# linyicheng1/trackingBench-SLAM

Hardware: AMD Instinct MI355X
Metric: frames/sec end-to-end (extract+match+local-BA) (higher is better)
Workload: dtype u8 (pyramid/FAST/ORB/Hamming) + f64 (pose-opt/BA); 1 GPU; 1280x720 stereo, 8-level pyramid x0.8, 2000 kpts/image (FAST 80/30), searchByBF L<->R, pose-opt, 10-KF/5000-pt local BA x10 iters; distinct_synthetic_pairs=64, distinct_ba_windows=32, ba_partitions=3, ba_schedule=joined at the end of every step, parallelism=frames sharded x1, RCCL gather of tracks

## Files before the change

### include/tb_capi.h

```cpp
#ifndef TB_CAPI_H
#define TB_CAPI_H

#include "tb_types.h"

#ifdef __cplusplus
extern "C" {
#endif

typedef struct tb_ctx tb_ctx;
typedef struct tb_extractor tb_extractor;

int tb_create(int device, tb_ctx** out);
void tb_destroy(tb_ctx* ctx);
const char* tb_last_error(const tb_ctx* ctx);
const char* tb_strerror(int code);
const char* tb_version(void);
int tb_set_stream(tb_ctx* ctx, void* hip_stream);
int tb_synchronize(tb_ctx* ctx);
int tb_profile_enable(tb_ctx* ctx, int on);
int tb_profile_only(tb_ctx* ctx, const char* kernel);
int tb_pack_rows_dev(tb_ctx* ctx, const void* src, int row_bytes, int cap, const int32_t* counts, int nframes, void* dst,
                     long long* total);
int tb_set_concurrency(tb_ctx* ctx, int peers);
int tb_measure_copy_seconds(tb_ctx* ctx, const void* d_src, void* d_dst, size_t bytes, int reps, double* seconds);
int tb_debug_force_dense_fast(tb_ctx* ctx, int on);
int tb_profile_report(tb_ctx* ctx, char* buf, int cap);

int tb_scale_factors(int nlevels, float scale, float* sf, float* inv_sf, float* sigma2, float* inv_sigma2);
int tb_pyramid_sizes(int width, int height, int nlevels, const float* sf, int* widths, int* heights);
int tb_orb_quotas(int nlevels, const float* sf, int target, int* quotas);

int tb_extractor_create(tb_ctx* ctx, int width, int height, int nlevels, const float* sf,
                        const int* widths, const int* heights,
                        int max_images, int max_target, tb_extractor** out);
void tb_extractor_destroy(tb_extractor* ex);
int tb_extractor_set_images_host(tb_extractor* ex, const uint8_t* images, int n, int stride, size_t pitch);
int tb_extractor_set_images_dev(tb_extractor* ex, const uint8_t* dev_images, int n, int stride, size_t pitch);
int tb_extractor_set_levels_host(tb_extractor* ex, int index, const uint8_t* const* levels, const int* strides);
int tb_extractor_build_pyramid(tb_extractor* ex, int n);
int tb_extractor_get_level_host(tb_extractor* ex, int index, int level, uint8_t* out, int out_stride);
int tb_extractor_orb(tb_extractor* ex, int n, int target, float init_th, float min_th, int quota_mode,
                     const tb_keypoint* exit_keys, int n_exit);
int tb_extractor_fastgrid(tb_extractor* ex, int n, const float* inv_sf, int target, float threshold,
                          const uint8_t* occupancy, int n_occupancy);
int tb_extractor_counts_host(tb_extractor* ex, int n, int* counts);
int tb_extractor_results_host(tb_extractor* ex, int index, tb_keypoint* kps, uint8_t* desc, int cap, int* count);
int tb_extractor_results_dev(tb_extractor* ex, const tb_keypoint** kps, const uint8_t** desc,
                             const int32_t** counts, int* kp_capacity);
int tb_extractor_copy_results_dev(tb_extractor* ex, int n, tb_keypoint* kps, uint8_t* desc, int32_t* counts, int cap);
int tb_extractor_candidates_host(tb_extractor* ex, int index, int level, tb_corner* out, int cap, int* count);

int tb_pyramid(tb_ctx* ctx, const uint8_t* image, int width, int height, int stride, int nlevels,
               const float* sf, uint8_t* const* levels_out, const int* strides_out);
int tb_fast_detect(tb_ctx* ctx, const uint8_t* image, int width, int height, int stride, int threshold,
                   int nms, tb_corner* out, int cap, int* count);
int tb_orb_extract(tb_ctx* ctx, const uint8_t* const* levels, const int* widths, const int* heights,
                   const int* strides, int nlevels, const float* sf, int target, float init_th, float min_th,
                   const tb_keypoint* exit_keys, int n_exit, int use_quotas, int* quotas_inout,
                   tb_keypoint* kps, uint8_t* desc, int cap, int* count);
int tb_fastgrid_extract(tb_ctx* ctx, const uint8_t* const* levels, const int* widths, const int* heights,
                        const int* strides, int nlevels, const float* inv_sf, int target, float threshold,
                        const uint8_t* occupancy, int n_occupancy, tb_keypoint* kps, int cap, int* count);

int tb_descriptor_distance(const uint8_t* a, const uint8_t* b);
void tb_three_maxima(const int* bin_sizes, int nbins, int* ind1, int* ind2, int* ind3);
int tb_match_bf(tb_ctx* ctx, const uint8_t* d1, int n1, const uint8_t* d2, int n2, int crosscheck,
                tb_match* out, int cap, int* count);
int tb_search_by_bf(tb_ctx* ctx, const uint8_t* d1, int n1, const uint8_t* d2, int n2, float ratio,
                    float min_th, tb_match* out, int cap, int* count);
int tb_search_by_bf_batch_dev(tb_ctx* ctx, int npairs, const uint8_t* desc1, const int32_t* counts1,
                              const uint8_t* desc2, const int32_t* counts2, size_t set_pitch,
                              float ratio, float min_th, tb_match* out, int cap, int32_t* out_counts);

typedef struct tb_lsh tb_lsh;
int tb_lsh_draw_bits(int tables, int key_size, uint64_t seed, uint16_t* out);
int tb_lsh_create(tb_ctx* ctx, int tables, int key_size, int multi_probe_level, uint64_t seed, const uint16_t* bits,
                  tb_lsh** out);
void tb_lsh_destroy(tb_lsh* lsh);
int tb_lsh_info(const tb_lsh* lsh, int* tables, int* key_size, int* multi_probe_level, uint16_t* bits);
int tb_match_lsh(tb_ctx* ctx, const tb_lsh* lsh, const uint8_t* d1, int n1, const uint8_t* d2, int n2, tb_match* out, int cap,
                 int* count);
int tb_search_by_nn(tb_ctx* ctx, const tb_lsh* lsh, const uint8_t* d1, int n1, const uint8_t* d2, int n2, float ratio,
                    float min_th, tb_match* out, int cap, int* count);
int tb_search_by_nn_batch_dev(tb_ctx* ctx, const tb_lsh* lsh, int npairs, const uint8_t* desc1, const int32_t* counts1,
                              const uint8_t* desc2, const int32_t* counts2, size_t set_pitch, float ratio, float min_th,
                              tb_match* out, int cap, int32_t* out_counts);
int tb_search_by_violence(tb_ctx* ctx, const tb_keypoint* k1, const uint8_t* d1, int n1,
                          const tb_keypoint* k2, const uint8_t* d2, int n2, int img2_width, int img2_height,
                          int min_level, int max_level, float radius, int th_low, float nratio,
                          int histo_len, int check_orientation, tb_match* out, int cap, int* count);

int tb_search_by_bow(tb_ctx* ctx, const tb_keypoint* k1, const uint8_t* d1, int n1, const uint32_t* nodes1, const int32_t* start1,
                     const uint32_t* items1, int nn1, const tb_keypoint* k2, const uint8_t* d2, int n2, const uint8_t* has_mp2,
                     const uint32_t* nodes2, const int32_t* start2, const uint32_t* items2, int nn2, int map_point_only, int th_low,
                     float nratio, int histo_len, int check_orientation, tb_match* out, int cap, int* count);

int tb_search_by_projection(tb_ctx* ctx, const float Tcw1[16], const tb_camera* cam1, int img1_width, int img1_height,
                            const tb_keypoint* k1, const uint8_t* d1, const uint8_t* taken1, int n1,
                            const tb_keypoint* k2, const tb_mappoint* mp2, const uint8_t* mp2_desc, int n2,
                            const float* scale_factors, int nlevels, float nratio, int th_high, int histo_len,
                            int check_orientation, tb_match* out, int cap, int* count);
int tb_search_by_projection_map(tb_ctx* ctx, const float Tcw1[16], const tb_camera* cam1, int img1_width, int img1_height,
                                const tb_keypoint* k1, const uint8_t* d1, const uint8_t* taken1, int n1,
                                const tb_mappoint* mps, const uint8_t* mp_desc, int nmp,
                                const float* scale_factors, int nlevels, float nratio, float radio, int th_high,
                                tb_match* out, int cap, int* count);

int tb_frame_grid_batch_dev(tb_ctx* ctx, int nframes, const tb_keypoint* keys, const int32_t* counts, int key_pitch,
                            int img_width, int img_height, int32_t* cell_start, int32_t* cell_items);
int tb_search_by_projection_batch_dev(tb_ctx* ctx, int npairs, const float* Tcw1, const tb_camera* cam1, int img1_width,
                                      int img1_height, const tb_keypoint* k1, const uint8_t* d1, const uint8_t* taken1,
                                      const int32_t* n1, int pitch1, const int32_t* cell_start, const int32_t* cell_items,
                                      const tb_keypoint* k2, const tb_mappoint* mp2, const uint8_t* mp2_desc,
                                      const int32_t* n2, int pitch2, const float* scale_factors, int nlevels, float nratio,
                                      int th_high, int histo_len, int check_orientation, tb_match* out, int cap,
                                      int32_t* out_counts, int32_t* flags);

int tb_search_by_projection_map_batch_dev(tb_ctx* ctx, int npairs, const float* Tcw1, const tb_camera* cam1, int img1_width,
                                          int img1_height, const tb_keypoint* k1, const uint8_t* d1, const uint8_t* taken1,
                                          const int32_t* n1, int pitch1, const int32_t* cell_start, const int32_t* cell_items,
                                          const tb_mappoint* mps, const uint8_t* mp_desc, const int32_t* nmp, int mp_pitch,
                                          int max_nmp, const float* scale_factors, int nlevels, float nratio, float radio,
                                          int th_high, tb_match* out, int cap, int32_t* out_counts, int32_t* flags);
int tb_search_by_violence_batch_dev(tb_ctx* ctx, int npairs, const tb_keypoint* k1, const uint8_t* d1, const int32_t* n1,
                                    int pitch1, const tb_keypoint* k2, const uint8_t* d2, const int32_t* n2, int pitch2,
                                    const int32_t* cell_start2, const int32_t* cell_items2, int img2_width, int img2_height,
                                    int min_level, int max_level, float radius, int th_low, float nratio, int histo_len,
                                    int check_orientation, tb_match* out, int cap, int32_t* out_counts, int32_t* flags);

typedef struct tb_vocab tb_vocab;
int tb_vocab_create(tb_ctx* ctx, const tb_vocabulary* host, tb_vocab** out);
void tb_vocab_destroy(tb_vocab* v);
int tb_bow_transform(tb_ctx* ctx, const tb_vocab* voc, const uint8_t* desc, int n, int levelsup, int32_t* word_ids,
                     double* weights, int32_t* node_ids);
int tb_bow_transform_batch_dev(tb_ctx* ctx, const tb_vocab* voc, int nframes, const uint8_t* desc, const int32_t* counts,
                               int desc_pitch, int levelsup, int32_t* word_ids, int32_t* node_ids, double* weights,
                               uint64_t* fv_keys, int32_t* fv_counts);
int tb_bow_vector_batch_dev(tb_ctx* ctx, const tb_vocab* voc, int nframes, const int32_t* word_ids, const double* weights,
                            const int32_t* counts, int desc_pitch, int32_t* bv_words, double* bv_values, int32_t* bv_counts);
enum { TB_SCORE_PAIRWISE = 0, TB_SCORE_ALL_PAIRS = 1 };
int tb_bow_score(int scoring, const int32_t* a_words, const double* a_values, int na, const int32_t* b_words, const double* b_values,
                 int nb, double* out);
int tb_bow_score_batch_dev(tb_ctx* ctx, int scoring, int mode, int na, const int32_t* a_words, const double* a_values,
                           const int32_t* a_counts, int a_pitch, int nb, const int32_t* b_words, const double* b_values,
                           const int32_t* b_counts, int b_pitch, double* out);
typedef struct tb_bow_db tb_bow_db;
int tb_bow_db_create(tb_ctx* ctx, int nseq, int capacity, int pitch, int scoring, tb_bow_db** out);
void tb_bow_db_destroy(tb_bow_db* db);
int tb_bow_db_clear(tb_bow_db* db);
int tb_bow_db_add_dev(tb_bow_db* db, const int32_t* bv_words, const double* bv_values, const int32_t* bv_counts, int src_pitch,
                      int32_t kf_id);
int tb_bow_db_query_dev(tb_bow_db* db, const int32_t* q_words, const double* q_values, const int32_t* q_counts, int q_pitch,
                        int exclude_newest, int topk, double* scores, int32_t* top_slot, int32_t* top_kf, double* top_score,
                        int32_t* top_count);
int tb_bow_db_state_dev(tb_bow_db* db, const int32_t** words, const double** values, const int32_t** counts, const int32_t** kf_ids,
                        int* nadded);
typedef struct tb_kf_store tb_kf_store;
typedef struct tb_reloc_params {
    int map_point_only, th_low; float nratio; int histo_len, check_orientation;
    int min_inliers;
} tb_reloc_params;
typedef struct tb_reloc_out {
    int32_t *cand_kf, *cand_matches, *cand_rows, *cand_inliers, *cand_flags;
    float* cand_Tcw;
    int32_t *best_rank, *best_kf;
    float* best_Tcw;
} tb_reloc_out;
int tb_kf_store_create(tb_ctx* ctx, int nseq, int capacity, int pitch, int max_candidates, tb_kf_store** out);
void tb_kf_store_destroy(tb_kf_store* st);
int tb_kf_store_clear(tb_kf_store* st);
int tb_kf_store_add_dev(tb_kf_store* st, const tb_keypoint* keys, const uint8_t* desc, const int32_t* counts, const uint64_t* fv_keys,
                        const int32_t* fv_counts, const float* map_points, const uint8_t* mp_valid, int src_pitch, const float* Tcw,
                        int32_t kf_id);
int tb_kf_store_state_dev(tb_kf_store* st, const tb_keypoint** keys, const uint8_t** desc, const int32_t** counts,
                          const uint64_t** fv_keys, const int32_t** fv_counts, const float** map_points, const uint8_t** mp_valid,
                          const float** Tcw, const int32_t** kf_ids, int* nadded);
int tb_kf_store_work_dev(tb_kf_store* st, tb_match** matches, int32_t** match_counts, const tb_obs** rows, const int32_t** row_counts,
                         const uint8_t** outlier, int* pitch);
int tb_relocalize_batch_dev(tb_kf_store* st, const double K[4], int nlevels, float scale, const tb_keypoint* q_keys,
                            const uint8_t* q_desc, const int32_t* q_counts, const uint64_t* q_fv_keys, const int32_t* q_fv_counts,
                            int q_pitch, const int32_t* cand_slot, int ncand, const tb_reloc_params* params, const tb_reloc_out* out);
int tb_reloc_rows_dev(tb_kf_store* st, int nlevels, float scale, const tb_keypoint* q_keys, const int32_t* q_counts, int q_pitch,
                      const int32_t* cand_slot, int ncand, const int32_t* match_counts, int32_t* cand_rows);
int tb_search_by_bow_batch_dev(tb_ctx* ctx, int npairs, const tb_keypoint* k1, const uint8_t* d1, int pitch1,
                               const uint64_t* fv1, const int32_t* fv_counts1, const tb_keypoint* k2, const uint8_t* d2, int pitch2,
                               const uint64_t* fv2, const int32_t* fv_counts2, const uint8_t* has_mp2, int map_point_only,
                               int th_low, float nratio, int histo_len, int check_orientation, tb_match* out, int cap,
                               int32_t* out_counts, int32_t* flags);

#define TB_VOC_MAX_L 8
typedef struct tb_vocab_train_params { int k, L, weighting, scoring; uint64_t seed; int max_iters; } tb_vocab_train_params;
typedef struct tb_vocab_train_stats { int nnodes, nwords, capped_nodes, empty_clusters; int iters_per_level[TB_VOC_MAX_L]; } tb_vocab_train_stats;
int tb_vocab_train_dev(tb_ctx* ctx, const tb_vocab_train_params* params, int ndocs, const uint8_t* desc, const int32_t* counts,
                       int desc_pitch, tb_vocab** out, tb_vocab_train_stats* stats);
int tb_vocab_train(tb_ctx* ctx, const tb_vocab_train_params* params, int ndocs, const uint8_t* desc, const int32_t* counts,
                   tb_vocab** out, tb_vocab_train_stats* stats);
int tb_vocab_info(const tb_vocab* voc, int* nnodes, int* nwords, int* k, int* L, int* weighting, int* scoring);
int tb_vocab_export(const tb_vocab* voc, int32_t* child_start, int32_t* child_items, uint8_t* desc, int32_t* word_id, double* weight);

int tb_stereo_tracks_to_obs_batch_dev(tb_ctx* ctx, int nframes, const tb_keypoint* keys_left, const tb_keypoint* keys_right,
                                      int key_pitch, const tb_match* matches, const int32_t* match_counts, int match_pitch,
                                      const float K[4], float bf, const float* inv_sigma2, int nlevels, tb_obs* obs, int obs_pitch,
                                      int32_t* obs_counts);

int tb_pose_opt(tb_ctx* ctx, const double K[4], const float Tcw_in[16], const tb_obs* obs, int n,
                uint8_t* outlier, float Tcw_out[16], int* n_inliers, double* stats);
int tb_pose_opt_batch_dev(tb_ctx* ctx, int nproblems, const double K[4], const float* Tcw_in,
                          const tb_obs* obs, const int32_t* counts, int obs_pitch, uint8_t* outlier,
                          float* Tcw_out, int32_t* n_inliers, double* stats);
int tb_clahe(tb_ctx* ctx, const uint8_t* src, int width, int height, int stride, double clip_limit, int tiles_x, int tiles_y,
             uint8_t* dst, int dst_stride);
int tb_clahe_dev(tb_ctx* ctx, const uint8_t* src, int width, int height, int stride, double clip_limit, int tiles_x, int tiles_y,
                 uint8_t* dst, int dst_stride);
int tb_optical_flow_pyr_lk(tb_ctx* ctx, const uint8_t* prev, const uint8_t* next, int width, int height, int stride,
                           const float* prev_pts, int n, int win, int max_level, float* next_pts, uint8_t* status,
                           float* err, int* top_level);
int tb_search_by_opflow(tb_ctx* ctx, const uint8_t* img1, const uint8_t* img2, int width, int height, int stride,
                        const tb_camera* cam1, const float* keys2_xy, int n, int equalized, int reject,
                        float* cur_points, tb_match* out, int cap, int* count);
int tb_search_by_opflow_batch_dev(tb_ctx* ctx, int npairs, const uint8_t* img1, const uint8_t* img2, int width, int height,
                                  int stride, size_t image_pitch, const tb_camera* cam1, const float* keys2_xy,
                                  const int32_t* counts, int pts_pitch, int equalized, int reject, float* cur_points,
                                  uint8_t* status, tb_match* out, int cap, int32_t* out_counts);
int tb_optical_flow_pyr_lk_dev(tb_ctx* ctx, const uint8_t* prev, const uint8_t* next, int width, int height, int stride,
                               const float* prev_pts, int n, int win, int max_level, float* next_pts, uint8_t* status,
                               float* err);
int tb_optical_flow_pyr_lk_batch_dev(tb_ctx* ctx, int npairs, const uint8_t* prev, const uint8_t* next, int width, int height,
                                     int stride, size_t image_pitch, const float* prev_pts, const int32_t* counts,
                                     int pts_pitch, int win, int max_level, float* next_pts, uint8_t* status, float* err);

int tb_find_fundamental_ransac(tb_ctx* ctx, const float* pts1, const float* pts2, int n, double thresh, double conf, uint8_t* mask,
                               double* F, int* iters, int* ok);
int tb_reject_with_f(tb_ctx* ctx, const float* cur_pts, const float* last_pts, int n, uint8_t* status);
int tb_reject_with_f_batch_dev(tb_ctx* ctx, int npairs, const float* cur_pts, const float* last_pts, const int32_t* counts,
                               int pts_pitch, uint8_t* status);
int tb_add_map_points_by_stereo(tb_ctx* ctx, const uint8_t* img_stereo, const uint8_t* img_current, int width, int height, int stride,
                                const tb_camera* cam_stereo, const float* keys_xy, int n, float bf, float* depth, int* n_depth);
int tb_add_map_points_by_stereo_batch_dev(tb_ctx* ctx, int npairs, const uint8_t* img_stereo, const uint8_t* img_current, int width,
                                          int height, int stride, size_t image_pitch, const tb_camera* cam_stereo, const float* keys_xy,
                                          const int32_t* counts, int pts_pitch, float bf, float* cur_points, uint8_t* status,
                                          float* depth);

int tb_local_ba(tb_ctx* ctx, const double K[4], int nkf, int nfixed, float* poses, int npt, float* pts,
                const tb_ba_obs* obs, int nobs, int iters, double* stats);
int tb_local_ba_batch_dev(tb_ctx* ctx, int nwindows, const double K[4], int nkf, int nfixed, float* poses, int npt,
                          float* pts, const tb_ba_obs* obs, const int32_t* obs_counts, int obs_pitch, int iters,
                          double* stats);

typedef struct tb_vo tb_vo;
typedef struct tb_vo_params {
    int width, height;
    int nlevels;
    float scale;
    int target;
    float init_th, min_th;
    double K[4];
    float bf;
    int keyframe_every;
} tb_vo_params;
int tb_vo_create(tb_ctx* ctx, const tb_vo_params* params, int nseq, tb_vo** out);
void tb_vo_destroy(tb_vo* vo);
int tb_vo_reset_dev(tb_vo* vo, const float* Tcw0);
int tb_vo_step_dev(tb_vo* vo, const uint8_t* left, const uint8_t* right, int stride, size_t pitch);
int tb_vo_state_dev(tb_vo* vo, const float** Tcw, const float** keys_xy, const float** map_points, const uint8_t** mp_valid,
                    const int32_t** key_counts, const tb_obs** obs, const int32_t** obs_counts, const int32_t** n_inliers,
                    const uint8_t** outlier, int* key_pitch, int* frame);

int tb_vo_reset_seq_dev(tb_vo* vo, const uint8_t* which, const float* Tcw0);
int tb_vo_step_ragged_dev(tb_vo* vo, const uint8_t* left, const uint8_t* right, int stride, size_t pitch, const uint8_t* active,
                          const uint8_t* force_keyframe);
int tb_vo_frames(tb_vo* vo, int32_t* frames, int32_t* kf_frames);

enum { TB_VO_OPFLOW = 0, TB_VO_BF = 1, TB_VO_VIOLENCE = 2, TB_VO_PROJECTION = 3, TB_VO_PROJECTION_MAP = 4, TB_VO_BOW = 5 };
typedef struct tb_vo_tracker {
    int kind;
    float bf_ratio, bf_min_th;
    int min_level, max_level;
    float radius;
    int th_low; float nratio; int histo_len; int check_orientation;
    int th_high;
    float radio;
    int map_keyframes;
} tb_vo_tracker;
int tb_vo_create_ex(tb_ctx* ctx, const tb_vo_params* params, const tb_vo_tracker* tracker, int nseq, tb_vo** out);
int tb_vo_tracker_state_dev(tb_vo* vo, const tb_keypoint** orb, const uint8_t** orb_desc, const int32_t** orb_counts,
                            const tb_match** matches, const int32_t** match_counts, const int32_t** flags, const tb_keypoint** kf_orb,
                            const uint8_t** kf_desc, const float** kf_map_points, const uint8_t** kf_mp_valid,
                            const int32_t** kf_counts, int* kf_frame);
typedef struct tb_vo_bow {
    int levelsup;
    int map_point_only;
    int th_low; float nratio; int histo_len; int check_orientation;
} tb_vo_bow;
int tb_vo_create_bow(tb_ctx* ctx, const tb_vo_params* params, const tb_vo_bow* bow, const tb_vocab* voc, int nseq, tb_vo** out);
enum { TB_VO_NN = 6 };
typedef struct tb_vo_lsh {
    float ratio, min_th;
    int min_level, max_level;
    int tables, key_size, multi_probe_level;
    uint64_t seed;
    const uint16_t* bits;
} tb_vo_lsh;
int tb_vo_create_lsh(tb_ctx* ctx, const tb_vo_params* params, const tb_vo_lsh* lsh, int nseq, tb_vo** out);
int tb_vo_bow_state_dev(tb_vo* vo, const uint64_t** fv_keys, const int32_t** fv_counts, const int32_t** bv_words, const double** bv_values,
                        const int32_t** bv_counts, const int32_t** word_ids, const int32_t** node_ids, const uint64_t** kf_fv_keys,
                        const int32_t** kf_fv_counts, const int32_t** kf_bv_words, const double** kf_bv_values, const int32_t** kf_bv_counts,
                        const int32_t** kf_word_ids, const int32_t** kf_node_ids);
int tb_vo_bow_db_enable(tb_vo* vo, int capacity);
int tb_vo_bow_db_get(tb_vo* vo, tb_bow_db** out);
int tb_vo_reloc_enable(tb_vo* vo, int max_candidates);
int tb_vo_relocalize_dev(tb_vo* vo, int topk, int exclude_newest, int min_inliers, double* scores, int32_t* top_slot, int32_t* top_kf,
                         double* top_score, int32_t* top_count, const tb_reloc_out* out);
int tb_vo_kf_store_get(tb_vo* vo, tb_kf_store** out);
typedef struct tb_vo_recover {
    int lost_inliers;
    int topk;
    int exclude_newest;
    int min_inliers;
} tb_vo_recover;
int tb_vo_recover_enable(tb_vo* vo, const tb_vo_recover* prm);
int tb_vo_recover_state_dev(tb_vo* vo, const uint8_t** lost, const int32_t** track_inliers, const int32_t** recovered_kf,
                            const int32_t** kf_ids, const int32_t** kf_word_ring, const int32_t** kf_node_ring);
typedef struct tb_vo_window_ba {
    int iters;
    int fixed;
    int min_obs;
    int min_points;
} tb_vo_window_ba;
int tb_vo_window_ba_enable(tb_vo* vo, const tb_vo_window_ba* prm);
int tb_vo_window_state_dev(tb_vo* vo, const float** seg_keys, const uint8_t** seg_ok, const float** seg_pose, const float** seg_pts,
                           const uint8_t** seg_spawned, const tb_ba_obs** obs, const int32_t** obs_counts, const int32_t** n_points,
                           const double** stats, const uint8_t** adopted, const float** ba_pose, const float** ba_pts, int* slot,
                           int* nslots);
int tb_vo_mp_desc_dev(tb_vo* vo, const uint8_t** mp_desc, const uint8_t** kf_mp_desc);
int tb_vo_map_state_dev(tb_vo* vo, const tb_mappoint** points, const uint8_t** desc, const int32_t** counts,
                        const int32_t** block_counts, int* capacity, int* map_keyframes, int* blocks);

typedef struct tb_batch_params {
    int width, height, nlevels;
    float scale;
    int target;
    float init_th, min_th;
    float bf_ratio, bf_min_th;
} tb_batch_params;
int tb_batch_run(tb_ctx** ctxs, int ngpu, const tb_batch_params* p, int nframes, const uint8_t* left, const uint8_t* right,
                 int stride, size_t pitch, int cap, tb_keypoint* kps, uint8_t* desc, int32_t* counts, tb_match* matches,
                 int32_t* match_counts);

#ifdef __cplusplus
}
#endif
#endif
```

### trackingbench_slam_amd/capi.py

```python
import ctypes as C
import os
import subprocess

import numpy as np

_HERE = os.path.dirname(os.path.abspath(__file__))
LIB_PATH = os.environ.get("TB_HIP_LIB") or os.path.join(_HERE, "libtb_hip.so")
_LIB = None

KEYPOINT = np.dtype([("x", "<f4"), ("y", "<f4"), ("size", "<f4"), ("angle", "<f4"),
                     ("response", "<f4"), ("octave", "<i4"), ("class_id", "<i4")])
MATCH = np.dtype([("queryIdx", "<i4"), ("trainIdx", "<i4"), ("imgIdx", "<i4"), ("distance", "<f4")])
CORNER = np.dtype([("x", "<i4"), ("y", "<i4"), ("score", "<i4")])
OBS = np.dtype([("u", "<f4"), ("v", "<f4"), ("X", "<f4"), ("Y", "<f4"), ("Z", "<f4"), ("inv_sigma2", "<f4")])
BA_OBS = np.dtype([("kf", "<i4"), ("pt", "<i4"), ("u", "<f4"), ("v", "<f4"), ("inv_sigma2", "<f4")])
CAMERA = np.dtype([("fx", "<f4"), ("fy", "<f4"), ("cx", "<f4"), ("cy", "<f4"), ("width", "<i4"), ("height", "<i4"),
                   ("has_distortion", "<i4"), ("d", "<f4", (5,))])
MAPPOINT = np.dtype([("pos", "<f4", (3,)), ("normal", "<f4", (3,)), ("min_dist", "<f4"), ("max_dist", "<f4"), ("bad", "<i4")])

TB_OK, TB_EINVAL, TB_ENOMEM, TB_ECAPACITY, TB_EUNSUPPORTED, TB_EDEVICE, TB_ESTATE = 0, -1, -2, -3, -4, -5, -6

EXPORTS = [
    "tb_create", "tb_destroy", "tb_last_error", "tb_strerror", "tb_version", "tb_set_stream", "tb_synchronize",
    "tb_profile_enable", "tb_profile_only", "tb_profile_report", "tb_debug_force_dense_fast", "tb_measure_copy_seconds", "tb_set_concurrency", "tb_pack_rows_dev",
    "tb_scale_factors", "tb_pyramid_sizes", "tb_orb_quotas",
    "tb_extractor_create", "tb_extractor_destroy", "tb_extractor_set_images_host", "tb_extractor_set_images_dev",
    "tb_extractor_set_levels_host", "tb_extractor_build_pyramid", "tb_extractor_get_level_host", "tb_extractor_orb",
    "tb_extractor_fastgrid", "tb_extractor_counts_host", "tb_extractor_results_host", "tb_extractor_results_dev",
    "tb_extractor_candidates_host", "tb_extractor_copy_results_dev",
    "tb_pyramid", "tb_fast_detect", "tb_orb_extract", "tb_fastgrid_extract",
    "tb_descriptor_distance", "tb_three_maxima", "tb_match_bf", "tb_search_by_bf", "tb_search_by_bf_batch_dev",
    "tb_search_by_violence", "tb_search_by_bow", "tb_search_by_projection", "tb_search_by_projection_map", "tb_frame_grid_batch_dev",
    "tb_search_by_projection_batch_dev", "tb_search_by_projection_map_batch_dev",
    "tb_search_by_violence_batch_dev", "tb_stereo_tracks_to_obs_batch_dev", "tb_vocab_create", "tb_vocab_destroy", "tb_bow_transform",
    "tb_bow_transform_batch_dev", "tb_search_by_bow_batch_dev", "tb_pose_opt", "tb_pose_opt_batch_dev", "tb_local_ba", "tb_local_ba_batch_dev",
    "tb_clahe", "tb_clahe_dev", "tb_optical_flow_pyr_lk", "tb_optical_flow_pyr_lk_dev", "tb_optical_flow_pyr_lk_batch_dev", "tb_search_by_opflow", "tb_search_by_opflow_batch_dev",
    "tb_find_fundamental_ransac", "tb_reject_with_f", "tb_reject_with_f_batch_dev", "tb_add_map_points_by_stereo", "tb_add_map_points_by_stereo_batch_dev",
    "tb_batch_run", "tb_vo_create", "tb_vo_destroy", "tb_vo_reset_dev", "tb_vo_step_dev", "tb_vo_state_dev",
    "tb_vo_create_ex", "tb_vo_tracker_state_dev", "tb_vo_mp_desc_dev", "tb_vo_map_state_dev",
    "tb_vocab_train", "tb_vocab_train_dev", "tb_vocab_info", "tb_vocab_export",
    "tb_bow_vector_batch_dev", "tb_vo_create_bow", "tb_vo_bow_state_dev",
    "tb_bow_score", "tb_bow_score_batch_dev", "tb_bow_db_create", "tb_bow_db_destroy", "tb_bow_db_clear", "tb_bow_db_add_dev",
    "tb_bow_db_query_dev", "tb_bow_db_state_dev", "tb_vo_bow_db_enable", "tb_vo_bow_db_get",
    "tb_kf_store_create", "tb_kf_store_destroy", "tb_kf_store_clear", "tb_kf_store_add_dev", "tb_kf_store_state_dev",
    "tb_kf_store_work_dev", "tb_relocalize_batch_dev", "tb_reloc_rows_dev", "tb_vo_reloc_enable", "tb_vo_relocalize_dev",
    "tb_vo_kf_store_get", "tb_vo_recover_enable", "tb_vo_recover_state_dev",
    "tb_vo_reset_seq_dev", "tb_vo_step_ragged_dev", "tb_vo_frames",
    "tb_vo_window_ba_enable", "tb_vo_window_state_dev",
    "tb_lsh_draw_bits", "tb_lsh_create", "tb_lsh_destroy", "tb_lsh_info", "tb_match_lsh", "tb_search_by_nn", "tb_search_by_nn_batch_dev",
    "tb_vo_create_lsh",
]

TB_VOC_MAX_L = 8
TB_SCORE_PAIRWISE, TB_SCORE_ALL_PAIRS = 0, 1


class VocabTrainParams(C.Structure):
    _fields_ = [("k", C.c_int), ("L", C.c_int), ("weighting", C.c_int), ("scoring", C.c_int), ("seed", C.c_uint64), ("max_iters", C.c_int)]


class VocabTrainStats(C.Structure):
    _fields_ = [("nnodes", C.c_int), ("nwords", C.c_int), ("capped_nodes", C.c_int), ("empty_clusters", C.c_int),
                ("iters_per_level", C.c_int * TB_VOC_MAX_L)]

    def as_dict(self):
        return dict(nnodes=self.nnodes, nwords=self.nwords, capped_nodes=self.capped_nodes, empty_clusters=self.empty_clusters,
                    iters_per_level=list(self.iters_per_level))


class TBError(RuntimeError):
    def __init__(self, code, msg):
        super().__init__("tb error %d: %s" % (code, msg))
        self.code = code


def build(force=False):
    if force or not os.path.exists(LIB_PATH):
        subprocess.check_call(["make", "-C", os.path.join(_HERE, "csrc"), "-j8"], stdout=subprocess.DEVNULL,
                              stderr=subprocess.DEVNULL)
    return LIB_PATH


def lib():
    global _LIB
    if _LIB is None:
        if not os.path.exists(LIB_PATH):
            raise TBError(TB_EDEVICE, "libtb_hip.so is not built (run __graft_entry__.build())")
        try:
            import torch
        except ImportError:
            pass
        L = C.CDLL(LIB_PATH)
        L.tb_last_error.restype = C.c_char_p
        L.tb_strerror.restype = C.c_char_p
        L.tb_version.restype = C.c_char_p
        L.tb_destroy.restype = None
        L.tb_extractor_destroy.restype = None
        L.tb_three_maxima.restype = None
        L.tb_vocab_destroy.restype = None
        L.tb_vocab_destroy.argtypes = [C.c_void_p]
        L.tb_last_error.argtypes = [C.c_void_p]
        L.tb_destroy.argtypes = [C.c_void_p]
        L.tb_extractor_destroy.argtypes = [C.c_void_p]
        L.tb_vo_destroy.restype = None
        L.tb_vo_destroy.argtypes = [C.c_void_p]
        L.tb_bow_db_destroy.restype = None
        L.tb_bow_db_destroy.argtypes = [C.c_void_p]
        L.tb_kf_store_destroy.restype = None
        L.tb_kf_store_destroy.argtypes = [C.c_void_p]
        L.tb_lsh_destroy.restype = None
        L.tb_lsh_destroy.argtypes = [C.c_void_p]
        _LIB = L
    return _LIB


def _p(a):
    return a.ctypes.data_as(C.c_void_p) if a is not None else None


def _u8img(img):
    img = np.ascontiguousarray(img, dtype=np.uint8)
    assert img.ndim == 2
    return img


def scale_factors(n, scale):
    sf = np.zeros(n, np.float32); isf = np.zeros(n, np.float32)
    s2 = np.zeros(n, np.float32); is2 = np.zeros(n, np.float32)
    rc = lib().tb_scale_factors(n, C.c_float(scale), _p(sf), _p(isf), _p(s2), _p(is2))
    if rc:
        raise TBError(rc, "tb_scale_factors")
    return sf, isf, s2, is2


def pyramid_sizes(w, h, sf):
    sf = np.ascontiguousarray(sf, np.float32)
    ws = np.zeros(len(sf), np.int32); hs = np.zeros(len(sf), np.int32)
    rc = lib().tb_pyramid_sizes(int(w), int(h), len(sf), _p(sf), _p(ws), _p(hs))
    if rc:
        raise TBError(rc, "tb_pyramid_sizes")
    return ws, hs


def orb_quotas(sf, target):
    sf = np.ascontiguousarray(sf, np.float32)
    q = np.zeros(len(sf), np.int32)
    rc = lib().tb_orb_quotas(len(sf), _p(sf), int(target), _p(q))
    if rc:
        raise TBError(rc, "tb_orb_quotas")
    return q


def descriptor_distance(a, b):
    a = np.ascontiguousarray(a, np.uint8); b = np.ascontiguousarray(b, np.uint8)
    return int(lib().tb_descriptor_distance(_p(a), _p(b)))


def three_maxima(sizes):
    sizes = np.ascontiguousarray(sizes, np.int32)
    i1, i2, i3 = C.c_int(-1), C.c_int(-1), C.c_int(-1)
    lib().tb_three_maxima(_p(sizes), len(sizes), C.byref(i1), C.byref(i2), C.byref(i3))
    return i1.value, i2.value, i3.value


class BatchParams(C.Structure):
    _fields_ = [("width", C.c_int), ("height", C.c_int), ("nlevels", C.c_int), ("scale", C.c_float), ("target", C.c_int),
                ("init_th", C.c_float), ("min_th", C.c_float), ("bf_ratio", C.c_float), ("bf_min_th", C.c_float)]


def batch_run(contexts, left, right, nlevels=8, scale=0.8, target=2000, init_th=80.0, min_th=30.0, bf_ratio=10.0,
              bf_min_th=30.0, cap=None):
    left = np.ascontiguousarray(left, np.uint8); right = np.ascontiguousarray(right, np.uint8)
    F, H, W = left.shape
    assert right.shape == left.shape and len(contexts) >= 1
    cap = int(cap or (target + 512))
    prm = BatchParams(W, H, int(nlevels), float(scale), int(target), float(init_th), float(min_th), float(bf_ratio), float(bf_min_th))
    kps = np.zeros((2, F, cap), KEYPOINT); desc = np.zeros((2, F, cap, 32), np.uint8); cnt = np.zeros((2, F), np.int32)
    mt = np.zeros((F, cap), MATCH); mc = np.zeros(F, np.int32)
    hs = (C.c_void_p * len(contexts))(*[c._h for c in contexts])
    rc = lib().tb_batch_run(hs, len(contexts), C.byref(prm), F, _p(left), _p(right), W, C.c_size_t(W * H), cap, _p(kps), _p(desc),
                            _p(cnt), _p(mt), _p(mc))
    if rc != 0:
        msgs = [lib().tb_last_error(c._h).decode() for c in contexts]
        raise TBError(rc, "; ".join(m for m in msgs if m) or lib().tb_strerror(rc).decode())
    return [(kps[0, f, :cnt[0, f]].copy(), desc[0, f, :cnt[0, f]].copy(), kps[1, f, :cnt[1, f]].copy(), desc[1, f, :cnt[1, f]].copy(),
             mt[f, :mc[f]].copy()) for f in range(F)]


class VOParams(C.Structure):
    _fields_ = [("width", C.c_int), ("height", C.c_int), ("nlevels", C.c_int), ("scale", C.c_float), ("target", C.c_int),
                ("init_th", C.c_float), ("min_th", C.c_float), ("K", C.c_double * 4), ("bf", C.c_float), ("keyframe_every", C.c_int)]


TB_VO_OPFLOW, TB_VO_BF, TB_VO_VIOLENCE, TB_VO_PROJECTION, TB_VO_PROJECTION_MAP = 0, 1, 2, 3, 4
TB_VO_BOW = 5
TB_VO_NN = 6


class VOTracker(C.Structure):
    _fields_ = [("kind", C.c_int), ("bf_ratio", C.c_float), ("bf_min_th", C.c_float), ("min_level", C.c_int), ("max_level", C.c_int),
                ("radius", C.c_float), ("th_low", C.c_int), ("nratio", C.c_float), ("histo_len", C.c_int),
                ("check_orientation", C.c_int), ("th_high", C.c_int), ("radio", C.c_float), ("map_keyframes", C.c_int)]


class VOBow(C.Structure):
    _fields_ = [("levelsup", C.c_int), ("map_point_only", C.c_int), ("th_low", C.c_int), ("nratio", C.c_float), ("histo_len", C.c_int),
                ("check_orientation", C.c_int)]


class VOLsh(C.Structure):
    _fields_ = [("ratio", C.c_float), ("min_th", C.c_float), ("min_level", C.c_int), ("max_level", C.c_int), ("tables", C.c_int),
                ("key_size", C.c_int), ("multi_probe_level", C.c_int), ("seed", C.c_uint64), ("bits", C.c_void_p)]


def lsh_draw_bits(tables, key_size, seed):
    out = np.zeros((max(int(tables), 0), max(int(key_size), 0)), np.uint16)
    rc = lib().tb_lsh_draw_bits(int(tables), int(key_size), C.c_uint64(int(seed) & (2 ** 64 - 1)), _p(out))
    if rc != TB_OK:
        raise TBError(rc, lib().tb_strerror(rc).decode())
    return out


def _lsh_bits(bits, tables, key_size):
    if bits is None:
        return None
    b = np.asarray(bits)
    if b.shape != (int(tables), int(key_size)) or b.min() < 0 or b.max() > 65535:
        raise ValueError("bits: a [tables, key_size] table of bit indices")
    return np.ascontiguousarray(b, np.uint16)


class VORecover(C.Structure):
    _fields_ = [("lost_inliers", C.c_int), ("topk", C.c_int), ("exclude_newest", C.c_int), ("min_inliers", C.c_int)]


class VOWindowBA(C.Structure):
    _fields_ = [("iters", C.c_int), ("fixed", C.c_int), ("min_obs", C.c_int), ("min_points", C.c_int)]


class VO:

    def __init__(self, ctx, params, nseq, tracker=None, use_ex=False, bow=None, vocab=None, lsh=None):
        self.ctx = ctx
        self.nseq = int(nseq)
        self._h = C.c_void_p()
        if lsh is not None:
            ctx.check(lib().tb_vo_create_lsh(ctx._h, C.byref(params), C.byref(lsh), self.nseq, C.byref(self._h)))
        elif bow is not None:
            ctx.check(lib().tb_vo_create_bow(ctx._h, C.byref(params), C.byref(bow), vocab, self.nseq, C.byref(self._h)))
        elif tracker is None and not use_ex:
            ctx.check(lib().tb_vo_create(ctx._h, C.byref(params), self.nseq, C.byref(self._h)))
        else:
            trp = C.byref(tracker) if tracker is not None else None
            ctx.check(lib().tb_vo_create_ex(ctx._h, C.byref(params), trp, self.nseq, C.byref(self._h)))

    def close(self):
        if self._h and self.ctx._h:
            lib().tb_vo_destroy(self._h)
        self._h = C.c_void_p()

    def __del__(self):
        try:
            self.close()
        except Exception:
            pass

    def reset_dev(self, Tcw0_ptr):
        self.ctx.check(lib().tb_vo_reset_dev(self._h, C.c_void_p(Tcw0_ptr)))

    def step_dev(self, left_ptr, right_ptr, stride, pitch):
        return lib().tb_vo_step_dev(self._h, C.c_void_p(left_ptr), C.c_void_p(right_ptr or None), int(stride), C.c_size_t(pitch))

    def reset_seq_dev(self, which, Tcw0_ptr):
        w = np.ascontiguousarray(np.asarray(which, bool).astype(np.uint8))
        assert w.shape == (self.nseq,)
        return lib().tb_vo_reset_seq_dev(self._h, _p(w), C.c_void_p(Tcw0_ptr))

    def step_ragged_dev(self, left_ptr, right_ptr, stride, pitch, active=None, force_keyframe=None):
        m = [None if x is None else np.ascontiguousarray(np.asarray(x, bool).astype(np.uint8)) for x in (active, force_keyframe)]
        assert all(x is None or x.shape == (self.nseq,) for x in m)
        return lib().tb_vo_step_ragged_dev(self._h, C.c_void_p(left_ptr), C.c_void_p(right_ptr or None), int(stride), C.c_size_t(pitch),
                                           _p(m[0]), _p(m[1]))

    def frames(self):
        f, k = np.zeros(self.nseq, np.int32), np.zeros(self.nseq, np.int32)
        self.ctx.check(lib().tb_vo_frames(self._h, _p(f), _p(k)))
        return f, k

    def state_dev(self):
        ptrs = [C.c_void_p() for _ in range(9)]
        pitch, frame = C.c_int(0), C.c_int(0)
        self.ctx.check(lib().tb_vo_state_dev(self._h, *[C.byref(q) for q in ptrs], C.byref(pitch), C.byref(frame)))
        names = ("Tcw", "keys_xy", "map_points", "mp_valid", "key_counts", "obs", "obs_counts", "n_inliers", "outlier")
        out = {k: q.value for k, q in zip(names, ptrs)}
        out["key_pitch"], out["frame"] = pitch.value, frame.value
        return out

    def tracker_state_dev(self):
        ptrs = [C.c_void_p() for _ in range(11)]
        kf_frame = C.c_int(0)
        self.ctx.check(lib().tb_vo_tracker_state_dev(self._h, *[C.byref(q) for q in ptrs], C.byref(kf_frame)))
        names = ("orb", "orb_desc", "orb_counts", "matches", "match_counts", "flags", "kf_orb", "kf_desc", "kf_map_points",
                 "kf_mp_valid", "kf_counts")
        out = {k: q.value for k, q in zip(names, ptrs)}
        out["kf_frame"] = kf_frame.value
        return out

    def bow_state_dev(self):
        names = ("fv_keys", "fv_counts", "bv_words", "bv_values", "bv_counts", "word_ids", "node_ids")
        names = names + tuple("kf_" + n for n in names)
        ptrs = [C.c_void_p() for _ in names]
        self.ctx.check(lib().tb_vo_bow_state_dev(self._h, *[C.byref(q) for q in ptrs]))
        return {k: q.value for k, q in zip(names, ptrs)}

    def bow_db_enable(self, capacity):
        rc = lib().tb_vo_bow_db_enable(self._h, int(capacity))
        if rc == 0:
            self._db_capacity = int(capacity)
        return rc

    def bow_db(self):
        h = C.c_void_p()
        self.ctx.check(lib().tb_vo_bow_db_get(self._h, C.byref(h)))
        return BowDatabase(self.ctx, self.nseq, self._db_capacity, self.state_dev()["key_pitch"], None, handle=h)

    def reloc_enable(self, max_candidates):
        rc = lib().tb_vo_reloc_enable(self._h, int(max_candidates))
        if rc == 0:
            self._max_candidates = int(max_candidates)
        return rc

    def kf_store(self):
        h = C.c_void_p()
        self.ctx.check(lib().tb_vo_kf_store_get(self._h, C.byref(h)))
        return KeyframeStore(self.ctx, self.nseq, self._db_capacity, self.state_dev()["key_pitch"], self._max_candidates, handle=h)

    def relocalize_dev(self, topk, exclude_newest, min_inliers, capacity, device):
        import torch
        S, k = self.nseq, max(int(topk), 0)
        q = dict(scores=torch.empty((S, capacity), dtype=torch.float64, device=device),
                 top_slot=torch.empty((S, k), dtype=torch.int32, device=device), top_kf=torch.empty((S, k), dtype=torch.int32, device=device),
                 top_score=torch.empty((S, k), dtype=torch.float64, device=device), top_count=torch.empty(S, dtype=torch.int32, device=device))
        ro, out = reloc_out(S, k, device)
        p = lambda t: C.c_void_p(t.data_ptr()) if t.numel() else None
        rc = lib().tb_vo_relocalize_dev(self._h, int(topk), int(exclude_newest), int(min_inliers), p(q["scores"]), p(q["top_slot"]),
                                        p(q["top_kf"]), p(q["top_score"]), p(q["top_count"]), C.byref(ro))
        q.update(out)
        return rc, q

    def recover_enable(self, prm):
        return lib().tb_vo_recover_enable(self._h, C.byref(prm) if prm is not None else None)

    def recover_state_dev(self):
        names = ("lost", "track_inliers", "recovered_kf", "kf_ids", "kf_word_ring", "kf_node_ring")
        ptrs = [C.c_void_p() for _ in names]
        self.ctx.check(lib().tb_vo_recover_state_dev(self._h, *[C.byref(q) for q in ptrs]))
        return {k: q.value for k, q in zip(names, ptrs)}

    def window_ba_enable(self, prm):
        return lib().tb_vo_window_ba_enable(self._h, C.byref(prm) if prm is not None else None)

    def window_state_dev(self):
        names = ("seg_keys", "seg_ok", "seg_pose", "seg_pts", "seg_spawned", "obs", "obs_counts", "n_points", "stats", "adopted",
                 "ba_pose", "ba_pts")
        ptrs = [C.c_void_p() for _ in names]
        slot, nslots = C.c_int(0), C.c_int(0)
        self.ctx.check(lib().tb_vo_window_state_dev(self._h, *[C.byref(q) for q in ptrs], C.byref(slot), C.byref(nslots)))
        out = {k: q.value for k, q in zip(names, ptrs)}
        out["slot"], out["nslots"] = slot.value, nslots.value
        return out

    def mp_desc_dev(self):
        a, b = C.c_void_p(), C.c_void_p()
        self.ctx.check(lib().tb_vo_mp_desc_dev(self._h, C.byref(a), C.byref(b)))
        return dict(mp_desc=a.value, kf_mp_desc=b.value)

    def map_state_dev(self):
        ptrs = [C.c_void_p() for _ in range(4)]
        cap, mk, nb = C.c_int(0), C.c_int(0), C.c_int(0)
        self.ctx.check(lib().tb_vo_map_state_dev(self._h, *[C.byref(q) for q in ptrs], C.byref(cap), C.byref(mk), C.byref(nb)))
        out = {k: q.value for k, q in zip(("points", "desc", "counts", "block_counts"), ptrs)}
        out["capacity"], out["map_keyframes"], out["blocks"] = cap.value, mk.value, nb.value
        return out


class Context:

    def __init__(self, device=0, stream=None):
        self._h = C.c_void_p()
        rc = lib().tb_create(int(device), C.byref(self._h))
        if rc:
            raise TBError(rc, "tb_create(device=%d): %s" % (device, lib().tb_strerror(rc).decode()))
        if stream is not None:
            self.set_stream(stream)

    def close(self):
        if self._h:
            lib().tb_destroy(self._h)
            self._h = C.c_void_p()

    def __del__(self):
        try:
            self.close()
        except Exception:
            pass

    def check(self, rc):
        if rc:
            raise TBError(rc, lib().tb_last_error(self._h).decode() or lib().tb_strerror(rc).decode())

    def set_stream(self, stream_ptr):
        if stream_ptr is None:
            self.check(lib().tb_set_stream(self._h, None))
            return
        if int(stream_ptr) == 0:
            raise ValueError("stream handle 0 (the legacy null stream / torch's default stream) is not accepted: "
                             "create a torch.cuda.Stream() and pass its .cuda_stream, or pass None")
        self.check(lib().tb_set_stream(self._h, C.c_void_p(int(stream_ptr))))

    def synchronize(self):
        self.check(lib().tb_synchronize(self._h))

    def profile_enable(self, on=True, only=None):
        self.check(lib().tb_profile_only(self._h, only.encode() if only else None))
        self.check(lib().tb_profile_enable(self._h, int(on)))

    def measure_copy_seconds(self, src_ptr, dst_ptr, nbytes, reps=10):
        sec = C.c_double(0)
        self.check(lib().tb_measure_copy_seconds(self._h, C.c_void_p(src_ptr), C.c_void_p(dst_ptr), C.c_size_t(nbytes), int(reps), C.byref(sec)))
        return sec.value

    def set_concurrency(self, peers):
        self.check(lib().tb_set_concurrency(self._h, int(peers)))

    def force_dense_fast(self, on=True):
        self.check(lib().tb_debug_force_dense_fast(self._h, int(on)))

    def profile_report(self):
        buf = C.create_string_buffer(8192)
        self.check(lib().tb_profile_report(self._h, buf, len(buf)))
        out = {}
        for line in buf.value.decode().splitlines():
            name, calls, ms = line.split()
            out[name] = (int(calls), float(ms))
        return out

    def pyramid(self, img, nlevels, scale):
        img = _u8img(img)
        sf = scale_factors(nlevels, scale)[0]
        ws, hs = pyramid_sizes(img.shape[1], img.shape[0], sf)
        levels = [img] + [np.zeros((int(hs[i]), int(ws[i])), np.uint8) for i in range(1, nlevels)]
        ptrs = (C.c_void_p * nlevels)(*[l.ctypes.data for l in levels])
        st = np.array([l.strides[0] for l in levels], np.int32)
        self.check(lib().tb_pyramid(self._h, _p(img), img.shape[1], img.shape[0], img.strides[0], nlevels, _p(sf), ptrs, _p(st)))
        return levels, sf

    def fast_detect(self, img, th, nms=True):
        img = _u8img(img)
        cap = img.size // (4 if nms else 1) + 4096
        out = np.zeros(cap, CORNER)
        n = C.c_int(0)
        self.check(lib().tb_fast_detect(self._h, _p(img), img.shape[1], img.shape[0], img.strides[0], int(th), int(nms),
                                        _p(out), cap, C.byref(n)))
        return out[:n.value].copy()

    @staticmethod
    def _level_args(levels):
        levels = [_u8img(l) for l in levels]
        n = len(levels)
        ptrs = (C.c_void_p * n)(*[l.ctypes.data for l in levels])
        ws = np.array([l.shape[1] for l in levels], np.int32)
        hs = np.array([l.shape[0] for l in levels], np.int32)
        st = np.array([l.strides[0] for l in levels], np.int32)
        return levels, ptrs, ws, hs, st

    def orb_extract(self, levels, sf, target, init_th, min_th, exit_keys=None, quotas=None):
        levels, ptrs, ws, hs, st = self._level_args(levels)
        sf = np.ascontiguousarray(sf, np.float32)
        cap = int(target) + 64 * len(levels) + 64
        if quotas is not None:
            cap = max(cap, int(np.sum(quotas)) + 64 * len(levels) + 64)
        kps = np.zeros(cap, KEYPOINT)
        desc = np.zeros((cap, 32), np.uint8)
        q = np.zeros(len(levels), np.int32) if quotas is None else np.ascontiguousarray(quotas, np.int32).copy()
        ek = None if exit_keys is None else np.ascontiguousarray(exit_keys, KEYPOINT)
        n = C.c_int(0)
        self.check(lib().tb_orb_extract(self._h, ptrs, _p(ws), _p(hs), _p(st), len(levels), _p(sf), int(target),
                                        C.c_float(init_th), C.c_float(min_th), _p(ek), 0 if ek is None else len(ek),
                                        int(quotas is not None), _p(q), _p(kps), _p(desc), cap, C.byref(n)))
        return kps[:n.value].copy(), desc[:n.value].copy(), q

    def fastgrid_extract(self, levels, inv_sf, target, threshold, occupancy=None):
        levels, ptrs, ws, hs, st = self._level_args(levels)
        inv_sf = np.ascontiguousarray(inv_sf, np.float32)
        cap = int(target) * 2 + 4096
        kps = np.zeros(cap, KEYPOINT)
        occ = None if occupancy is None else np.ascontiguousarray(occupancy, np.uint8)
        n = C.c_int(0)
        self.check(lib().tb_fastgrid_extract(self._h, ptrs, _p(ws), _p(hs), _p(st), len(levels), _p(inv_sf), int(target),
                                             C.c_float(threshold), _p(occ), 0 if occ is None else len(occ), _p(kps), cap,
                                             C.byref(n)))
        return kps[:n.value].copy()

    @staticmethod
    def _desc(d):
        d = np.ascontiguousarray(d, np.uint8)
        if d.size == 0:
            d = d.reshape(0, 32)
        assert d.ndim == 2 and d.shape[1] == 32
        return d

    def bf_match(self, d1, d2, crosscheck=True):
        d1, d2 = self._desc(d1), self._desc(d2)
        out = np.zeros(max(len(d1), 1), MATCH)
        n = C.c_int(0)
        self.check(lib().tb_match_bf(self._h, _p(d1), len(d1), _p(d2), len(d2), int(crosscheck), _p(out), len(out), C.byref(n)))
        return out[:n.value].copy()

    def search_by_bf(self, d1, d2, ratio, min_th):
        d1, d2 = self._desc(d1), self._desc(d2)
        out = np.zeros(max(len(d1), 1), MATCH)
        n = C.c_int(0)
        self.check(lib().tb_search_by_bf(self._h, _p(d1), len(d1), _p(d2), len(d2), C.c_float(ratio), C.c_float(min_th),
                                         _p(out), len(out), C.byref(n)))
        return out[:n.value].copy()

    def lsh(self, tables=20, key_size=10, multi_probe_level=2, seed=0, bits=None):
        return Lsh(self, tables, key_size, multi_probe_level, seed, bits)

    def match_lsh(self, lsh, d1, d2):
        d1, d2 = self._desc(d1), self._desc(d2)
        out = np.zeros(max(len(d1), 1), MATCH)
        n = C.c_int(0)
        self.check(lib().tb_match_lsh(self._h, lsh._h, _p(d1), len(d1), _p(d2), len(d2), _p(out), len(out), C.byref(n)))
        return out[:n.value].copy()

    def search_by_nn(self, lsh, d1, d2, ratio, min_th, cap=None):
        d1, d2 = self._desc(d1), self._desc(d2)
        out = np.zeros(max(len(d1), 1) if cap is None else max(int(cap), 1), MATCH)
        n = C.c_int(0)
        self.check(lib().tb_search_by_nn(self._h, lsh._h, _p(d1), len(d1), _p(d2), len(d2), C.c_float(ratio), C.c_float(min_th), _p(out),
                                         len(out) if cap is None else int(cap), C.byref(n)))
        return out[:n.value].copy()

    def search_by_nn_batch_dev(self, lsh, npairs, desc1_ptr, counts1_ptr, desc2_ptr, counts2_ptr, set_pitch, ratio, min_th, out_ptr, cap,
                               out_counts_ptr):
        return lib().tb_search_by_nn_batch_dev(self._h, lsh._h, int(npairs), C.c_void_p(desc1_ptr), C.c_void_p(counts1_ptr),
                                               C.c_void_p(desc2_ptr), C.c_void_p(counts2_ptr), C.c_size_t(set_pitch), C.c_float(ratio),
                                               C.c_float(min_th), C.c_void_p(out_ptr), int(cap), C.c_void_p(out_counts_ptr))

    def search_by_violence(self, k1, d1, k2, d2, img2_w, img2_h, min_level=0, max_level=1, radius=10.0, th_low=50,
                           nratio=0.0, histo_len=30, check_orientation=True):
        k1 = np.ascontiguousarray(k1, KEYPOINT); k2 = np.ascontiguousarray(k2, KEYPOINT)
        d1, d2 = self._desc(d1), self._desc(d2)
        out = np.zeros(max(len(k1), 1), MATCH)
        n = C.c_int(0)
        self.check(lib().tb_search_by_violence(self._h, _p(k1), _p(d1), len(k1), _p(k2), _p(d2), len(k2), int(img2_w),
                                               int(img2_h), int(min_level), int(max_level), C.c_float(radius), int(th_low),
                                               C.c_float(nratio), int(histo_len), int(check_orientation), _p(out), len(out),
                                               C.byref(n)))
        return out[:n.value].copy()

    @staticmethod
    def _fv(fv):
        nodes = np.array(sorted(fv), np.uint32)
        start = np.zeros(len(nodes) + 1, np.int32)
        items = []
        for i, nd in enumerate(nodes):
            items.extend(int(x) for x in fv[int(nd)])
            start[i + 1] = len(items)
        return nodes, start, np.array(items, np.uint32)

    def search_by_bow(self, k1, d1, fv1, k2, d2, fv2, has_mp2=None, map_point_only=False, th_low=50, nratio=0.0, histo_len=30,
                      check_orientation=True):
        k1 = np.ascontiguousarray(k1, KEYPOINT); k2 = np.ascontiguousarray(k2, KEYPOINT)
        d1, d2 = self._desc(d1), self._desc(d2)
        n1a, s1a, i1a = self._fv(fv1)
        n2a, s2a, i2a = self._fv(fv2)
        hm = None if has_mp2 is None else np.ascontiguousarray(has_mp2, np.uint8)
        out = np.zeros(max(len(i1a), 1), MATCH)
        n = C.c_int(0)
        self.check(lib().tb_search_by_bow(self._h, _p(k1), _p(d1), len(k1), _p(n1a), _p(s1a), _p(i1a), len(n1a), _p(k2), _p(d2), len(k2),
                                          _p(hm), _p(n2a), _p(s2a), _p(i2a), len(n2a), int(map_point_only), int(th_low),
                                          C.c_float(nratio), int(histo_len), int(check_orientation), _p(out), len(out), C.byref(n)))
        return out[:n.value].copy()

    def clahe(self, img, clip_limit=3.0, tiles=(8, 8)):
# ... 543 lines not shown
```

### trackingbench_slam_amd/csrc/k_ba.hip

```cpp
#include <mutex>
#include <type_traits>
#include "tb_internal.h"
#include "tb_device.h"
#include "tb_se3.h"

#define BA_T 256
#ifndef BA_KFCH
#define BA_KFCH 512
#endif
#ifndef BA_KFBLK
#define BA_KFBLK 4
#endif
#define BA_BIG_MAXF 64
#define BA_SMALL_MAXF 10
#define BA_SORT_LDS 8192
#ifndef BA_EMAX
#define BA_EMAX 64
#endif
#ifndef BA_PCAP
#define BA_PCAP 21
#endif

struct BaState {
    double lambda, ni, currentChi, chi0, scale_p, rho;
    int iter, qmax, status, need_lin, cur, ok2, done_iters, err;
    int sing, pad0, hq_fresh, pad2;
};

struct BaDims {
    int W, nkf, nfixed, nfree, np, npt, obs_pitch, iters;
    int nblkP, kfChunks, G, nChunks;
    int Gbase, Gextra;
    int Vbase, Vextra;
    int big, npairs;
    unsigned long long oBigA;
    unsigned long long oPairStart, oPairCnt, oPairItems, maxItems;
    double fx, fy, cx, cy;
    unsigned long long wstride, oT, oP, oHll, oBl, oHq, oHpp, oBp, oXp, oPartKF, oPartP, oPartS;
    unsigned long long istride, oPtStart, oPtFree, oKfStart, oKfEdges, oFreeKP;
    unsigned long long oKfRec;
    unsigned long long oPtMask, oPermA, oPermB, oPtRank, oKPs, oGDesc;
    unsigned long long oGCost;
    unsigned long long oGCut;
    int renum;
    unsigned long long oPerm;
    int schurWaveLds;
    int wgReduce;
};

__host__ __device__ inline int ba_schur_waves(const BaDims& d, int w) {
    return d.wgReduce ? 4 * (d.Gbase + (w < d.Gextra ? 1 : 0)) : d.Vbase + (w < d.Vextra ? 1 : 0);
}
__device__ __forceinline__ void ba_schur_unit(int u, int base, int extra, int& w, int& i) {
    const int head = extra * (base + 1);
    if (u < head) { w = u / (base + 1); i = u - w * (base + 1); }
    else { const int r = u - head; w = extra + r / base; i = r - (w - extra) * base; }
}

typedef double ba_d4 __attribute__((ext_vector_type(4)));
typedef double ba_d2 __attribute__((ext_vector_type(2)));

__device__ __forceinline__ double ba_huber_rho0(double c, double delta) {
    const double dsqr = delta * delta;
    return (c <= dsqr) ? c : 2 * sqrt(c) * delta - dsqr;
}
struct BaLin { double ww, e0, e1, c2, invz; double pc[3]; double Jl[6]; };
__device__ __forceinline__ double ba_rcp(double x) {
    double r = __builtin_amdgcn_rcp(x);
    r = fma(fma(-x, r, 1.0), r, r);
    r = fma(fma(-x, r, 1.0), r, r);
    return r;
}
__device__ __forceinline__ void ba_residual(const double* Rt, const double* X, float u, float v, float inv_sigma2, double fx,
                                            double fy, double cx, double cy, double delta, BaLin& L) {
#pragma unroll
    for (int i = 0; i < 3; i++) L.pc[i] = fma(Rt[3 * i + 2], X[2], fma(Rt[3 * i + 1], X[1], fma(Rt[3 * i], X[0], Rt[9 + i])));
    L.invz = ba_rcp(L.pc[2]);
    L.e0 = (double)u - fma(L.pc[0] * L.invz, fx, cx);
    L.e1 = (double)v - fma(L.pc[1] * L.invz, fy, cy);
    const double wgt = (double)inv_sigma2;
    L.c2 = fma(L.e0, wgt * L.e0, L.e1 * (wgt * L.e1));
    const double r1 = (L.c2 <= delta * delta) ? 1.0 : delta / sqrt(L.c2);
    L.ww = r1 * wgt;
}
__device__ __forceinline__ void ba_linearize(const double* Rt, const double* X, float u, float v, float inv_sigma2, double fx,
                                             double fy, double cx, double cy, double delta, BaLin& L) {
    ba_residual(Rt, X, u, v, inv_sigma2, fx, fy, cx, cy, delta, L);
    const double ax = -(L.pc[0] * L.invz) * fx, ay = -(L.pc[1] * L.invz) * fy, m = -L.invz;
#pragma unroll
    for (int c = 0; c < 3; c++) {
        L.Jl[c] = m * fma(ax, Rt[6 + c], fx * Rt[c]);
        L.Jl[3 + c] = m * fma(ay, Rt[6 + c], fy * Rt[3 + c]);
    }
}
__device__ __forceinline__ void ba_pose_to_Rt(const double* T7, double* Rt) {
    PoSE3 s;
    s.qx = T7[0]; s.qy = T7[1]; s.qz = T7[2]; s.qw = T7[3]; s.tx = T7[4]; s.ty = T7[5]; s.tz = T7[6];
    po_to_R(s, Rt);
    Rt[9] = s.tx; Rt[10] = s.ty; Rt[11] = s.tz;
}
__device__ __forceinline__ void ba_jac_pose_iz(const double* pc, double invz, double fx, double fy, double* J) {
    const double xz = pc[0] * invz, yz = pc[1] * invz, xf = xz * fx, yf = yz * fy;
    J[0] = xf * yz; J[1] = -fma(xf, xz, fx); J[2] = yz * fx;
    J[3] = -invz * fx; J[4] = 0; J[5] = xf * invz;
    J[6] = fma(yf, yz, fy); J[7] = -(xz * yf); J[8] = -xz * fy;
    J[9] = 0; J[10] = -invz * fy; J[11] = yf * invz;
}

__device__ __forceinline__ bool ba_inv3(const double* H6, double lambda, double* I) {
    const double A0 = H6[0] + lambda, A1 = H6[1], A2 = H6[2], A4 = H6[3] + lambda, A5 = H6[4], A8 = H6[5] + lambda;
    const double A3 = A1, A6 = A2, A7 = A5;
    const double det = A0 * (A4 * A8 - A5 * A7) - A1 * (A3 * A8 - A5 * A6) + A2 * (A3 * A7 - A4 * A6);
    if (!(fabs(det) > 0)) return false;
    const double id = 1.0 / det;
    I[0] = (A4 * A8 - A5 * A7) * id; I[1] = (A2 * A7 - A1 * A8) * id; I[2] = (A1 * A5 - A2 * A4) * id;
    I[3] = (A5 * A6 - A3 * A8) * id; I[4] = (A0 * A8 - A2 * A6) * id; I[5] = (A2 * A3 - A0 * A5) * id;
    I[6] = (A3 * A7 - A4 * A6) * id; I[7] = (A1 * A6 - A0 * A7) * id; I[8] = (A0 * A4 - A1 * A3) * id;
    return true;
}
__device__ __forceinline__ PoSE3 ba_load_se3(const double* p) {
    PoSE3 s;
    s.qx = p[0]; s.qy = p[1]; s.qz = p[2]; s.qw = p[3]; s.tx = p[4]; s.ty = p[5]; s.tz = p[6];
    return s;
}
__device__ __forceinline__ void ba_store_se3(double* p, const PoSE3& s) {
    p[0] = s.qx; p[1] = s.qy; p[2] = s.qz; p[3] = s.qw; p[4] = s.tx; p[5] = s.ty; p[6] = s.tz;
}
__device__ __forceinline__ double ba_block_sum1(double v, double* red) {
    const int wave = threadIdx.x >> 6, lane = threadIdx.x & 63;
    v = po_wave_sum(v);
    __syncthreads();
    if (lane == 0) red[wave] = v;
    __syncthreads();
    return (red[0] + red[1]) + (red[2] + red[3]);
}
__device__ __forceinline__ double ba_block_max1(double v, double* red) {
    const int wave = threadIdx.x >> 6, lane = threadIdx.x & 63;
#pragma unroll
    for (int d = 32; d > 0; d >>= 1) v = fmax(v, __shfl_xor(v, d, 64));
    __syncthreads();
    if (lane == 0) red[wave] = v;
    __syncthreads();
    return fmax(fmax(red[0], red[1]), fmax(red[2], red[3]));
}

template <class Pred, class Pred2, class Visit>
__device__ __forceinline__ int ba_ordered_rank(int n, int* tmp, Pred pred, Pred2 pred2, int* total2, Visit visit) {
    const int wave = threadIdx.x >> 6, lane = threadIdx.x & 63;
    const int q = (((n + 3) >> 2) + 63) & ~63, lo = min(wave * q, n), hi = min(lo + q, n);
    int cnt = 0, cnt2 = 0;
    for (int e0 = lo; e0 < hi; e0 += 256) {
#pragma unroll
        for (int i = 0; i < 4; i++) {
            const int e = e0 + 64 * i + lane;
            cnt += (e < hi && pred(e)) ? 1 : 0;
            cnt2 += (e < hi && pred2(e)) ? 1 : 0;
        }
    }
    cnt = tb_wave_sum(cnt);
    cnt2 = tb_wave_sum(cnt2);
    if (lane == 0) { tmp[wave] = cnt; tmp[4 + wave] = cnt2; }
    __syncthreads();
    int base = 0;
    for (int v = 0; v < wave; v++) base += tmp[v];
    const int total = tmp[0] + tmp[1] + tmp[2] + tmp[3];
    *total2 = tmp[4] + tmp[5] + tmp[6] + tmp[7];
    const unsigned long long lt = (lane == 0) ? 0ull : (~0ull >> (64 - lane));
    for (int e0 = lo; e0 < hi; e0 += 256) {
        bool f[4];
#pragma unroll
        for (int i = 0; i < 4; i++) { const int e = e0 + 64 * i + lane; f[i] = e < hi && pred(e); }
#pragma unroll
        for (int i = 0; i < 4; i++) {
            const int e = e0 + 64 * i + lane;
            const unsigned long long m = __ballot(f[i]);
            if (e < hi) visit(e, base + __popcll(m & lt), f[i]);
            base += __popcll(m);
        }
    }
    __syncthreads();
    return total;
}

__global__ void __launch_bounds__(BA_T)
k_ba_setup(BaDims d, const float* __restrict__ poses, const float* __restrict__ pts, const tb_ba_obs* __restrict__ obsOrig,
           const tb_ba_obs* __restrict__ obsAll, const int32_t* __restrict__ obsCounts, double* __restrict__ dw, int* __restrict__ iw,
           BaState* __restrict__ states, int* __restrict__ errflag) {
    __shared__ int tmp[8];
    const int w = blockIdx.y, k = blockIdx.x, tid = threadIdx.x;
    const tb_ba_obs* obs = obsOrig + (size_t)w * d.obs_pitch;
    const int nobs = min(obsCounts[w], d.obs_pitch);
    double* D = dw + (size_t)w * d.wstride;
    int* I = iw + (size_t)w * d.istride;
    BaState* st = states + w;
    {
        const int nb = gridDim.x, per = (nobs + nb - 1) / nb;
        bool bad = false;
        for (int e = k * per + tid; e < min((k + 1) * per, nobs); e += BA_T) {
            const tb_ba_obs o = obs[e];
            if (o.kf < 0 || o.kf >= d.nkf || o.pt < 0 || o.pt >= d.npt || (e > 0 && o.pt < obs[e - 1].pt)) bad = true;
            for (int b0 = 1; b0 <= d.nkf && b0 <= e; b0 += 8) {
                int pk[8], pp[8];
#pragma unroll
                for (int i = 0; i < 8; i++) { const int ee = max(e - b0 - i, 0); pk[i] = obs[ee].kf; pp[i] = obs[ee].pt; }
#pragma unroll
                for (int i = 0; i < 8; i++)
                    if (b0 + i <= d.nkf && b0 + i <= e && pp[i] == o.pt && pk[i] == o.kf) bad = true;
                if (pp[7] != o.pt) break;
            }
        }
        if (bad) errflag[w] = 1;
    }
    obs = obsAll + (size_t)w * d.obs_pitch;
    if (d.renum && k != d.nkf) return;
    if (k < d.nkf) {
        int base = 0;
        const int mine = ba_ordered_rank(nobs, tmp, [&](int e) { return obs[e].kf == k; },
                                         [&](int e) { const int kf = obs[e].kf; return kf >= 0 && kf < k; }, &base,
                                         [&](int e, int rank, bool hit) {
                                             if (hit) {
                                                 I[d.oKfEdges + base + rank] = e;
                                                 const tb_ba_obs o = obs[e];
                                                 int4 r;
                                                 r.x = o.pt; r.y = __float_as_int(o.u); r.z = __float_as_int(o.v); r.w = __float_as_int(o.inv_sigma2);
                                                 *reinterpret_cast<int4*>(I + d.oKfRec + 4 * (size_t)(base + rank)) = r;
                                             }
                                         });
        if (tid == 0) {
            I[d.oKfStart + k] = base;
            if (k == d.nkf - 1) I[d.oKfStart + d.nkf] = base + mine;
        }
        return;
    }
    if (k == d.nkf + 1) {
        int unused = 0;
        const int nfreeE = ba_ordered_rank(nobs, tmp, [&](int e) { return obs[e].kf >= d.nfixed; }, [](int) { return false; }, &unused,
            [&](int e, int ce, bool hit) {
                const int prev = (e > 0) ? obs[e - 1].pt : -1, cur = obs[e].pt;
                for (int p = max(prev + 1, 0); p <= min(cur, d.npt); p++) I[d.oPtFree + p] = ce;
                if (hit) {
                    const tb_ba_obs o = obs[e];
                    int4 r;
                    r.x = (int)(((unsigned)cur << 6) | ((unsigned)(o.kf - d.nfixed) & 63u));
                    r.y = __float_as_int(o.u); r.z = __float_as_int(o.v); r.w = __float_as_int(o.inv_sigma2);
                    *reinterpret_cast<int4*>(I + d.oFreeKP + 4 * (size_t)ce) = r;
                }
            });
        for (int p = max((nobs > 0 ? obs[nobs - 1].pt : -1) + 1, 0) + tid; p <= d.npt; p += BA_T) I[d.oPtFree + p] = nfreeE;
        return;
    }
    if (tid == 0) {
        st->lambda = 0; st->ni = 2; st->currentChi = 0; st->chi0 = 0; st->scale_p = 0; st->rho = 0;
        st->iter = 0; st->qmax = 0; st->status = (d.iters > 0 && nobs > 0) ? 0 : 1; st->need_lin = 1; st->cur = 0; st->ok2 = 1;
        st->done_iters = 0; st->err = 0; st->sing = 0; st->hq_fresh = 0;
    }
    __syncthreads();
    if (!d.renum) {
        for (int e = tid; e < nobs; e += BA_T) {
            const int prev = (e > 0) ? obs[e - 1].pt : -1, cur = obs[e].pt;
            for (int p = max(prev + 1, 0); p <= min(cur, d.npt); p++) I[d.oPtStart + p] = e;
        }
        for (int p = max((nobs > 0 ? obs[nobs - 1].pt : -1) + 1, 0) + tid; p <= d.npt; p += BA_T) I[d.oPtStart + p] = nobs;
        if (d.big) for (int p = tid; p < d.npt; p += BA_T) I[d.oPtRank + p] = p;
    }
    for (int kk = tid; kk < d.nkf; kk += BA_T) {
        const float* T = poses + ((size_t)w * d.nkf + kk) * 16;
        double R[9], t[3];
        for (int i = 0; i < 3; i++) { for (int j = 0; j < 3; j++) R[i * 3 + j] = (double)T[i * 4 + j]; t[i] = (double)T[i * 4 + 3]; }
        const PoSE3 s = po_from_Rt(R, t);
        ba_store_se3(D + d.oT + (size_t)kk * 7, s);
        ba_store_se3(D + d.oT + (size_t)(d.nkf + kk) * 7, s);
    }
    for (int i = tid; i < d.npt * 3; i += BA_T) {
        const int r = i / 3, c = i - 3 * r;
        const double v = (double)pts[(size_t)w * d.npt * 3 + (d.renum ? 3 * (size_t)I[d.oPerm + r] + c : (size_t)i)];
        D[d.oP + i] = v;
        D[d.oP + (size_t)d.npt * 3 + i] = v;
    }
}

__device__ __forceinline__ void ba_write_rec(double* q, const double* Hll, const double* bl, const double* X, double lambda,
                                             BaState* st) {
    const double a00 = Hll[0] + lambda, a10 = Hll[1], a20 = Hll[2], a11 = Hll[3] + lambda, a21 = Hll[4], a22 = Hll[5] + lambda;
    bool ok = a00 > 0;
    const double i00 = 1.0 / sqrt(ok ? a00 : 1.0), c10 = a10 * i00, c20 = a20 * i00;
    const double d1 = a11 - c10 * c10;
    ok = ok && d1 > 0;
    const double i11 = 1.0 / sqrt(ok ? d1 : 1.0), c21 = (a21 - c20 * c10) * i11;
    const double d2 = a22 - c20 * c20 - c21 * c21;
    ok = ok && d2 > 0 && isfinite(d2);
    const double i22 = 1.0 / sqrt(ok ? d2 : 1.0);
    if (!ok) st->sing = 1;
    const double u00 = i00, u11 = i11, u22 = i22, u01 = -c10 * i00 * i11, u12 = -c21 * i11 * i22,
                 u02 = -(c20 * i00 + c21 * u01) * i22;
    q[0] = ok ? u00 : 0.0; q[1] = ok ? u01 : 0.0; q[2] = ok ? u02 : 0.0;
    q[3] = ok ? u11 : 0.0; q[4] = ok ? u12 : 0.0; q[5] = ok ? u22 : 0.0;
    q[6] = bl[0]; q[7] = bl[1]; q[8] = bl[2];
    q[9] = X[0]; q[10] = X[1]; q[11] = X[2];
}
__device__ __forceinline__ void ba_rec_utb(const double* q, double* t) {
    t[0] = q[0] * q[6];
    t[1] = q[1] * q[6] + q[3] * q[7];
    t[2] = q[2] * q[6] + q[4] * q[7] + q[5] * q[8];
}

__device__ __forceinline__ void ba_points_pass(const BaDims& d, const tb_ba_obs* __restrict__ obsAll, double* __restrict__ dw, const int* __restrict__ iw,
                                               BaState* __restrict__ states, const int* __restrict__ errflag, int bx, int w) {
    __shared__ double red[4];
    extern __shared__ __attribute__((aligned(16))) double sRt[];
    const int tid = threadIdx.x;
    if (errflag[w]) {
        if (bx == 0 && tid == 0) { states[w].status = 1; states[w].err = 1; }
        return;
    }
    const BaState st = states[w];
    if (st.status) return;
    double* D = dw + (size_t)w * d.wstride;
    const int* I = iw + (size_t)w * d.istride;
    const bool lam_known = st.iter > 0 || !st.need_lin;
    const tb_ba_obs* obs = obsAll + (size_t)w * d.obs_pitch;
    const double* T = D + d.oT + (size_t)st.cur * d.nkf * 7;
    const double* P = D + d.oP + (size_t)st.cur * d.npt * 3;
    for (int k = tid; k < d.nkf; k += BA_T) ba_pose_to_Rt(T + k * 7, sRt + k * 12);
    __syncthreads();
    const double delta = (double)sqrtf(5.991f);
    const int p = bx * BA_T + tid;
    double chi = 0, maxd = 0;
    if (p < d.npt) {
        double Hll[6] = {0, 0, 0, 0, 0, 0}, bl[3] = {0, 0, 0};
        const double X[3] = {P[3 * p], P[3 * p + 1], P[3 * p + 2]};
        const int eBeg = I[d.oPtStart + p], eEnd = I[d.oPtStart + p + 1];
        tb_ba_obs on = obs[min(eBeg, d.obs_pitch - 1)];
        for (int e = eBeg; e < eEnd; e++) {
            const tb_ba_obs o = on;
            on = obs[min(e + 1, d.obs_pitch - 1)];
            BaLin L;
            ba_linearize(sRt + o.kf * 12, X, o.u, o.v, o.inv_sigma2, d.fx, d.fy, d.cx, d.cy, delta, L);
            const double ww = L.ww, e0 = L.e0, e1 = L.e1;
            const double* Jl = L.Jl;
            chi += ba_huber_rho0(L.c2, delta);
            for (int a = 0; a < 3; a++) bl[a] = fma(-ww, fma(Jl[a], e0, Jl[3 + a] * e1), bl[a]);
            Hll[0] = fma(ww, fma(Jl[0], Jl[0], Jl[3] * Jl[3]), Hll[0]);
            Hll[1] = fma(ww, fma(Jl[0], Jl[1], Jl[3] * Jl[4]), Hll[1]);
            Hll[2] = fma(ww, fma(Jl[0], Jl[2], Jl[3] * Jl[5]), Hll[2]);
            Hll[3] = fma(ww, fma(Jl[1], Jl[1], Jl[4] * Jl[4]), Hll[3]);
            Hll[4] = fma(ww, fma(Jl[1], Jl[2], Jl[4] * Jl[5]), Hll[4]);
            Hll[5] = fma(ww, fma(Jl[2], Jl[2], Jl[5] * Jl[5]), Hll[5]);
        }
        if (!lam_known) {
            for (int a = 0; a < 6; a++) D[d.oHll + (size_t)p * 6 + a] = Hll[a];
            for (int a = 0; a < 3; a++) D[d.oBl + (size_t)p * 3 + a] = bl[a];
        } else ba_write_rec(D + d.oHq + (size_t)I[d.oPtRank + p] * 12, Hll, bl, X, st.lambda, states + w);
        maxd = fmax(fabs(Hll[0]), fmax(fabs(Hll[3]), fabs(Hll[5])));
    }
    const double s = ba_block_sum1(chi, red);
    const double m = ba_block_max1(maxd, red);
    if (tid == 0) {
        D[d.oPartP + (size_t)bx * 4] = s;
        D[d.oPartP + (size_t)bx * 4 + 1] = m;
    }
}

#define BA_KFG 14
#define BA_KFR_LDS (4 * (BA_KFG * 65 + 64) + 4 * 27)
__device__ __forceinline__ double ba_block_sum27(const double (&v)[27], double* sh) {
    const int tid = threadIdx.x, wave = tid >> 6, lane = tid & 63;
    double* T = sh + wave * (BA_KFG * 65 + 64);
    double* Qs = T + BA_KFG * 65;
    double* red = sh + 4 * (BA_KFG * 65 + 64);
#pragma unroll
    for (int g = 0; g < (27 + BA_KFG - 1) / BA_KFG; g++) {
        const int nv = min(BA_KFG, 27 - BA_KFG * g);
#pragma unroll
        for (int i = 0; i < BA_KFG; i++)
            if (i < nv) T[i * 65 + lane] = v[BA_KFG * g + i];
        __builtin_amdgcn_fence(__ATOMIC_SEQ_CST, "wavefront");
        const int q = lane / BA_KFG, i = lane - BA_KFG * q;
        if (lane < 4 * BA_KFG && i < nv) {
            const double* src = T + i * 65 + 16 * q;
            double s = src[0];
#pragma unroll
            for (int k = 1; k < 16; k++) s += src[k];
            Qs[lane] = s;
        }
        __builtin_amdgcn_fence(__ATOMIC_SEQ_CST, "wavefront");
        if (lane < nv) red[wave * 27 + BA_KFG * g + lane] = (Qs[lane] + Qs[BA_KFG + lane]) + (Qs[2 * BA_KFG + lane] + Qs[3 * BA_KFG + lane]);
        __builtin_amdgcn_fence(__ATOMIC_SEQ_CST, "wavefront");
    }
    __syncthreads();
    double r = 0;
    if (tid < 27) r = (red[tid] + red[27 + tid]) + (red[54 + tid] + red[81 + tid]);
    __syncthreads();
    return r;
}

__device__ __forceinline__ void ba_kf_pass(const BaDims& d, const tb_ba_obs* __restrict__ obsAll, double* __restrict__ dw, const int* __restrict__ iw,
                                           const BaState* __restrict__ states, const int* __restrict__ errflag, int bid) {
    __shared__ double red[BA_KFR_LDS];
    const int tid = threadIdx.x, nx = min(BA_KFBLK, d.kfChunks), per = nx * d.nfree;
    const int run = bid / (8 * per), rr_ = bid - run * (8 * per);
    const int w = run * 8 + (rr_ & 7), slot = rr_ >> 3;
    if (w >= d.W) return;
    if (errflag[w]) return;
    const int chunk0 = slot % nx, kfree = slot / nx, kf = d.nfixed + kfree;
    const BaState st = states[w];
    if (st.status || !st.need_lin) return;
    double* D = dw + (size_t)w * d.wstride;
    const int* I = iw + (size_t)w * d.istride;
    const int beg = I[d.oKfStart + kf], end = I[d.oKfStart + kf + 1];
    double Tk[12];
    ba_pose_to_Rt(D + d.oT + ((size_t)st.cur * d.nkf + kf) * 7, Tk);
    const double* P = D + d.oP + (size_t)st.cur * d.npt * 3;
    const double delta = (double)sqrtf(5.991f);
    for (int chunk = chunk0; chunk * BA_KFCH < end - beg; chunk += BA_KFBLK) {
        double acc[27];
#pragma unroll
        for (int i = 0; i < 27; i++) acc[i] = 0;
        int4 rr[BA_KFCH / BA_T];
        double XX[BA_KFCH / BA_T][3];
        const int4* KR = reinterpret_cast<const int4*>(I + d.oKfRec);
#pragma unroll
        for (int j = 0; j < BA_KFCH / BA_T; j++) {
            const int idx = beg + chunk * BA_KFCH + j * BA_T + tid;
            rr[j] = KR[min(idx, end - 1)];
            if (idx >= end) rr[j].x = -1;
        }
#pragma unroll
        for (int j = 0; j < BA_KFCH / BA_T; j++) {
            const int p = min(max(rr[j].x, 0), d.npt - 1);
            XX[j][0] = P[3 * p]; XX[j][1] = P[3 * p + 1]; XX[j][2] = P[3 * p + 2];
        }
#pragma unroll
        for (int j = 0; j < BA_KFCH / BA_T; j++) {
            if (rr[j].x < 0) continue;
            const float ou = __int_as_float(rr[j].y), ov = __int_as_float(rr[j].z), ow = __int_as_float(rr[j].w);
            const double* X = XX[j];
            double Jp[12];
            BaLin L;
            ba_residual(Tk, X, ou, ov, ow, d.fx, d.fy, d.cx, d.cy, delta, L);
            ba_jac_pose_iz(L.pc, L.invz, d.fx, d.fy, Jp);
            const double ww = L.ww, e0 = L.e0, e1 = L.e1;
#pragma unroll
            for (int a = 0; a < 6; a++) {
                const double wa = ww * Jp[a], wb = ww * Jp[6 + a];
                acc[21 + a] -= fma(wa, e0, wb * e1);
#pragma unroll
                for (int c = a; c < 6; c++) {
                    const int at = a * 6 - (a * (a - 1)) / 2 + (c - a);
                    acc[at] += fma(wa, Jp[c], wb * Jp[6 + c]);
                }
            }
        }
        const double tot = ba_block_sum27(acc, red);
        if (tid < 27) D[d.oPartKF + ((size_t)kfree * d.kfChunks + chunk) * 27 + tid] = tot;
    }
}

__global__ void __launch_bounds__(BA_T)
k_ba_points(BaDims d, const tb_ba_obs* __restrict__ obsAll, double* __restrict__ dw, const int* __restrict__ iw, BaState* __restrict__ states,
            const int* __restrict__ errflag) {
    ba_points_pass(d, obsAll, dw, iw, states, errflag, (int)blockIdx.x, (int)blockIdx.y);
}
__global__ void __launch_bounds__(BA_T)
k_ba_kf(BaDims d, const tb_ba_obs* __restrict__ obsAll, double* __restrict__ dw, const int* __restrict__ iw, const BaState* __restrict__ states,
        const int* __restrict__ errflag) {
    ba_kf_pass(d, obsAll, dw, iw, states, errflag, (int)blockIdx.x);
}
__global__ void __launch_bounds__(BA_T)
k_ba_lin(BaDims d, const tb_ba_obs* __restrict__ obsAll, double* __restrict__ dw, const int* __restrict__ iw, BaState* __restrict__ states,
         const int* __restrict__ errflag, int nKfBlocks) {
    if ((int)blockIdx.x < nKfBlocks) ba_kf_pass(d, obsAll, dw, iw, states, errflag, (int)blockIdx.x);
    else {
        const int b = (int)blockIdx.x - nKfBlocks;
        ba_points_pass(d, obsAll, dw, iw, states, errflag, b % d.nblkP, b / d.nblkP);
    }
}

__device__ __forceinline__ void ba_reduce_body(const BaDims& d, double* __restrict__ dw, const int* __restrict__ iw, BaState* __restrict__ states,
                                               int w, double* red) {
    const int tid = threadIdx.x;
    BaState* st = states + w;
    double* D = dw + (size_t)w * d.wstride;
    const int* I = iw + (size_t)w * d.istride;
    double maxd = 0;
    for (int i = tid; i < d.nfree * 27; i += BA_T) {
        const int kf = i / 27, c = i - kf * 27;
        const int nedges = I[d.oKfStart + d.nfixed + kf + 1] - I[d.oKfStart + d.nfixed + kf];
        const int nch = (nedges + BA_KFCH - 1) / BA_KFCH;
        double s = 0;
        for (int ch = 0; ch < nch; ch++) s += D[d.oPartKF + ((size_t)kf * d.kfChunks + ch) * 27 + c];
        if (c >= 21) D[d.oBp + kf * 6 + (c - 21)] = s;
        else {
            int a = 0, rem = c;
            while (rem >= 6 - a) { rem -= 6 - a; a++; }
            const int b = a + rem;
            D[d.oHpp + (size_t)kf * 36 + a * 6 + b] = s;
            D[d.oHpp + (size_t)kf * 36 + b * 6 + a] = s;
            if (a == b) maxd = fmax(maxd, fabs(s));
        }
    }
    const double mH = ba_block_max1(maxd, red);
    if (tid == 0) {
        double chi = 0, mL = 0;
        for (int b = 0; b < d.nblkP; b++) { chi += D[d.oPartP + (size_t)b * 4]; mL = fmax(mL, D[d.oPartP + (size_t)b * 4 + 1]); }
        st->currentChi = chi;
        if (st->iter == 0) { st->chi0 = chi; st->lambda = 1e-5 * fmax(mH, mL); st->ni = 2; }
        st->hq_fresh = st->iter > 0 ? 1 : 0;
        st->need_lin = 0;
    }
}

__global__ void __launch_bounds__(BA_T)
k_ba_reduce(BaDims d, double* __restrict__ dw, const int* __restrict__ iw, BaState* __restrict__ states) {
    __shared__ double red[4];
    const int w = blockIdx.x;
    if (states[w].status || !states[w].need_lin) return;
    ba_reduce_body(d, dw, iw, states, w, red);
}

__global__ void __launch_bounds__(BA_T)
k_ba_hinv(BaDims d, double* __restrict__ dw, const int* __restrict__ iw, BaState* __restrict__ states) {
    const int w = blockIdx.y, p = blockIdx.x * BA_T + threadIdx.x;
    const BaState st = states[w];
    if (st.status || st.hq_fresh || p >= d.npt) return;
    double* D = dw + (size_t)w * d.wstride;
    const int* I = iw + (size_t)w * d.istride;
    double ph[6], pb[3], X[3];
#pragma unroll
    for (int i = 0; i < 6; i++) ph[i] = D[d.oHll + (size_t)p * 6 + i];
#pragma unroll
    for (int i = 0; i < 3; i++) { pb[i] = D[d.oBl + (size_t)p * 3 + i]; X[i] = D[d.oP + ((size_t)st.cur * d.npt + p) * 3 + i]; }
    ba_write_rec(D + d.oHq + (size_t)I[d.oPtRank + p] * 12, ph, pb, X, st.lambda, states + w);
}

#define BA_MAXT 4
#define BA_REC 12
#define BA_RECS_LDS 256
#define BA_KMFMA 5
#define BA_ZERO_LDS 40
__device__ __forceinline__ void ba_wave_lds_fence() { __builtin_amdgcn_fence(__ATOMIC_SEQ_CST, "wavefront"); }

__host__ __device__ constexpr int ba_c_cap(int k) { return (BA_EMAX / k) < BA_PCAP ? (BA_EMAX / k) : BA_PCAP; }
__host__ __device__ constexpr int ba_c_nb(int k) { return (6 * k + 1 + 3) / 4; }
__host__ __device__ constexpr int ba_c_ld(int k) { return ((3 * ba_c_cap(k) + 3) / 4) * 4 + 2; }
__host__ __device__ constexpr int ba_c_tile(int k) { return 4 * ba_c_nb(k) * ba_c_ld(k); }
#define BA_CB 37
__host__ __device__ constexpr int ba_c_rhs(int k) { return BA_CB * (k * (k + 1) / 2); }
__host__ __device__ constexpr int ba_c_tri(int k) { return ba_c_rhs(k) + 6 * k; }
__host__ __device__ constexpr int ba_c_nacc(int k) {
    const int nb = ba_c_nb(k), nvf = nb / 4, rem = nb % 4;
    return 3 * nvf + 2 * nvf * (nvf - 1) + rem * (nvf + 1);
}
struct BaCTab { int cap[BA_SMALL_MAXF + 1], ld[BA_SMALL_MAXF + 1], nacc[BA_SMALL_MAXF + 1]; };
__host__ __device__ constexpr BaCTab ba_c_tab() {
    BaCTab t = {};
    for (int k = 1; k <= BA_SMALL_MAXF; k++) { t.cap[k] = ba_c_cap(k); t.ld[k] = ba_c_ld(k); t.nacc[k] = ba_c_nacc(k); }
    return t;
}
__device__ const BaCTab ba_ctab = ba_c_tab();
static int ba_c_wave_lds(int nfree) {
    int m = 0;
    for (int k = 1; k <= nfree; k++) m = std::max(m, std::max(ba_c_tile(k), k <= BA_KMFMA ? ba_c_tri(k) : 0));
    return ((m + 3) & ~3) + BA_RECS_LDS + BA_ZERO_LDS;
}

template <class IsZero>
__device__ __forceinline__ void ba_stable_split(int n, int* tmp, const int* src, int* dst, IsZero isZero) {
    const int wave = threadIdx.x >> 6, lane = threadIdx.x & 63;
    const int q = (((n + 3) >> 2) + 63) & ~63, lo = min(wave * q, n), hi = min(lo + q, n);
    int cnt = 0;
    for (int e = lo + lane; e < hi; e += 64) cnt += isZero(src[e]) ? 1 : 0;
    cnt = tb_wave_sum(cnt);
    if (lane == 0) tmp[wave] = cnt;
    __syncthreads();
    int z = 0;
    for (int v = 0; v < wave; v++) z += tmp[v];
    int o = (tmp[0] + tmp[1] + tmp[2] + tmp[3]) + (lo - z);
    const unsigned long long lt = (lane == 0) ? 0ull : (~0ull >> (64 - lane));
    for (int e0 = lo; e0 < hi; e0 += 64) {
        const int e = e0 + lane;
        const bool valid = e < hi;
        const int v = valid ? src[e] : 0;
        const bool f = valid && isZero(v);
        const unsigned long long m0 = __ballot(f), m1 = __ballot(valid && !f);
        if (valid) dst[f ? z + __popcll(m0 & lt) : o + __popcll(m1 & lt)] = v;
        z += __popcll(m0);
        o += __popcll(m1);
    }
    __threadfence_block();
    __syncthreads();
}

#define BA_RT 1024
#define BA_PREP_MAXKF 64
__global__ void __launch_bounds__(BA_RT)
k_ba_prepare(BaDims d, const tb_ba_obs* __restrict__ obsAll, const int32_t* __restrict__ obsCounts, int* __restrict__ iw,
             tb_ba_obs* __restrict__ obs2All) {
    extern __shared__ __attribute__((aligned(16))) unsigned prep_lds[];
    unsigned* word = prep_lds;
    int* first = reinterpret_cast<int*>(prep_lds + d.npt);
    int* start2 = first + d.npt;
    unsigned short* pbuf = reinterpret_cast<unsigned short*>(start2 + d.npt + 1);
    constexpr int NW = BA_RT / 64;
    __shared__ int tmp[NW + 2];
    __shared__ int bins[1 << BA_SMALL_MAXF];
    __shared__ int kfc[NW][BA_PREP_MAXKF];
    const int w = blockIdx.x, tid = threadIdx.x, wave = tid >> 6, lane = tid & 63;
    const unsigned long long lt = (lane == 0) ? 0ull : (~0ull >> (64 - lane));
    const tb_ba_obs* obs = obsAll + (size_t)w * d.obs_pitch;
    tb_ba_obs* obs2 = obs2All + (size_t)w * d.obs_pitch;
    const int nobs = min(max(obsCounts[w], 0), d.obs_pitch);
    int* I = iw + (size_t)w * d.istride;
    for (int p = tid; p < d.npt; p += BA_RT) { word[p] = 0; first[p] = 0; }
    for (int i = tid; i < (1 << BA_SMALL_MAXF); i += BA_RT) bins[i] = 0;
    __syncthreads();
    for (int e0 = tid; e0 < nobs; e0 += 4 * BA_RT) {
        tb_ba_obs o[4];
        int prev[4];
#pragma unroll
        for (int i = 0; i < 4; i++) {
            const int e = min(e0 + i * BA_RT, nobs - 1);
            o[i] = obs[e];
            prev[i] = obs[max(e - 1, 0)].pt;
        }
#pragma unroll
        for (int i = 0; i < 4; i++) {
            const int e = e0 + i * BA_RT;
            if (e >= nobs || (unsigned)o[i].pt >= (unsigned)d.npt || (unsigned)o[i].kf >= (unsigned)d.nkf) continue;
            atomicAdd(&word[o[i].pt], 0x10000u);
            if (o[i].kf >= d.nfixed) atomicOr(&word[o[i].pt], 1u << (o[i].kf - d.nfixed));
            if (e == 0 || prev[i] != o[i].pt) first[o[i].pt] = e;
        }
    }
    unsigned short* pa_ = pbuf;
    unsigned short* pb_ = pbuf + d.npt;
    for (int p = tid; p < d.npt; p += BA_RT) pa_[p] = (unsigned short)p;
    __syncthreads();
    {
        const int q = (((d.npt + NW - 1) / NW) + 63) & ~63, lo = min(wave * q, d.npt), hi = min(lo + q, d.npt);
        for (int b = 0; b < d.nfree; b++) {
            int cnt = 0;
            for (int e = lo + lane; e < hi; e += 64) cnt += ((word[pa_[e]] >> b) & 1) ? 0 : 1;
            cnt = tb_wave_sum(cnt);
            if (lane == 0) tmp[wave] = cnt;
            __syncthreads();
            int z = 0, all = 0;
            for (int v = 0; v < NW; v++) { const int c = tmp[v]; all += c; if (v < wave) z += c; }
            int o = all + (lo - z);
            for (int e0 = lo; e0 < hi; e0 += 64) {
                const int e = e0 + lane;
                const bool valid = e < hi;
                const int v = valid ? pa_[e] : 0;
                const bool f = valid && !((word[v] >> b) & 1);
                const unsigned long long m0 = __ballot(f), m1 = __ballot(valid && !f);
                if (valid) pb_[f ? z + __popcll(m0 & lt) : o + __popcll(m1 & lt)] = (unsigned short)v;
                z += __popcll(m0);
                o += __popcll(m1);
            }
            __syncthreads();
            unsigned short* t = pa_; pa_ = pb_; pb_ = t;
        }
    }
    for (int r = tid; r < d.npt; r += BA_RT) {
        const int p = pa_[r];
        I[d.oPerm + r] = p;
        I[d.oPtRank + r] = r;
        start2[r] = (int)(word[p] >> 16);
        pb_[p] = (unsigned short)r;
    }
    __syncthreads();
    const int total = tb_block_excl_scan(start2, d.npt, tmp);
    if (tid == 0) start2[d.npt] = total;
    __syncthreads();
    for (int r = tid; r <= d.npt; r += BA_RT) I[d.oPtStart + r] = start2[r];
    for (int e0 = tid; e0 < nobs; e0 += 4 * BA_RT) {
        tb_ba_obs o[4];
#pragma unroll
        for (int i = 0; i < 4; i++) o[i] = obs[min(e0 + i * BA_RT, nobs - 1)];
#pragma unroll
        for (int i = 0; i < 4; i++) {
            const int e = e0 + i * BA_RT;
            if (e >= nobs || (unsigned)o[i].pt >= (unsigned)d.npt || (unsigned)o[i].kf >= (unsigned)d.nkf) continue;
            const int r = pb_[o[i].pt], j = e - first[o[i].pt];
            if ((unsigned)j >= (word[o[i].pt] >> 16)) continue;
            o[i].pt = r;
            obs2[start2[r] + j] = o[i];
        }
    }
    __threadfence_block();
    __syncthreads();
    for (int r = tid; r < d.npt; r += BA_RT) {
        const unsigned m = word[pa_[r]] & 0xffffu;
        first[r] = __popc(m);
        if (m) atomicAdd(&bins[m], 1);
    }
    __syncthreads();
    for (int r = tid; r < d.npt; r += BA_RT) pb_[r] = (unsigned short)(word[pa_[r]] & 0xffffu);
    const int nfreeE = tb_block_excl_scan(first, d.npt, tmp);
    (void)nfreeE;
    unsigned short* mk = pb_;
    {
        const int q = (((total + NW - 1) / NW) + 63) & ~63, lo = min(wave * q, total), hi = min(lo + q, total);
        int cnt = 0;
        for (int e0 = lo; e0 < hi; e0 += 256) {
            int kf4[4];
#pragma unroll
            for (int u = 0; u < 4; u++) { const int e = e0 + 64 * u + lane; kf4[u] = (e < hi) ? obs2[e].kf : -1; }
#pragma unroll
            for (int u = 0; u < 4; u++)
                for (int k = 0; k < d.nkf; k++) {
                    const unsigned long long m = __ballot(kf4[u] == k);
                    if (lane == k) cnt += __popcll(m);
                }
        }
        if (lane < d.nkf) kfc[wave][lane] = cnt;
        __syncthreads();
        if (tid < d.nkf) {
            int base = 0;
            for (int k = 0; k < tid; k++)
                for (int v = 0; v < NW; v++) base += kfc[v][k];
            I[d.oKfStart + tid] = base;
            int run = base;
            for (int v = 0; v < NW; v++) run += kfc[v][tid];
            if (tid == d.nkf - 1) I[d.oKfStart + d.nkf] = run;
        }
        __syncthreads();
        if (tid < d.nkf) {
            int run = I[d.oKfStart + tid];
            for (int v = 0; v < NW; v++) { const int c = kfc[v][tid]; kfc[v][tid] = run; run += c; }
        }
        __syncthreads();
        int4* KR = reinterpret_cast<int4*>(I + d.oKfRec);
        for (int e00 = lo; e00 < hi; e00 += 256) {
            tb_ba_obs o4[4];
#pragma unroll
            for (int u = 0; u < 4; u++) {
                const int e = e00 + 64 * u + lane;
                o4[u].kf = -1; o4[u].pt = 0; o4[u].u = o4[u].v = o4[u].inv_sigma2 = 0.f;
                if (e < hi) o4[u] = obs2[e];
            }
#pragma unroll
            for (int u = 0; u < 4; u++) {
                const int e = e00 + 64 * u + lane;
                const tb_ba_obs o = o4[u];
                unsigned long long mine = 0;
                int add = 0;
                for (int k = 0; k < d.nkf; k++) {
                    const unsigned long long m = __ballot(o.kf == k);
                    if (o.kf == k) mine = m;
                    if (lane == k) add = __popcll(m);
                }
                if (o.kf >= 0 && o.kf < d.nkf) {
                    const int pos = kfc[wave][o.kf] + __popcll(mine & lt);
                    I[d.oKfEdges + pos] = e;
                    KR[pos] = make_int4(o.pt, __float_as_int(o.u), __float_as_int(o.v), __float_as_int(o.inv_sigma2));
                }
                ba_wave_lds_fence();
                if (lane < d.nkf) kfc[wave][lane] += add;
                ba_wave_lds_fence();
            }
        }
    }
    int4* KPs = reinterpret_cast<int4*>(I + d.oKPs);
    for (int r = tid; r < d.npt; r += BA_RT) {
        const int m = mk[r];
        if (m == 0) continue;
        const int base = first[r];
        for (int e = start2[r]; e < start2[r + 1]; e++) {
            const tb_ba_obs o = obs2[e];
            const int fk = o.kf - d.nfixed;
            if ((unsigned)fk >= (unsigned)d.nfree) continue;
            KPs[base + __popc(m & ((1 << fk) - 1))] = make_int4((int)(((unsigned)r << 6) | (unsigned)fk), __float_as_int(o.u), __float_as_int(o.v),
                                                                 __float_as_int(o.inv_sigma2));
        }
    }
    tb_block_excl_scan(bins, 1 << BA_SMALL_MAXF, tmp);
    int zero_pts = 0;
    {
        int c = 0;
        for (int r = tid; r < d.npt; r += BA_RT) c += (mk[r] == 0) ? 1 : 0;
        c = tb_wave_sum(c);
        __syncthreads();
        if (lane == 0) tmp[wave] = c;
        __syncthreads();
        for (int v = 0; v < NW; v++) zero_pts += tmp[v];
        __syncthreads();
    }
    auto pat_first = [&](int m) { return zero_pts + bins[m]; };
    auto pat_count = [&](int m) { return ((m + 1 < (1 << BA_SMALL_MAXF)) ? bins[m + 1] : d.npt - zero_pts) - bins[m]; };
    int* gflag = start2;
    __syncthreads();
    for (int r = tid; r < d.npt; r += BA_RT) {
        const int m = mk[r];
        gflag[r] = (m != 0 && (r - pat_first(m)) % ba_ctab.cap[__popc(m)] == 0) ? 1 : 0;
    }
    __syncthreads();
    const int ng = tb_block_excl_scan(gflag, d.npt, tmp);
    int4* GD = reinterpret_cast<int4*>(I + d.oGDesc);
    for (int r = tid; r < d.npt; r += BA_RT) {
        const int m = mk[r];
        if (m == 0) continue;
        const int k = __popc(m), at = r - pat_first(m);
        if (at % ba_ctab.cap[k] != 0) continue;
        GD[gflag[r]] = make_int4(r, first[r], m, min(ba_ctab.cap[k], pat_count(m) - at));
    }
    if (tid == 0) I[d.oGDesc + 4 * (size_t)d.npt] = ng;
    __threadfence_block();
    __syncthreads();
    int* GC = gflag;
    for (int g = tid; g < ng; g += BA_RT) {
        const int4 gd = GD[g];
        const int k = __popc(gd.z), nks = (3 * gd.w + 3) >> 2;
        GC[g] = 55 + ((k <= BA_KMFMA) ? nks * ba_ctab.nacc[k] : 12 * gd.w);
    }
    __syncthreads();
    const int cost = tb_block_excl_scan(GC, ng, tmp);
    if (tid == 0) GC[ng] = cost;
    __syncthreads();
    const int nwv = ba_schur_waves(d, w);
    for (int v = tid; v <= nwv; v += BA_RT) {
        const long long target = ((long long)cost * v + nwv - 1) / nwv;
        int lo = 0, hi = ng;
        while (lo < hi) {
            const int mid = (lo + hi) >> 1;
            if (GC[mid] < target) lo = mid + 1; else hi = mid;
        }
        I[d.oGCut + v] = (v == 0) ? 0 : (v == nwv) ? ng : lo;
    }
}

__global__ void __launch_bounds__(BA_T)
k_ba_groups(BaDims d, int* __restrict__ iw, const int* __restrict__ errflag) {
    __shared__ int cntb[1 << BA_SMALL_MAXF], bst[1 << BA_SMALL_MAXF], ebin[1 << BA_SMALL_MAXF], tmp[16];
    __shared__ unsigned short sortbuf[3 * BA_SORT_LDS];
    const int w = blockIdx.x, tid = threadIdx.x;
    if (errflag[w]) return;
    int* I = iw + (size_t)w * d.istride;
    const int4* KP = reinterpret_cast<const int4*>(I + d.oFreeKP);
    const int nbins = 1 << d.nfree;
    for (int i = tid; i < nbins; i += BA_T) cntb[i] = 0;
    __syncthreads();
    for (int p = tid; p < d.npt; p += BA_T) {
        const int e0 = I[d.oPtFree + p], e1 = I[d.oPtFree + p + 1];
// ... 921 lines not shown
    __shared__ int sgood;
    if (tid == 0) sgood = st->sing == 0;
    __syncthreads();
    for (int k0 = 0; k0 < np; k0 += BA_PB) {
        const int nb = min(BA_PB, np - k0), mr = np + 1 - k0;
        if (tid < 64) {
            const int r = tid;
            double dr[BA_PB];
#pragma unroll
            for (int c = 0; c < BA_PB; c++)
                dr[c] = (r < nb && c < nb) ? ((c <= r) ? A[(size_t)(k0 + r) * np + k0 + c] : 0.0) : ((c == r) ? 1.0 : 0.0);
            bool good = sgood != 0;
#pragma unroll
            for (int j = 0; j < BA_PB; j++) {
                const double dj = ba_readlane(dr[j], j);
                if (!(dj > 0) || !isfinite(dj)) good = false;
                const double sj = sqrt(good ? dj : 1.0), isj = 1.0 / sj;
                dr[j] = (r == j) ? sj : dr[j] * isj;
#pragma unroll
                for (int k = j + 1; k < BA_PB; k++) dr[k] -= dr[j] * ba_readlane(dr[j], k);
            }
            if (r < BA_PB) {
#pragma unroll
                for (int c = 0; c < BA_PB; c++) {
                    Ld[r * BA_PLD + c] = (c <= r) ? dr[c] : 0.0;
                    if (c == r) invd[r] = 1.0 / dr[c];
                    if (r < nb && c <= r) A[(size_t)(k0 + r) * np + k0 + c] = dr[c];
                }
            }
            if (r == 0) sgood = good ? 1 : 0;
        }
        __syncthreads();
        static_assert(BA_ST > 6 * BA_BIG_MAXF, "one thread per row below the diagonal block");
        if (const int r = nb + tid; r < mr) {
            double row[BA_PB];
            double* Ar = A + (size_t)(k0 + r) * np + k0;
#pragma unroll
            for (int c = 0; c < BA_PB; c++) {
                row[c] = Ar[c];
                asm volatile("" : "+v"(row[c]));
            }
#pragma unroll
            for (int c = 0; c < BA_PB; c++) row[c] = (c < nb) ? row[c] : 0.0;
#pragma unroll
            for (int c = 0; c < BA_PB; c++) {
                row[c] *= invd[c];
#pragma unroll
                for (int c2 = c + 1; c2 < BA_PB; c2++) row[c2] -= row[c] * Ld[c2 * BA_PLD + c];
#pragma unroll
                for (int c2 = c + 1; c2 < BA_PB; c2++) asm volatile("" : "+v"(row[c2]) : : "memory");
            }
#pragma unroll
            for (int c = 0; c < BA_PB; c++) {
                Pn[r * BA_PLD + c] = row[c];
                if (c < nb) Ar[c] = row[c];
            }
        }
        __syncthreads();
        const int mt = np - k0 - nb;
        if (mt > 0) {
            const int nT = (mt + 1 + 3) >> 2, last = mr - 1;
            for (int t = tid; t < nT * (nT + 1) / 2; t += BA_ST) {
                int ti = (int)((sqrt(8.0 * t + 1.0) - 1.0) * 0.5);
                while ((ti + 1) * (ti + 2) / 2 <= t) ti++;
                while (ti * (ti + 1) / 2 > t) ti--;
                const int tj = t - ti * (ti + 1) / 2;
                const int ra = nb + 4 * ti, rb = nb + 4 * tj;
                double acc[4][4] = {};
#pragma unroll 4
                for (int c = 0; c < BA_PB; c++) {
                    double av[4], bv[4];
#pragma unroll
                    for (int q = 0; q < 4; q++) { av[q] = Pn[min(ra + q, last) * BA_PLD + c]; bv[q] = Pn[min(rb + q, last) * BA_PLD + c]; }
#pragma unroll
                    for (int q = 0; q < 4; q++)
#pragma unroll
                        for (int s = 0; s < 4; s++) acc[q][s] = fma(av[q], bv[s], acc[q][s]);
                }
#pragma unroll
                for (int q = 0; q < 4; q++)
#pragma unroll
                    for (int s = 0; s < 4; s++) {
                        const int i = k0 + ra + q, j = k0 + rb + s;
                        if (i <= np && j < np && j <= i) A[(size_t)i * np + j] -= acc[q][s];
                    }
            }
        }
        __syncthreads();
    }
    for (int i = tid; i < np; i += BA_ST) xs[i] = A[(size_t)np * np + i];
    __syncthreads();
    for (int k0 = ((np - 1) / BA_PB) * BA_PB; k0 >= 0; k0 -= BA_PB) {
        const int nb = min(BA_PB, np - k0), mr = np - k0;
        for (int idx = tid; idx < mr * nb; idx += BA_ST) {
            const int r = idx / nb, c = idx - r * nb;
            Pn[r * BA_PLD + c] = (c <= r) ? A[(size_t)(k0 + r) * np + k0 + c] : 0.0;
        }
        __syncthreads();
        {
            const int c = tid & (BA_PB - 1), cls = tid >> 5;
            double s = 0;
            if (c < nb)
                for (int r = nb + cls; r < mr; r += BA_ST / BA_PB) s += Pn[r * BA_PLD + c] * xs[k0 + r];
            part[cls * BA_PB + c] = s;
        }
        __syncthreads();
        if (tid < 64) {
            const int c = tid;
            double t = 0;
            if (c < nb) {
                double s = 0;
                for (int k = 0; k < BA_ST / BA_PB; k++) s += part[k * BA_PB + c];
                t = xs[k0 + c] - s;
            }
            for (int j = nb - 1; j >= 0; j--) {
                const double xj = ba_readlane(t, j) / Pn[j * BA_PLD + j];
                if (c == j) t = xj;
                else if (c < j) t -= Pn[j * BA_PLD + c] * xj;
            }
            if (c < nb) xs[k0 + c] = t;
        }
        __syncthreads();
    }
    const bool good = sgood != 0;
    double term = 0;
    for (int i = tid; i < np; i += BA_ST) {
        const double xi = good ? xs[i] : 0.0;
        xs[i] = xi;
        D[d.oXp + i] = xi;
        term += xi * (lambda * xi + D[d.oBp + i]);
    }
    term = po_wave_sum(term);
    if ((tid & 63) == 0) red[tid >> 6] = term;
    __syncthreads();
    if (tid == 0) {
        double sc = 0;
        for (int k = 0; k < BA_ST / 64; k++) sc += red[k];
        st->scale_p = sc; st->ok2 = good ? 1 : 0;
    }
    __syncthreads();
    const double* T = D + d.oT + (size_t)st->cur * d.nkf * 7;
    double* Tn = D + d.oT + (size_t)(st->cur ^ 1) * d.nkf * 7;
    for (int k = tid; k < d.nkf; k += BA_ST) {
        const PoSE3 Tk = ba_load_se3(T + k * 7);
        if (k < d.nfixed) ba_store_se3(Tn + k * 7, Tk);
        else {
            double u[6];
            for (int a = 0; a < 6; a++) u[a] = xs[6 * (k - d.nfixed) + a];
            ba_store_se3(Tn + k * 7, po_exp_mul(u, Tk));
        }
    }
}

__global__ void __launch_bounds__(BA_T)
k_ba_update(BaDims d, const tb_ba_obs* __restrict__ obsAll, double* __restrict__ dw, const int* __restrict__ iw,
            const BaState* __restrict__ states) {
    __shared__ double red[4];
    extern __shared__ __attribute__((aligned(16))) double sdyn[];
    double* const sRt = sdyn;
    double* const sRtc = sdyn + (size_t)d.nkf * 12;
    double* const sx = sdyn + (size_t)d.nkf * 24;
    const int w = blockIdx.y, tid = threadIdx.x;
    const BaState st = states[w];
    if (st.status) return;
    const tb_ba_obs* obs = obsAll + (size_t)w * d.obs_pitch;
    double* D = dw + (size_t)w * d.wstride;
    const int* I = iw + (size_t)w * d.istride;
    const double* Tn = D + d.oT + (size_t)(st.cur ^ 1) * d.nkf * 7;
    for (int k = tid; k < d.nkf; k += BA_T) ba_pose_to_Rt(D + d.oT + ((size_t)st.cur * d.nkf + k) * 7, sRtc + k * 12);
    const double* P = D + d.oP + (size_t)st.cur * d.npt * 3;
    double* Pn = D + d.oP + (size_t)(st.cur ^ 1) * d.npt * 3;
    for (int k = tid; k < d.nkf; k += BA_T) ba_pose_to_Rt(Tn + k * 7, sRt + k * 12);
    for (int i = tid; i < d.np; i += BA_T) sx[i] = D[d.oXp + i];
    __syncthreads();
    const double delta = (double)sqrtf(5.991f);
    const int p = blockIdx.x * BA_T + tid;
    double chi = 0, sc = 0;
    if (p < d.npt) {
        const double* q = D + d.oHq + (size_t)I[d.oPtRank + p] * 12;
        double r[3] = {q[6], q[7], q[8]};
        const double bl[3] = {r[0], r[1], r[2]};
        double xl[3] = {0, 0, 0};
        const int eBeg = I[d.oPtStart + p], eEnd = I[d.oPtStart + p + 1];
        if (st.ok2) {
            const double u00 = q[0], u01 = q[1], u02 = q[2], u11 = q[3], u12 = q[4], u22 = q[5];
            const double Xc[3] = {P[3 * p], P[3 * p + 1], P[3 * p + 2]};
            tb_ba_obs on = obs[min(eBeg, d.obs_pitch - 1)];
            for (int e = eBeg; e < eEnd; e++) {
                const tb_ba_obs o = on;
                on = obs[min(e + 1, d.obs_pitch - 1)];
                if (o.kf < d.nfixed) continue;
                BaLin L;
                double Jp[12];
                ba_linearize(sRtc + o.kf * 12, Xc, o.u, o.v, o.inv_sigma2, d.fx, d.fy, d.cx, d.cy, delta, L);
                ba_jac_pose_iz(L.pc, L.invz, d.fx, d.fy, Jp);
                const double* xp = sx + 6 * (o.kf - d.nfixed);
                double s0 = 0, s1 = 0;
#pragma unroll
                for (int a = 0; a < 6; a++) { s0 = fma(Jp[a], xp[a], s0); s1 = fma(Jp[6 + a], xp[a], s1); }
#pragma unroll
                for (int c = 0; c < 3; c++) r[c] = fma(-L.ww, fma(L.Jl[c], s0, L.Jl[3 + c] * s1), r[c]);
            }
            const double t0 = u00 * r[0], t1 = u01 * r[0] + u11 * r[1], t2 = u02 * r[0] + u12 * r[1] + u22 * r[2];
            xl[0] = u00 * t0 + u01 * t1 + u02 * t2;
            xl[1] = u11 * t1 + u12 * t2;
            xl[2] = u22 * t2;
        }
        double X[3];
        for (int a = 0; a < 3; a++) {
            X[a] = P[3 * p + a] + xl[a];
            Pn[3 * p + a] = X[a];
            sc += xl[a] * (st.lambda * xl[a] + bl[a]);
        }
        tb_ba_obs on2 = obs[min(eBeg, d.obs_pitch - 1)];
        for (int e = eBeg; e < eEnd; e++) {
            const tb_ba_obs o = on2;
            on2 = obs[min(e + 1, d.obs_pitch - 1)];
            BaLin L;
            ba_residual(sRt + o.kf * 12, X, o.u, o.v, o.inv_sigma2, d.fx, d.fy, d.cx, d.cy, delta, L);
            chi += ba_huber_rho0(L.c2, delta);
        }
    }
    const double s1 = ba_block_sum1(chi, red);
    const double s2 = ba_block_sum1(sc, red);
    if (tid == 0) {
        D[d.oPartP + (size_t)blockIdx.x * 4 + 2] = s1;
        D[d.oPartP + (size_t)blockIdx.x * 4 + 3] = s2;
    }
}

__global__ void __launch_bounds__(64)
k_ba_decide(BaDims d, const double* __restrict__ dw, BaState* __restrict__ states, int* __restrict__ running) {
    const int w = blockIdx.x, lane = threadIdx.x;
    BaState* st = states + w;
    if (st->status) return;
    const double* D = dw + (size_t)w * d.wstride;
    double tc = 0, sc = 0;
    for (int b = lane; b < d.nblkP; b += 64) { tc += D[d.oPartP + (size_t)b * 4 + 2]; sc += D[d.oPartP + (size_t)b * 4 + 3]; }
    tc = po_wave_sum(tc);
    sc = po_wave_sum(sc);
    if (lane != 0) return;
    double tempChi = tc, scale = st->scale_p + sc;
    if (!st->ok2) tempChi = 1.7976931348623157e308;
    scale += 1e-3;
    const double rho = (st->currentChi - tempChi) / scale;
    if (rho > 0 && isfinite(tempChi)) {
        double alpha = 1. - pow(2 * rho - 1, 3);
        alpha = fmin(alpha, 2. / 3.);
        st->lambda *= fmax(1. / 3., alpha);
        st->ni = 2;
        st->currentChi = tempChi;
        st->cur ^= 1;
        st->need_lin = 1;
    } else {
        st->lambda *= st->ni;
        st->ni *= 2;
    }
    st->qmax++;
    st->rho = rho;
    st->sing = 0;
    st->hq_fresh = 0;
    if (!(rho < 0 && st->qmax < 10)) {
        st->done_iters++;
        const bool terminate = (st->qmax == 10 || rho == 0);
        st->iter++;
        st->qmax = 0;
        st->need_lin = 1;
        if (terminate || st->iter >= d.iters) st->status = 1;
    }
    if (!st->status) atomicAdd(running, 1);
}

__global__ void __launch_bounds__(BA_T)
k_ba_finish(BaDims d, const double* __restrict__ dw, const int* __restrict__ iw, const BaState* __restrict__ states,
            float* __restrict__ poses, float* __restrict__ pts, double* __restrict__ stats) {
    const int w = blockIdx.x, tid = threadIdx.x;
    const BaState st = states[w];
    const double* D = dw + (size_t)w * d.wstride;
    const int* I = iw + (size_t)w * d.istride;
    if (!st.err) {
        for (int k = tid; k < d.nkf; k += BA_T) {
            const PoSE3 s = ba_load_se3(D + d.oT + ((size_t)st.cur * d.nkf + k) * 7);
            double R[9];
            po_to_R(s, R);
            float* T = poses + ((size_t)w * d.nkf + k) * 16;
            for (int i = 0; i < 3; i++) { for (int j = 0; j < 3; j++) T[i * 4 + j] = (float)R[i * 3 + j]; }
            T[3] = (float)s.tx; T[7] = (float)s.ty; T[11] = (float)s.tz;
            T[12] = T[13] = T[14] = 0.f; T[15] = 1.f;
        }
        for (int i = tid; i < d.npt * 3; i += BA_T) {
            const int r = i / 3, c = i - 3 * r;
            pts[(size_t)w * d.npt * 3 + (d.renum ? 3 * (size_t)I[d.oPerm + r] + c : (size_t)i)] = (float)D[d.oP + (size_t)st.cur * d.npt * 3 + i];
        }
    }
    if (stats && tid == 0) {
        double* s = stats + 8 * w;
        s[0] = st.done_iters; s[1] = st.chi0; s[2] = st.currentChi; s[3] = st.lambda;
        s[4] = st.rho; s[5] = st.iter; s[6] = 0; s[7] = st.err ? -1.0 : 0.0;
    }
}

__global__ void k_ba_zero(int* __restrict__ p, int n) {
    const int i = blockIdx.x * blockDim.x + threadIdx.x;
    if (i < n) p[i] = 0;
}

static void ba_dims(BaDims& d, int num_cu, int peers, int W, const double K[4], int nkf, int nfixed, int npt, int obs_pitch, int iters) {
    memset(&d, 0, sizeof d);
    d.W = W; d.nkf = nkf; d.nfixed = nfixed; d.nfree = nkf - nfixed; d.np = 6 * d.nfree; d.npt = npt; d.obs_pitch = obs_pitch;
    d.iters = iters;
    d.nblkP = (npt + BA_T - 1) / BA_T;
    d.kfChunks = (obs_pitch + BA_KFCH - 1) / BA_KFCH;
    d.nChunks = 0;
    {
        const int slots = std::max(2 * std::max(num_cu, 1) / std::max(peers, 1), 1), cap = std::min(32, std::max((npt / 64 + 3) / 4, 1));
        d.Gbase = std::min(std::max(slots / std::max(W, 1), 1), cap);
        d.Gextra = (d.Gbase < cap && slots > d.Gbase * W) ? std::min(slots - d.Gbase * W, W) : 0;
        d.G = d.Gbase + (d.Gextra > 0 ? 1 : 0);
        d.wgReduce = d.Gbase > 4 ? 1 : 0;
        const int T = 4 * std::max(slots, W);
        d.Vbase = std::min(T / std::max(W, 1), 4 * cap);
        d.Vextra = d.Vbase < 4 * cap ? T % std::max(W, 1) : 0;
    }
    d.big = d.nfree > BA_SMALL_MAXF;
    d.renum = (!d.big && npt <= BA_SORT_LDS && nkf <= BA_PREP_MAXKF) ? 1 : 0;
    d.schurWaveLds = d.big ? 0 : ba_c_wave_lds(d.nfree);
    d.npairs = d.nfree * (d.nfree + 1) / 2;
    d.maxItems = (unsigned long long)obs_pitch * (d.nfree + 1) / 2 + 1;
    d.fx = K[0]; d.fy = K[1]; d.cx = K[2]; d.cy = K[3];
    unsigned long long o = 0;
    auto take = [&](unsigned long long n) { unsigned long long r = o; o += (n + 1) & ~1ull; return r; };
    d.oT = take(2ull * nkf * 7);
    d.oP = take(2ull * npt * 3);
    d.oHll = take(6ull * npt);
    d.oBl = take(3ull * npt);
    d.oHq = take(12ull * npt);
    d.oHpp = take(36ull * std::max(d.nfree, 1));
    d.oBp = take(std::max(64, d.np));
    d.oXp = take(std::max(64, d.np));
    d.oPartKF = take(27ull * std::max(d.nfree, 1) * d.kfChunks);
    d.oPartP = take(4ull * d.nblkP);
    const int maxWaves = d.wgReduce ? 4 * d.G : d.Vbase + (d.Vextra > 0 ? 1 : 0);
    d.oPartS = take(d.big ? 0 : 4096ull * (d.wgReduce ? d.G : maxWaves));
    d.oBigA = take(d.big ? (unsigned long long)(d.np + 1) * d.np + 32 : 0);
    d.wstride = o;
    unsigned long long io = 0;
    auto itake = [&](unsigned long long n) { unsigned long long r = io; io += (n + 3) & ~3ull; return r; };
    d.oPtStart = itake(npt + 1);
    d.oPtFree = itake(npt + 1);
    d.oKfStart = itake(nkf + 1);
    d.oKfEdges = itake(obs_pitch);
    d.oFreeKP = itake(4ull * obs_pitch);
    d.oKfRec = itake(4ull * obs_pitch);
    d.oPtRank = itake(npt);
    d.oPerm = itake(d.renum ? npt : 0);
    d.oPtMask = itake(d.big ? 0 : npt);
    d.oPermA = itake(d.big ? 0 : npt);
    d.oPermB = itake(d.big ? 0 : npt);
    d.oKPs = itake(d.big ? 0 : 4ull * obs_pitch);
    d.oGDesc = itake(d.big ? 0 : 4ull * npt + 4);
    d.oGCost = itake(d.big ? 0 : (unsigned long long)npt + 1);
    d.oGCut = itake(d.big ? 0 : (unsigned long long)maxWaves + 1);
    d.oPairStart = itake(d.big ? d.npairs + 1 : 0);
    d.oPairCnt = itake(d.big ? d.npairs : 0);
    d.oPairItems = itake(d.big ? 2 * d.maxItems : 0);
    d.istride = io;
}

size_t tbk_local_ba_work_bytes(const tb_ctx* ctx, int W, int nkf, int nfixed, int npt, int obs_pitch) {
    BaDims d;
    const double K[4] = {1, 1, 0, 0};
    ba_dims(d, ctx->num_cu, ctx->peers, W, K, nkf, nfixed, npt, obs_pitch, 1);
    return (size_t)W * (d.wstride * sizeof(double) + d.istride * sizeof(int) + sizeof(BaState) + sizeof(int)) + 4096 +
           (d.renum ? (size_t)W * obs_pitch * sizeof(tb_ba_obs) + 64 : 0);
}

int tbk_local_ba_batch(tb_ctx* ctx, int W, const double K[4], int nkf, int nfixed, float* d_poses, int npt, float* d_pts,
                       const tb_ba_obs* d_obs, const int32_t* d_counts, int obs_pitch, int iters, double* d_stats, void* d_work,
                       size_t work_bytes) {
    if (W <= 0) return TB_OK;
    const int nfree = nkf - nfixed;
    if (nfree < 1 || nfree > BA_BIG_MAXF)
        return tb_fail(ctx, TB_EUNSUPPORTED, "local BA: %d free keyframes (this build supports 1..64)", nfree);
    if (nkf > TB_MAX_LEVELS * 8) return tb_fail(ctx, TB_EUNSUPPORTED, "local BA: too many keyframes");
    if (npt > (1 << 25)) return tb_fail(ctx, TB_EUNSUPPORTED, "local BA: more than 2^25 points per window");
    if (nfree > BA_SMALL_MAXF && (unsigned long long)obs_pitch * (nfree + 1) >= (1ull << 31))
        return tb_fail(ctx, TB_EUNSUPPORTED, "local BA: large window with more than 2^31 / (free keyframes + 1) observations");
    if (iters > 99) return tb_fail(ctx, TB_EUNSUPPORTED, "local BA: more than 99 LM iterations (one still-running counter per trial, 1000 of them)");
    BaDims d;
    ba_dims(d, ctx->num_cu, ctx->peers, W, K, nkf, nfixed, npt, obs_pitch, iters);
    if (tbk_local_ba_work_bytes(ctx, W, nkf, nfixed, npt, obs_pitch) > work_bytes) return tb_fail(ctx, TB_ENOMEM, "local BA workspace too small");
    char* base = (char*)d_work;
    double* dw = (double*)base;
    int* iw = (int*)(base + (size_t)W * d.wstride * sizeof(double));
    BaState* states = (BaState*)((char*)iw + (size_t)W * d.istride * sizeof(int));
    int* running = (int*)((char*)states + (size_t)W * sizeof(BaState));
    hipStream_t s = ctx->stream;
    const size_t schur_lds = std::max<size_t>(4 * (size_t)d.schurWaveLds, d.wgReduce ? 64 * 64 : 0) * sizeof(double);
    const int ring = 1000;
    int* errflag = running + ring;
    tb_ba_obs* obs2 = (tb_ba_obs*)(((uintptr_t)(errflag + W) + 63) & ~(uintptr_t)63);
    const tb_ba_obs* d_obs_in = d_obs;
    if (d.renum) d_obs = obs2;
    const size_t big_lds = (size_t)(d.np + 1) * BA_PLD * sizeof(double);
    const int R = (d.np + 15) >> 4;
    typedef void (*schur_t)(BaDims, double*, const int*, BaState*);
    const schur_t ks = R == 1 ? (schur_t)k_ba_schur_c<1> : R == 2 ? (schur_t)k_ba_schur_c<2> : R == 3 ? (schur_t)k_ba_schur_c<3> : (schur_t)k_ba_schur_c<4>;
    if (!d.big) TB_HIP(ctx, hipFuncSetAttribute((const void*)ks, hipFuncAttributeMaxDynamicSharedMemorySize, (int)schur_lds));
    if (d.renum) TB_HIP(ctx, hipFuncSetAttribute((const void*)k_ba_prepare, hipFuncAttributeMaxDynamicSharedMemorySize, npt * 16 + 16));
    else TB_HIP(ctx, hipFuncSetAttribute((const void*)k_ba_solve_big, hipFuncAttributeMaxDynamicSharedMemorySize, (int)big_lds));
    auto enqueue_head = [&]() -> int {
        hipLaunchKernelGGL(k_ba_zero, dim3((ring + W + 255) / 256), dim3(256), 0, s, running, ring + W);
        if (d.renum) {
            tb_prof_begin(ctx, "k_ba_prepare");
            hipLaunchKernelGGL(k_ba_prepare, dim3(W), dim3(BA_RT), (size_t)npt * 16 + 16, s, d, d_obs_in, d_counts, iw, obs2);
            tb_prof_end(ctx);
        }
        tb_prof_begin(ctx, "k_ba_setup");
        hipLaunchKernelGGL(k_ba_setup, dim3(nkf + 2, W), dim3(BA_T), 0, s, d, d_poses, d_pts, d_obs_in, d_obs, d_counts, dw, iw, states, errflag);
        tb_prof_end(ctx);
        if (d.renum) {
        } else if (!d.big) {
            tb_prof_begin(ctx, "k_ba_groups");
            hipLaunchKernelGGL(k_ba_groups, dim3(W), dim3(BA_T), 0, s, d, iw, errflag);
            tb_prof_end(ctx);
        } else {
            tb_prof_begin(ctx, "k_ba_pairs");
            hipLaunchKernelGGL(k_ba_pairs<false>, dim3(d.nfree, W), dim3(64), 0, s, d, d_obs, iw, errflag);
            hipLaunchKernelGGL(k_ba_pair_scan, dim3(W), dim3(BA_T), 0, s, d, iw, errflag);
            hipLaunchKernelGGL(k_ba_pairs<true>, dim3(d.nfree, W), dim3(64), 0, s, d, d_obs, iw, errflag);
            tb_prof_end(ctx);
        }
        TB_HIP(ctx, hipGetLastError());
        return TB_OK;
    };
    auto enqueue_round = [&](int round) -> int {
        {
            const int nKfBlocks = ((W + 7) / 8) * 8 * std::min(BA_KFBLK, d.kfChunks) * d.nfree;
            if (W <= 32) {
                tb_prof_begin(ctx, "k_ba_lin");
                hipLaunchKernelGGL(k_ba_lin, dim3(nKfBlocks + d.nblkP * W), dim3(BA_T), (size_t)d.nkf * 12 * sizeof(double), s, d, d_obs, dw, iw, states,
                                   errflag, nKfBlocks);
                tb_prof_end(ctx);
            } else {
                tb_prof_begin(ctx, "k_ba_points");
                hipLaunchKernelGGL(k_ba_points, dim3(d.nblkP, W), dim3(BA_T), (size_t)d.nkf * 12 * sizeof(double), s, d, d_obs, dw, iw, states, errflag);
                tb_prof_end(ctx);
                tb_prof_begin(ctx, "k_ba_kf");
                hipLaunchKernelGGL(k_ba_kf, dim3(nKfBlocks), dim3(BA_T), 0, s, d, d_obs, dw, iw, states, errflag);
                tb_prof_end(ctx);
            }
        }
        const bool reduce_in_solve = !d.big && round > 0;
        if (!reduce_in_solve) {
            tb_prof_begin(ctx, "k_ba_reduce");
            hipLaunchKernelGGL(k_ba_reduce, dim3(W), dim3(BA_T), 0, s, d, dw, iw, states);
            tb_prof_end(ctx);
        }
        if (round == 0) {
            tb_prof_begin(ctx, "k_ba_hinv");
            hipLaunchKernelGGL(k_ba_hinv, dim3(d.nblkP, W), dim3(BA_T), 0, s, d, dw, iw, states);
            tb_prof_end(ctx);
        }
        if (d.big) {
            tb_prof_begin(ctx, "k_ba_schur_pairs");
            hipLaunchKernelGGL(k_ba_schur_pairs, dim3((d.npairs + 3) / 4, W), dim3(BA_T), 0, s, d, dw, iw, states);
            tb_prof_end(ctx);
            tb_prof_begin(ctx, "k_ba_solve_big");
            hipLaunchKernelGGL(k_ba_solve_big, dim3(W), dim3(BA_ST), big_lds, s, d, dw, states);
            tb_prof_end(ctx);
        } else {
            tb_prof_begin(ctx, "k_ba_schur");
            hipLaunchKernelGGL(ks, dim3(d.wgReduce ? d.Gbase * W + d.Gextra : (d.Vbase * W + d.Vextra + 3) / 4), dim3(BA_T), schur_lds, s, d, dw, iw, states);
            tb_prof_end(ctx);
            tb_prof_begin(ctx, "k_ba_solve");
            if (d.np <= 16) hipLaunchKernelGGL(k_ba_solve<16>, dim3(W), dim3(BA_SOLVE_T), 0, s, d, dw, iw, states, reduce_in_solve ? 1 : 0);
            else if (d.np <= 32) hipLaunchKernelGGL(k_ba_solve<32>, dim3(W), dim3(BA_SOLVE_T), 0, s, d, dw, iw, states, reduce_in_solve ? 1 : 0);
            else if (d.np <= 48) hipLaunchKernelGGL(k_ba_solve<48>, dim3(W), dim3(BA_SOLVE_T), 0, s, d, dw, iw, states, reduce_in_solve ? 1 : 0);
            else hipLaunchKernelGGL(k_ba_solve<64>, dim3(W), dim3(BA_SOLVE_T), 0, s, d, dw, iw, states, reduce_in_solve ? 1 : 0);
            tb_prof_end(ctx);
        }
        tb_prof_begin(ctx, "k_ba_update");
        hipLaunchKernelGGL(k_ba_update, dim3(d.nblkP, W), dim3(BA_T), ((size_t)d.nkf * 24 + d.np) * sizeof(double), s, d, d_obs, dw, iw, states);
        tb_prof_end(ctx);
        tb_prof_begin(ctx, "k_ba_decide");
        hipLaunchKernelGGL(k_ba_decide, dim3(W), dim3(64), 0, s, d, dw, states, running + round % ring);
        tb_prof_end(ctx);
        TB_HIP(ctx, hipGetLastError());
        return TB_OK;
    };
    int host_running = 1, rounds = 0, rc = TB_OK;
    const int max_rounds = std::min(iters * 10 + 1, 1000);
    int batch = iters;
    const bool use_graph = W <= 32 && !ctx->prof && std::min(batch, max_rounds) > 0;
    if (use_graph) {
        struct Key { BaDims d; const void *poses, *pts, *obs, *counts, *work; hipStream_t s; } key;
        memset(&key, 0, sizeof key);
        key.d = d; key.poses = d_poses; key.pts = d_pts; key.obs = d_obs_in; key.counts = d_counts; key.work = d_work; key.s = s;
        const std::string kb((const char*)&key, sizeof key);
        hipGraphExec_t exec = nullptr;
        for (auto& g : ctx->ba_graphs)
            if (g.first == kb) exec = g.second;
        const int nfirst = std::min(batch, max_rounds);
        if (!exec) {
            static std::mutex capture_lock;
            std::lock_guard<std::mutex> guard(capture_lock);
            hipGraph_t graph = nullptr;
            TB_HIP(ctx, hipStreamBeginCapture(s, hipStreamCaptureModeThreadLocal));
            rc = enqueue_head();
            for (int r = 0; r < nfirst && rc == TB_OK; r++) rc = enqueue_round(r);
            const hipError_t e = hipStreamEndCapture(s, &graph);
            if (rc != TB_OK) { if (graph) hipGraphDestroy(graph); return rc; }
            TB_HIP(ctx, e);
            const hipError_t e2 = hipGraphInstantiate(&exec, graph, nullptr, nullptr, 0);
            hipGraphDestroy(graph);
            TB_HIP(ctx, e2);
            if (ctx->ba_graphs.size() >= 8) {
                hipGraphExecDestroy(ctx->ba_graphs.front().second);
                ctx->ba_graphs.erase(ctx->ba_graphs.begin());
            }
            ctx->ba_graphs.emplace_back(kb, exec);
        }
        TB_HIP(ctx, hipGraphLaunch(exec, s));
        rounds = nfirst;
    } else if ((rc = enqueue_head()) != TB_OK) return rc;
    bool replayed = use_graph;
    while (host_running > 0 && (rounds < max_rounds || replayed)) {
        if (!replayed)
            for (int r = 0; r < batch && rounds < max_rounds; r++, rounds++)
                if ((rc = enqueue_round(rounds)) != TB_OK) return rc;
        replayed = false;
        TB_HIP(ctx, hipMemcpyAsync(&host_running, running + (rounds - 1) % ring, sizeof(int), hipMemcpyDeviceToHost, s));
        TB_HIP(ctx, hipStreamSynchronize(s));
        batch = 4;
    }
    tb_prof_begin(ctx, "k_ba_finish");
    hipLaunchKernelGGL(k_ba_finish, dim3(W), dim3(BA_T), 0, s, d, dw, iw, states, d_poses, d_pts, d_stats);
    tb_prof_end(ctx);
    TB_HIP(ctx, hipGetLastError());
    return TB_OK;
}
```

### trackingbench_slam_amd/csrc/tb_capi.cpp

```cpp
#include "tb_internal.h"
#include "tb_math.h"

#include <stdarg.h>
#include <string.h>
#include <algorithm>
#include <cfloat>
#include <climits>
#include <cmath>
#include <memory>

int tb_fail(tb_ctx* ctx, int code, const char* fmt, ...) {
    char buf[512];
    va_list ap;
    va_start(ap, fmt);
    vsnprintf(buf, sizeof buf, fmt, ap);
    va_end(ap);
    if (ctx) ctx->err = buf;
    return code;
}

int tb_scratch(tb_ctx* ctx, int slot, size_t bytes, void** out) {
    if (bytes < 256) bytes = 256;
    if (ctx->scratch_cap[slot] < bytes) {
        if (ctx->scratch[slot]) {
// ... 9 lines not shown
    *out = ctx->scratch[slot];
    return TB_OK;
}

static hipEvent_t prof_event(tb_ctx* ctx) {
    if (!ctx->prof_pool.empty()) { hipEvent_t e = ctx->prof_pool.back(); ctx->prof_pool.pop_back(); return e; }
    hipEvent_t e = nullptr;
    hipEventCreate(&e);
    return e;
}
void tb_prof_begin(tb_ctx* ctx, const char* name) {
    ctx->prof_open = false;
    if (!ctx->prof) return;
    if (!ctx->prof_only.empty() && ctx->prof_only != name) return;
    ctx->prof_open = true;
    tb_ctx::ProfRec r;
    r.name = name;
    r.a = prof_event(ctx);
    r.b = prof_event(ctx);
    hipEventRecord(r.a, ctx->stream);
    ctx->prof_recs.push_back(r);
}
void tb_prof_end(tb_ctx* ctx) {
    if (!ctx->prof || !ctx->prof_open || ctx->prof_recs.empty()) return;
    hipEventRecord(ctx->prof_recs.back().b, ctx->stream);
    ctx->prof_open = false;
}
static void prof_drain(tb_ctx* ctx) {
    hipStreamSynchronize(ctx->stream);
    for (auto& r : ctx->prof_recs) {
        float ms = 0.f;
        if (hipEventElapsedTime(&ms, r.a, r.b) == hipSuccess) {
            auto& acc = ctx->prof_acc[r.name];
            acc.first += 1;
            acc.second += ms;
        }
        ctx->prof_pool.push_back(r.a);
        ctx->prof_pool.push_back(r.b);
    }
    ctx->prof_recs.clear();
}

extern "C" {

int tb_profile_enable(tb_ctx* ctx, int on) {
    TB_ENTER(ctx);
    if (!ctx) return TB_EINVAL;
    prof_drain(ctx);
    ctx->prof_acc.clear();
    ctx->prof = on != 0;
    return TB_OK;
}

int tb_profile_only(tb_ctx* ctx, const char* kernel) {
    TB_ENTER(ctx);
    if (!ctx) return TB_EINVAL;
    ctx->prof_only = kernel ? kernel : "";
    return TB_OK;
}

int tb_profile_report(tb_ctx* ctx, char* buf, int cap) {
    TB_ENTER(ctx);
    if (!ctx || !buf || cap < 1) return TB_EINVAL;
    prof_drain(ctx);
    std::string out;
    char line[256];
    for (auto& kv : ctx->prof_acc) {
        snprintf(line, sizeof line, "%s %ld %.6f\n", kv.first.c_str(), kv.second.first, kv.second.second);
        out += line;
    }
    if ((int)out.size() + 1 > cap) return tb_fail(ctx, TB_ECAPACITY, "profile report needs %d bytes", (int)out.size() + 1);
    memcpy(buf, out.c_str(), out.size() + 1);
    return TB_OK;
}

const char* tb_version(void) { return "trackingbench-slam_amd 0.1 (gfx950)"; }

const char* tb_strerror(int code) {
    switch (code) {
        case TB_OK: return "ok";
        case TB_EINVAL: return "invalid argument";
        case TB_ENOMEM: return "out of memory";
        case TB_ECAPACITY: return "output capacity too small";
        case TB_EUNSUPPORTED: return "unsupported input (reference behaviour undefined)";
        case TB_EDEVICE: return "HIP device error";
        case TB_ESTATE: return "call sequence error";
        default: return "unknown error";
    }
}

int tb_create(int device, tb_ctx** out) {
    if (!out) return TB_EINVAL;
    *out = nullptr;
    int ndev = 0;
    if (hipGetDeviceCount(&ndev) != hipSuccess || ndev <= 0) return TB_EDEVICE;
    if (device < 0 || device >= ndev) return TB_EINVAL;
    if (hipSetDevice(device) != hipSuccess) return TB_EDEVICE;
    tb_ctx* ctx = new (std::nothrow) tb_ctx();
    if (!ctx) return TB_ENOMEM;
    ctx->device = device;
    {
        int ncu = 0;
        if (hipDeviceGetAttribute(&ncu, hipDeviceAttributeMultiprocessorCount, device) == hipSuccess && ncu > 0) ctx->num_cu = ncu;
    }
    if (hipStreamCreateWithFlags(&ctx->own_stream, hipStreamNonBlocking) != hipSuccess) {
        delete ctx;
        return TB_EDEVICE;
    }
    ctx->stream = ctx->own_stream;
    *out = ctx;
    return TB_OK;
}

int tb_measure_copy_seconds(tb_ctx* ctx, const void* d_src, void* d_dst, size_t bytes, int reps, double* seconds) {
    TB_ENTER(ctx);
    if (!ctx || !d_src || !d_dst || !seconds || reps < 1 || bytes < 16 || (bytes & 15) || ((uintptr_t)d_src & 15) || ((uintptr_t)d_dst & 15))
        return TB_EINVAL;
    hipEvent_t e0, e1;
    TB_HIP(ctx, hipEventCreate(&e0));
    TB_HIP(ctx, hipEventCreate(&e1));
    int rc = tbk_copy16(ctx, d_src, d_dst, bytes);
    if (rc == TB_OK) {
        hipError_t e = hipEventRecord(e0, ctx->stream);
        for (int i = 0; i < reps && rc == TB_OK; i++) rc = tbk_copy16(ctx, d_src, d_dst, bytes);
        if (e == hipSuccess) e = hipEventRecord(e1, ctx->stream);
        if (e == hipSuccess) e = hipEventSynchronize(e1);
        float ms = 0;
        if (e == hipSuccess) e = hipEventElapsedTime(&ms, e0, e1);
        if (e != hipSuccess && rc == TB_OK) rc = tb_fail(ctx, TB_EDEVICE, "tb_measure_copy_seconds: %s", hipGetErrorString(e));
        *seconds = (double)ms * 1e-3 / reps;
    }
    hipEventDestroy(e0);
    hipEventDestroy(e1);
    return rc;
}

int tb_pack_rows_dev(tb_ctx* ctx, const void* src, int row_bytes, int cap, const int32_t* counts, int nframes, void* dst, long long* total) {
    TB_ENTER(ctx);
    if (!ctx || nframes < 0 || cap < 1 || row_bytes < 4 || (row_bytes & 3)) return TB_EINVAL;
    if (nframes == 0) return TB_OK;
    if (!src || !dst || !counts || src == dst) return TB_EINVAL;
    return tbk_pack_rows(ctx, src, row_bytes, cap, counts, nframes, dst, total);
}

int tb_set_concurrency(tb_ctx* ctx, int peers) {
    if (!ctx || peers < 1) return TB_EINVAL;
    ctx->peers = peers;
    return TB_OK;
}

int tb_debug_force_dense_fast(tb_ctx* ctx, int on) {
    if (!ctx) return TB_EINVAL;
    ctx->dbg_fast_dense = on ? 1 : 0;
    return TB_OK;
}

void tb_destroy(tb_ctx* ctx) {
    if (!ctx) return;
    hipSetDevice(ctx->device);
    hipStreamSynchronize(ctx->stream);
    ctx->plans.clear();
    while (!ctx->live.empty()) tb_extractor_destroy(*ctx->live.begin());
    for (int i = 0; i < TB_NSLOTS; i++)
        if (ctx->scratch[i]) hipFree(ctx->scratch[i]);
    for (auto& g : ctx->ba_graphs) hipGraphExecDestroy(g.second);
    prof_drain(ctx);
    for (hipEvent_t e : ctx->prof_pool) hipEventDestroy(e);
    if (ctx->own_stream) hipStreamDestroy(ctx->own_stream);
    delete ctx;
}

const char* tb_last_error(const tb_ctx* ctx) { return ctx ? ctx->err.c_str() : "null context"; }

int tb_set_stream(tb_ctx* ctx, void* hip_stream) {
    TB_ENTER(ctx);
    if (!ctx) return TB_EINVAL;
    TB_HIP(ctx, hipStreamSynchronize(ctx->stream));
    ctx->stream = hip_stream ? (hipStream_t)hip_stream : ctx->own_stream;
    return TB_OK;
}

int tb_synchronize(tb_ctx* ctx) {
    TB_ENTER(ctx);
    if (!ctx) return TB_EINVAL;
    TB_HIP(ctx, hipStreamSynchronize(ctx->stream));
    return TB_OK;
}

int tb_scale_factors(int n, float scale, float* sf, float* inv_sf, float* sigma2, float* inv_sigma2) {
    if (n < 1 || !sf) return TB_EINVAL;
    float cur = 1.f, icur = 1.f;
    for (int i = 0; i < n; i++) {
        if (i > 0) { cur = cur * scale; icur = icur / scale; }
        sf[i] = cur;
        if (inv_sf) inv_sf[i] = icur;
        const float s2 = (i == 0) ? 1.f : cur * cur;
        if (sigma2) sigma2[i] = s2;
        if (inv_sigma2) inv_sigma2[i] = (i == 0) ? 1.f : 1.f / s2;
    }
    return TB_OK;
}

int tb_pyramid_sizes(int width, int height, int nlevels, const float* sf, int* widths, int* heights) {
    if (nlevels < 1 || !sf || !widths || !heights) return TB_EINVAL;
    widths[0] = width;
    heights[0] = height;
    for (int i = 1; i < nlevels; i++) {
        widths[i] = (int)((float)width * sf[i]);
        heights[i] = (int)((float)height * sf[i]);
    }
    return TB_OK;
}

int tb_orb_quotas(int nlevels, const float* sf, int target, int* quotas) {
    if (nlevels < 2 || !sf || !quotas) return TB_EINVAL;
    float nDesired = target * (1 - sf[1]) / (1 - (float)pow((double)sf[1], (double)nlevels));
    int sum = 0;
    for (int level = 0; level < nlevels - 1; level++) {
        quotas[level] = tbm::cv_round(nDesired);
        sum += quotas[level];
        nDesired *= sf[1];
    }
    quotas[nlevels - 1] = std::max(target - sum, 0);
    return TB_OK;
}

static void build_resize_tables(int sw, int sh, int dw, int dh, std::vector<ResizeX>& rx, std::vector<ResizeY>& ry) {
    const double inv_scale_x = (double)dw / sw, inv_scale_y = (double)dh / sh;
    const double scale_x = 1. / inv_scale_x, scale_y = 1. / inv_scale_y;
    rx.resize(dw);
    ry.resize(dh);
    for (int dx = 0; dx < dw; dx++) {
        float fx = (float)((dx + 0.5) * scale_x - 0.5);
        int sx = tbm::cv_floor(fx);
        fx -= sx;
        if (sx < 0) { fx = 0; sx = 0; }
        if (sx >= sw - 1) { fx = 0; sx = sw - 1; }
        rx[dx].sx = (int16_t)sx;
        rx[dx].sx1 = (int16_t)std::min(sx + 1, sw - 1);
        rx[dx].a0 = (int16_t)tbm::cv_round((1.f - fx) * 2048.f);
        rx[dx].a1 = (int16_t)tbm::cv_round(fx * 2048.f);
    }
    for (int dy = 0; dy < dh; dy++) {
        float fy = (float)((dy + 0.5) * scale_y - 0.5);
        int sy = tbm::cv_floor(fy);
        fy -= sy;
        ry[dy].sy0 = std::min(std::max(sy, 0), sh - 1);
        ry[dy].sy1 = std::min(std::max(sy + 1, 0), sh - 1);
        ry[dy].b0 = (int16_t)tbm::cv_round((1.f - fy) * 2048.f);
        ry[dy].b1 = (int16_t)tbm::cv_round(fy * 2048.f);
    }
}

static int fastgrid_ncell(int width, int height, int target) {
    const int cell = (int)sqrtf((float)width * (float)height / (float)target);
    if (cell < 1) return 0;
    const int cols = (int)((float)width / (float)cell), rows = (int)((float)height / (float)cell);
    return std::max((rows + 2) * (cols + 1), target);
}

void tb_extractor_destroy(tb_extractor* ex) {
    if (!ex) return;
    ex->ctx->live.erase(ex);
    for (auto it = ex->ctx->plans.begin(); it != ex->ctx->plans.end();)
        it = (it->second == ex) ? ex->ctx->plans.erase(it) : std::next(it);
    hipSetDevice(ex->ctx->device);
    hipStreamSynchronize(ex->ctx->stream);
    hipFree(ex->d_slab); hipFree(ex->d_img0_copy); hipFree(ex->d_blocks);
    for (int l = 0; l < TB_MAX_LEVELS; l++) { hipFree(ex->d_rx[l]); hipFree(ex->d_ry[l]); }
    hipFree(ex->d_cand); hipFree(ex->d_candCount); hipFree(ex->d_knode); hipFree(ex->d_sel); hipFree(ex->d_selCount);
    hipFree(ex->d_kps); hipFree(ex->d_desc); hipFree(ex->d_counts); hipFree(ex->d_exit); hipFree(ex->d_enode);
    hipFree(ex->d_gridBest); hipFree(ex->d_occ);
    delete ex;
}

int tb_extractor_create(tb_ctx* ctx, int width, int height, int nlevels, const float* sf, const int* widths,
                        const int* heights, int max_images, int max_target, tb_extractor** out) {
    TB_ENTER(ctx);
    if (!ctx || !out) return TB_EINVAL;
    *out = nullptr;
    if (width < 1 || height < 1 || nlevels < 1 || nlevels > TB_MAX_LEVELS || !sf || max_images < 1 || max_target < 1)
        return tb_fail(ctx, TB_EINVAL, "extractor_create: bad geometry %dx%d levels=%d images=%d target=%d", width, height,
                       nlevels, max_images, max_target);
    if (width > 4095 || height > 4095) return tb_fail(ctx, TB_EUNSUPPORTED, "images larger than 4095 px are not supported");
    TB_HIP(ctx, hipSetDevice(ctx->device));
    std::unique_ptr<tb_extractor> exu(new tb_extractor());
    tb_extractor* ex = exu.get();
    ex->ctx = ctx;
    ex->max_images = max_images;
    ex->max_target = max_target;
    ex->sf.assign(sf, sf + nlevels);
    for (int l = 0; l < TB_MAX_LEVELS; l++) { ex->d_rx[l] = nullptr; ex->d_ry[l] = nullptr; ex->quotas[l] = 0; }
    PlanGeom& g = ex->g;
    memset(&g, 0, sizeof g);
    g.nlevels = nlevels;
    g.width = width;
    g.height = height;
    std::vector<int> ws(nlevels), hs(nlevels);
    if (widths && heights) {
        for (int l = 0; l < nlevels; l++) { ws[l] = widths[l]; hs[l] = heights[l]; }
        if (ws[0] != width || hs[0] != height) return tb_fail(ctx, TB_EINVAL, "level 0 size mismatch");
    } else {
        tb_pyramid_sizes(width, height, nlevels, sf, ws.data(), hs.data());
    }
    int maxq[TB_MAX_LEVELS] = {0};
    if (nlevels >= 2) tb_orb_quotas(nlevels, sf, max_target, maxq);
// ... 352 lines not shown
    for (int i = 0; i < c; i++) {
        out[i].x = keyed[i].second & 0xfff;
        out[i].y = (keyed[i].second >> 12) & 0xfff;
        out[i].score = keyed[i].second >> 24;
    }
    return TB_OK;
}

static size_t stage_piece(size_t& end, size_t bytes) {
    const size_t o = end;
    end += (bytes + 15) & ~(size_t)15;
    return o;
}

#define TB_UPLOAD(ctx, dst, src, bytes) \
    do { if (bytes) TB_HIP(ctx, hipMemcpyAsync((dst), (src), (bytes), hipMemcpyHostToDevice, (ctx)->stream)); } while (0)
#define TB_DOWNLOAD(ctx, dst, src, bytes) \
    do { if (bytes) TB_HIP(ctx, hipMemcpyAsync((dst), (src), (bytes), hipMemcpyDeviceToHost, (ctx)->stream)); } while (0)

static int get_plan(tb_ctx* ctx, const char* tag, int nlevels, const float* sf, const int* ws, const int* hs, int max_target,
                    tb_extractor** out) {
    std::string key = tag;
    char buf[64];
    for (int l = 0; l < nlevels; l++) {
        snprintf(buf, sizeof buf, ":%dx%d:%08x", ws[l], hs[l], *reinterpret_cast<const uint32_t*>(&sf[l]));
        key += buf;
    }
    auto it = ctx->plans.find(key);
    if (it != ctx->plans.end() && it->second->max_target >= max_target) { *out = it->second; return TB_OK; }
    if (it != ctx->plans.end()) tb_extractor_destroy(it->second);
    tb_extractor* ex = nullptr;
    int rc = tb_extractor_create(ctx, ws[0], hs[0], nlevels, sf, ws, hs, 1, std::max(max_target, 2048), &ex);
    if (rc) return rc;
    ctx->plans[key] = ex;
    *out = ex;
    return TB_OK;
}

int tb_pyramid(tb_ctx* ctx, const uint8_t* image, int width, int height, int stride, int nlevels, const float* sf,
               uint8_t* const* levels_out, const int* strides_out) {
    TB_ENTER(ctx);
    if (!ctx || !image || !sf || !levels_out || !strides_out || nlevels < 1 || nlevels > TB_MAX_LEVELS) return TB_EINVAL;
    std::vector<int> ws(nlevels), hs(nlevels);
    tb_pyramid_sizes(width, height, nlevels, sf, ws.data(), hs.data());
    tb_extractor* ex = nullptr;
    int rc = get_plan(ctx, "pyr", nlevels, sf, ws.data(), hs.data(), 1, &ex);
    if (rc) return rc;
    rc = tb_extractor_set_images_host(ex, image, 1, stride, 0);
    if (rc) return rc;
    rc = tb_extractor_build_pyramid(ex, 1);
    if (rc) return rc;
    for (int l = 1; l < nlevels; l++) {
        if (!levels_out[l]) continue;
        rc = tb_extractor_get_level_host(ex, 0, l, levels_out[l], strides_out[l]);
        if (rc) return rc;
    }
    return tb_synchronize(ctx);
}

int tb_fast_detect(tb_ctx* ctx, const uint8_t* image, int width, int height, int stride, int threshold, int nms,
                   tb_corner* out, int cap, int* count) {
    TB_ENTER(ctx);
    if (!ctx || !image || !count || width < 0 || height < 0 || width > 4095 || height > 4095) return TB_EINVAL;
    *count = 0;
    if (width < 7 || height < 7) return TB_OK;
    threshold = std::min(std::max(threshold, 0), 255);
    const int rcap = (nms ? ((width + 1) / 2) * ((height + 1) / 2) : width * height) + 64;
    size_t end = 0;
    const size_t oImg = stage_piece(end, (size_t)width * height), oOut = stage_piece(end, (size_t)rcap * 4), oCnt = stage_piece(end, 4);
    char* b;
    int rc;
    if ((rc = tb_scratch(ctx, TB_SLOT_HOST, end, (void**)&b))) return rc;
    TB_HIP(ctx, hipMemcpy2DAsync(b + oImg, width, image, stride, width, height, hipMemcpyHostToDevice, ctx->stream));
    rc = tbk_fast_image(ctx, (const uint8_t*)(b + oImg), width, height, width, threshold, nms, 9, (uint32_t*)(b + oOut), rcap,
                        (int32_t*)(b + oCnt));
    if (rc) return rc;
    int32_t c = 0;
    TB_DOWNLOAD(ctx, &c, b + oCnt, 4);
    TB_HIP(ctx, hipStreamSynchronize(ctx->stream));
    *count = c;
    if (c > cap || c > rcap) return tb_fail(ctx, TB_ECAPACITY, "fast_detect: %d corners, capacity %d", c, cap);
    std::vector<uint32_t> rec((size_t)c);
    if (c > 0) {
        TB_HIP(ctx, hipMemcpy(rec.data(), b + oOut, (size_t)c * 4, hipMemcpyDeviceToHost));
        std::sort(rec.begin(), rec.end(), [](uint32_t a, uint32_t b) { return (a & 0xffffff) < (b & 0xffffff); });
    }
    for (int i = 0; i < c && out; i++) {
        out[i].x = rec[i] & 0xfff;
        out[i].y = (rec[i] >> 12) & 0xfff;
        out[i].score = rec[i] >> 24;
    }
    return TB_OK;
}

int tb_orb_extract(tb_ctx* ctx, const uint8_t* const* levels, const int* widths, const int* heights, const int* strides,
                   int nlevels, const float* sf, int target, float init_th, float min_th, const tb_keypoint* exit_keys,
                   int n_exit, int use_quotas, int* quotas_inout, tb_keypoint* kps, uint8_t* desc, int cap, int* count) {
    TB_ENTER(ctx);
    if (!ctx || !levels || !widths || !heights || !strides || !sf || !quotas_inout || !count || nlevels < 1 ||
        nlevels > TB_MAX_LEVELS)
        return TB_EINVAL;
    *count = 0;
    if (!levels[0] || widths[0] < 1 || heights[0] < 1) return TB_OK;
    if (nlevels < 2) return tb_fail(ctx, TB_EUNSUPPORTED, "ORB extraction reads sf[1]: needs >= 2 levels");
    int qsum = 0;
    if (use_quotas) for (int l = 0; l < nlevels; l++) qsum += quotas_inout[l];
    tb_extractor* ex = nullptr;
    int rc = get_plan(ctx, "orb", nlevels, sf, widths, heights, std::max(target, qsum), &ex);
    if (rc) return rc;
    rc = tb_extractor_set_levels_host(ex, 0, levels, strides);
    if (rc) return rc;
    if (use_quotas) {
        for (int l = 0; l < nlevels; l++) ex->quotas[l] = quotas_inout[l];
        ex->have_quotas = true;
    }
    rc = tb_extractor_orb(ex, 1, target, init_th, min_th, use_quotas ? 1 : 0, exit_keys, n_exit);
    if (rc) return rc;
    if (!use_quotas) for (int l = 0; l < nlevels; l++) quotas_inout[l] = ex->quotas[l];
    return tb_extractor_results_host(ex, 0, kps, desc, cap, count);
}

int tb_fastgrid_extract(tb_ctx* ctx, const uint8_t* const* levels, const int* widths, const int* heights, const int* strides,
                        int nlevels, const float* inv_sf, int target, float threshold, const uint8_t* occupancy,
                        int n_occupancy, tb_keypoint* kps, int cap, int* count) {
    TB_ENTER(ctx);
    if (!ctx || !levels || !widths || !heights || !strides || !inv_sf || !count || nlevels < 1 || nlevels > TB_MAX_LEVELS ||
        target < 1)
        return TB_EINVAL;
    *count = 0;
    if (!levels[0] || widths[0] < 1 || heights[0] < 1) return TB_OK;
    std::vector<float> sf(nlevels);
    for (int l = 0; l < nlevels; l++) sf[l] = 1.f / inv_sf[l];
    tb_extractor* ex = nullptr;
    int rc = get_plan(ctx, "fg", nlevels, sf.data(), widths, heights, target, &ex);
    if (rc) return rc;
    rc = tb_extractor_set_levels_host(ex, 0, levels, strides);
    if (rc) return rc;
    rc = tb_extractor_fastgrid(ex, 1, inv_sf, target, threshold, occupancy, n_occupancy);
    if (rc) return rc;
    return tb_extractor_results_host(ex, 0, kps, nullptr, cap, count);
}

int tb_descriptor_distance(const uint8_t* a, const uint8_t* b) {
    int dist = 0;
    for (int i = 0; i < 4; i++) {
        uint64_t x, y;
        memcpy(&x, a + 8 * i, 8);
        memcpy(&y, b + 8 * i, 8);
        dist += __builtin_popcountll(x ^ y);
    }
    return dist;
}

void tb_three_maxima(const int* sizes, int L, int* ind1, int* ind2, int* ind3) {
    tbm::three_maxima(sizes, L, ind1, ind2, ind3);
}

static int match_tail(tb_ctx* ctx, const tb_match* dout, const int32_t* dcf, int cap, tb_match* out, int* count) {
    int32_t cf[2] = {0, 0};
    TB_HIP(ctx, hipMemcpyAsync(cf, dcf, sizeof cf, hipMemcpyDeviceToHost, ctx->stream));
    TB_HIP(ctx, hipStreamSynchronize(ctx->stream));
    if (cf[1] == 1) return tb_fail(ctx, TB_EINVAL, "searchByProjection: a key octave is outside the scale factors");
    if (cf[1] == 2) return tb_fail(ctx, TB_EUNSUPPORTED, "rotation bin outside histogram (reference asserts)");
    *count = cf[0];
    if (cf[0] > cap) return tb_fail(ctx, TB_ECAPACITY, "matches: %d, capacity %d", cf[0], cap);
    if (cf[0] > 0 && out) TB_HIP(ctx, hipMemcpy(out, dout, (size_t)cf[0] * sizeof(tb_match), hipMemcpyDeviceToHost));
    return TB_OK;
}

static int bf_host(tb_ctx* ctx, const uint8_t* d1, int n1, const uint8_t* d2, int n2, int crosscheck, int filter, float ratio,
                   float min_th, tb_match* out, int cap, int* count) {
    if (!ctx || !count || n1 < 0 || n2 < 0 || (n1 && !d1) || (n2 && !d2)) return TB_EINVAL;
    *count = 0;
    if (n1 == 0 || n2 == 0) return TB_OK;
    const int max_n = std::max(n1, n2);
    const size_t pitch = (size_t)max_n * 32;
    size_t end = 0;
    const size_t oD1 = stage_piece(end, pitch), oD2 = stage_piece(end, pitch), oTb = stage_piece(end, (size_t)max_n * 8),
                 oQb = stage_piece(end, (size_t)max_n * 8), oOut = stage_piece(end, (size_t)n1 * sizeof(tb_match)), oCnt = stage_piece(end, 16);
    char* b;
    int rc;
    if ((rc = tb_scratch(ctx, TB_SLOT_HOST, end, (void**)&b))) return rc;
    const int32_t cnt[4] = {n1, n2, 0, 0};
    int32_t* dcnt = (int32_t*)(b + oCnt);
    TB_UPLOAD(ctx, b + oD1, d1, (size_t)n1 * 32);
    TB_UPLOAD(ctx, b + oD2, d2, (size_t)n2 * 32);
    TB_UPLOAD(ctx, dcnt, cnt, sizeof cnt);
    if ((rc = tbk_bf_batch(ctx, 1, (const uint8_t*)(b + oD1), dcnt, (const uint8_t*)(b + oD2), dcnt + 1, pitch, max_n, crosscheck, filter,
                           ratio, min_th, (tb_match*)(b + oOut), n1, dcnt + 2, (unsigned long long*)(b + oTb), (unsigned long long*)(b + oQb))))
        return rc;
    return match_tail(ctx, (const tb_match*)(b + oOut), dcnt + 2, cap, out, count);
}

int tb_match_bf(tb_ctx* ctx, const uint8_t* d1, int n1, const uint8_t* d2, int n2, int crosscheck, tb_match* out, int cap,
                int* count) {
    TB_ENTER(ctx);
    return bf_host(ctx, d1, n1, d2, n2, crosscheck, 0, 0.f, 0.f, out, cap, count);
}

int tb_search_by_bf(tb_ctx* ctx, const uint8_t* d1, int n1, const uint8_t* d2, int n2, float ratio, float min_th,
                    tb_match* out, int cap, int* count) {
    TB_ENTER(ctx);
    return bf_host(ctx, d1, n1, d2, n2, 1, 1, ratio, min_th, out, cap, count);
}

int tb_search_by_bf_batch_dev(tb_ctx* ctx, int npairs, const uint8_t* desc1, const int32_t* counts1, const uint8_t* desc2,
                              const int32_t* counts2, size_t set_pitch, float ratio, float min_th, tb_match* out, int cap,
                              int32_t* out_counts) {
    TB_ENTER(ctx);
    if (!ctx || npairs < 0 || !desc1 || !desc2 || !counts1 || !counts2 || !out || !out_counts || set_pitch < 32 || cap < 1)
        return TB_EINVAL;
    if (npairs == 0) return TB_OK;
    const int max_n = (int)(set_pitch / 32);
    void *tb, *qb;
    int rc;
    if ((rc = tb_scratch(ctx, TB_SLOT_BF_TRAIN, (size_t)npairs * max_n * 8, &tb))) return rc;
    if ((rc = tb_scratch(ctx, TB_SLOT_BF_QUERY, (size_t)npairs * max_n * 8, &qb))) return rc;
    return tbk_bf_batch(ctx, npairs, desc1, counts1, desc2, counts2, set_pitch, max_n, 1, 1, ratio, min_th, out, cap, out_counts,
                        (unsigned long long*)tb, (unsigned long long*)qb);
}

#define TB_LSH_MAX_N 8192

static bool lsh_params_ok(int tables, int key_size, int probe) {
    return tables >= 1 && tables <= 32 && key_size >= 1 && key_size <= 32 && probe >= 0 && probe <= key_size;
}

int tb_lsh_draw_bits(int tables, int key_size, uint64_t seed, uint16_t* out) {
    if (!out || tables < 1 || tables > 32 || key_size < 1 || key_size > 32) return TB_EINVAL;
    uint16_t pool[256];
    int have = 0, at = 0;
    uint64_t word = 0;
    for (int t = 0; t < tables; t++) {
        if (have < key_size) {
            for (int i = 0; i < 256; i++) pool[i] = (uint16_t)i;
            for (int i = 255; i >= 1; i--) {
                uint64_t z = seed + (++word) * 0x9E3779B97F4A7C15ull;
                z = (z ^ (z >> 30)) * 0xBF58476D1CE4E5B9ull;
                z = (z ^ (z >> 27)) * 0x94D049BB133111EBull;
                z = z ^ (z >> 31);
                const int j = (int)(z % (uint64_t)(i + 1));
                std::swap(pool[i], pool[j]);
            }
            have = 256; at = 0;
        }
        for (int b = 0; b < key_size; b++) out[(size_t)t * key_size + b] = pool[at + b];
        at += key_size; have -= key_size;
    }
    return TB_OK;
}

int tb_lsh_create(tb_ctx* ctx, int tables, int key_size, int multi_probe_level, uint64_t seed, const uint16_t* bits, tb_lsh** out) {
    TB_ENTER(ctx);
    if (out) *out = nullptr;
    if (!ctx || !out) return TB_EINVAL;
    if (!lsh_params_ok(tables, key_size, multi_probe_level))
        return tb_fail(ctx, TB_EINVAL, "tb_lsh_create: tables %d (1..32), key_size %d (1..32), multi_probe_level %d (0..key_size)", tables,
                       key_size, multi_probe_level);
    std::unique_ptr<tb_lsh, void (*)(tb_lsh*)> h(new tb_lsh(), tb_lsh_destroy);
    h->ctx = ctx; h->T = tables; h->k = key_size; h->L = multi_probe_level;
    h->bits.resize((size_t)tables * key_size);
    if (bits) {
        for (int t = 0; t < tables; t++) {
            bool seen[256] = {};
            for (int b = 0; b < key_size; b++) {
                const uint16_t v = bits[(size_t)t * key_size + b];
                if (v > 255 || seen[v]) return tb_fail(ctx, TB_EINVAL, "tb_lsh_create: bit %d of table %d is %d (0..255, once per table)", b, t, (int)v);
                seen[v] = true;
            }
        }
        std::copy(bits, bits + h->bits.size(), h->bits.begin());
    } else {
        tb_lsh_draw_bits(tables, key_size, seed, h->bits.data());
    }
    std::vector<uint8_t> b8(h->bits.begin(), h->bits.end());
    TB_HIP(ctx, hipMalloc((void**)&h->d_bits, b8.size()));
    TB_HIP(ctx, hipMemcpy(h->d_bits, b8.data(), b8.size(), hipMemcpyHostToDevice));
    *out = h.release();
    return TB_OK;
}

void tb_lsh_destroy(tb_lsh* lsh) {
    if (!lsh) return;
    if (lsh->ctx) hipSetDevice(lsh->ctx->device);
    hipFree(lsh->d_bits);
    delete lsh;
}

int tb_lsh_info(const tb_lsh* lsh, int* tables, int* key_size, int* multi_probe_level, uint16_t* bits) {
    if (!lsh) return TB_EINVAL;
    if (tables) *tables = lsh->T;
    if (key_size) *key_size = lsh->k;
    if (multi_probe_level) *multi_probe_level = lsh->L;
    if (bits) std::copy(lsh->bits.begin(), lsh->bits.end(), bits);
    return TB_OK;
}

static int lsh_host(tb_ctx* ctx, const tb_lsh* lsh, const uint8_t* d1, int n1, const uint8_t* d2, int n2, int filter, float ratio,
                    float min_th, tb_match* out, int cap, int* count) {
    if (!ctx || !lsh || lsh->ctx != ctx || !count || n1 < 0 || n2 < 0 || (n1 && !d1) || (n2 && !d2)) return TB_EINVAL;
    *count = 0;
    if (n1 > TB_LSH_MAX_N || n2 > TB_LSH_MAX_N) return tb_fail(ctx, TB_EINVAL, "searchByNN: sets of %d / %d descriptors (at most %d)", n1, n2, TB_LSH_MAX_N);
    if (n1 == 0 || n2 == 0) return TB_OK;
    const int max_n = std::max(n1, n2);
    const size_t pitch = (size_t)max_n * 32;
    size_t end = 0;
// ... 1269 lines not shown
```

### trackingbench_slam_amd/csrc/tb_internal.h

```cpp
#ifndef TB_INTERNAL_H
#define TB_INTERNAL_H

#include <hip/hip_runtime.h>
#include <stdint.h>
#include <stdio.h>
#include <map>
#include <set>
#include <string>
#include <vector>

#include "../../include/tb_capi.h"

#define TB_MAX_LEVELS 16
#define TB_BORDER 16
#define TB_NODE_CAP_MAX 2048
#define TB_GRID_CELLS (120 * 36)
#define TB_GRID_STARTS (TB_GRID_CELLS + 1)

enum {
    TB_SLOT_HOST = 0,
    TB_SLOT_BF_TRAIN = 1,
    TB_SLOT_BF_QUERY = 2,
    TB_SLOT_BOW_NODES = 3,
    TB_SLOT_STEREO_SIGMA = 3,
    TB_SLOT_BOW_WEIGHTS = 4,
    TB_SLOT_OPFLOW_EQ = 4,
    TB_SLOT_WORK = 5,
    TB_SLOT_LK = 6,
    TB_SLOT_RANSAC = 7,
    TB_SLOT_RANSAC_FLAGS = 8,
    TB_SLOT_STEREO_MATCHES = 9,
    TB_SLOT_STEREO_COUNTS = 10,
    TB_NSLOTS = 11
};

struct tb_ctx {
    int device = 0;
    int num_cu = 256;
    std::vector<std::pair<std::string, hipGraphExec_t>> ba_graphs;
    int peers = 1;
    int dbg_fast_dense = 0;
    hipStream_t own_stream = nullptr;
    hipStream_t stream = nullptr;
    std::string err;
    std::map<std::string, tb_extractor*> plans;
    std::set<tb_extractor*> live;
    bool prof = false;
    bool prof_open = false;
    std::string prof_only;
    struct ProfRec { const char* name; hipEvent_t a, b; };
    std::vector<ProfRec> prof_recs;
    std::vector<hipEvent_t> prof_pool;
    std::map<std::string, std::pair<long, double>> prof_acc;
    void* scratch[TB_NSLOTS] = {};
    size_t scratch_cap[TB_NSLOTS] = {};
};

int tb_fail(tb_ctx* ctx, int code, const char* fmt, ...);
void tb_prof_begin(tb_ctx* ctx, const char* name);
void tb_prof_end(tb_ctx* ctx);
int tb_scratch(tb_ctx* ctx, int slot, size_t bytes, void** out);

#define TB_HIP(ctx, call)                                                                     \
    do {                                                                                      \
        hipError_t e_ = (call);                                                               \
        if (e_ != hipSuccess)                                                                 \
            return tb_fail((ctx), TB_EDEVICE, "%s: %s (%s:%d)", #call, hipGetErrorString(e_), \
                           __FILE__, __LINE__);                                               \
    } while (0)

#define TB_TRY(call)            \
    do {                        \
        int rc_ = (call);       \
        if (rc_) return rc_;    \
    } while (0)

struct tb_dev_owner {
    std::vector<void*> ptrs;
    void release() {
        for (void* p : ptrs) hipFree(p);
        ptrs.clear();
    }
};

template <class T>
static int tb_dev_alloc(tb_ctx* ctx, tb_dev_owner& own, T** out, size_t count, int fill = -1) {
    void* p = nullptr;
    hipError_t e = hipMalloc(&p, count * sizeof(T));
    if (e == hipSuccess) {
        own.ptrs.push_back(p);
        *out = static_cast<T*>(p);
        if (fill >= 0) e = hipMemsetAsync(p, fill, count * sizeof(T), ctx->stream);
    }
    if (e != hipSuccess) return tb_fail(ctx, TB_EDEVICE, "device buffer of %zu x %zu bytes: %s", count, sizeof(T), hipGetErrorString(e));
    return TB_OK;
}

#define TB_ENTER(ctx)                                                                          \
    do {                                                                                       \
        tb_ctx* c_ = (ctx);                                                                    \
        if (c_) {                                                                              \
            hipError_t e_ = hipSetDevice(c_->device);                                          \
            if (e_ != hipSuccess) {  \
                c_->err = std::string("hipSetDevice: ") + hipGetErrorString(e_);               \
                return TB_EDEVICE;                                                             \
            }                                                                                  \
        }                                                                                      \
    } while (0)

struct LevelGeom {
    int w, h, stride;
    int nCols, nRows;
    int wCell, hCell;
    int cellBase;
    int nCells;
    int candCap;
    int nodeCap;
    int nodeCapAlloc;
    int nIni;
    int quota;
    int selBase;
    float hX;
    float patchSize;
    float sf;
    float inv_sf;
    unsigned long long off;
    unsigned long long candOff;
};

struct PlanGeom {
    int nlevels;
    int width, height;
    int selCap;
    unsigned long long slabBytes;
    unsigned long long candPerImage;
    const uint8_t* img0;
    unsigned long long img0_pitch;
    int img0_stride;
    int pad_;
    LevelGeom lv[TB_MAX_LEVELS];
};

struct FastBlock {
    int16_t level;
    int16_t ncx, ncy;
    int16_t sA;
    int16_t x0, y0, x1, y1;
    int16_t nss, rowsPer;
    int16_t nPass;
    uint16_t invNss;
};
#define FB_S 160
#ifndef FB_TH
#define FB_TH 68
#endif
#define FB_MAX_CX 4
#ifndef FB_MAX_CY
#define FB_MAX_CY 2
#endif

struct ResizeX { int16_t sx, sx1, a0, a1; };
struct ResizeY { int32_t sy0, sy1; int16_t b0, b1; };

struct tb_extractor {
    tb_ctx* ctx = nullptr;
    PlanGeom g;
    int max_images = 0, max_target = 0;
    std::vector<float> sf;
    bool have_quotas = false;
    int quotas[TB_MAX_LEVELS];
    int last_n = 0;
    bool last_was_orb = false;
    uint8_t* d_slab = nullptr;
    uint8_t* d_img0_copy = nullptr;
    FastBlock* d_blocks = nullptr; int nBlocksTotal = 0;
    ResizeX* d_rx[TB_MAX_LEVELS]; ResizeY* d_ry[TB_MAX_LEVELS];
    uint32_t* d_cand = nullptr;
    int32_t* d_candCount = nullptr;
    uint32_t* d_knode = nullptr;
    uint32_t* d_sel = nullptr;
    int32_t* d_selCount = nullptr;
    tb_keypoint* d_kps = nullptr;
    uint8_t* d_desc = nullptr;
    int32_t* d_counts = nullptr;
    float* d_exit = nullptr; int exitCap = 0;
    int32_t* d_enode = nullptr; size_t enodeCap = 0;
    unsigned long long* d_gridBest = nullptr; size_t gridBestCap = 0;
    uint8_t* d_occ = nullptr; size_t occCap = 0;
};

struct tb_vocab {
    tb_ctx* ctx = nullptr;
    int nnodes = 0, k = 0, L = 0, weighting = 0, scoring = 0;
    int32_t *d_child_start = nullptr, *d_child_items = nullptr, *d_word_id = nullptr;
// ... 223 lines not shown
```

### trackingbench_slam_amd/csrc/tb_math.h

```cpp
#ifndef TB_MATH_H
#define TB_MATH_H

#include <stdint.h>
#include <math.h>
#include <string.h>

#if defined(__HIPCC__)
#include <hip/hip_runtime.h>
#define TB_HD __host__ __device__ inline
#else
#define TB_HD inline
#endif

#if defined(__clang__)
#pragma clang fp contract(off)
#endif

namespace tbm {

#if defined(__HIP_DEVICE_COMPILE__)
#define TB_FMUL(a, b) __fmul_rn((a), (b))
#define TB_FADD(a, b) __fadd_rn((a), (b))
#define TB_FSUB(a, b) __fsub_rn((a), (b))
#define TB_DMUL(a, b) __dmul_rn((a), (b))
#define TB_DADD(a, b) __dadd_rn((a), (b))
#define TB_DSUB(a, b) __dsub_rn((a), (b))
#define TB_FDIV(a, b) __fdiv_rn((a), (b))
#else
#define TB_FMUL(a, b) ((a) * (b))
#define TB_FADD(a, b) ((a) + (b))
#define TB_FSUB(a, b) ((a) - (b))
#define TB_DMUL(a, b) ((a) * (b))
#define TB_DADD(a, b) ((a) + (b))
#define TB_DSUB(a, b) ((a) - (b))
#define TB_FDIV(a, b) ((a) / (b))
#endif

TB_HD int cv_round(float v) {
#if defined(__HIP_DEVICE_COMPILE__)
    return __float2int_rn(v);
#else
    return (int)nearbyintf(v);
#endif
}
TB_HD int cv_round(double v) {
#if defined(__HIP_DEVICE_COMPILE__)
    return __double2int_rn(v);
#else
    return (int)nearbyint(v);
#endif
}
TB_HD int cv_floor(float v) { int i = (int)v; return i - (i > v); }
TB_HD int cv_floor(double v) { int i = (int)v; return i - (i > v); }

TB_HD uint32_t abstop12(float x) {
#if defined(__HIP_DEVICE_COMPILE__)
    return (__float_as_uint(x) >> 20) & 0x7ff;
#else
    uint32_t u;
    memcpy(&u, &x, 4);
    return (u >> 20) & 0x7ff;
#endif
}

#define TB_SC_HPI_INV 0x1.45F306DC9C883p+23
#define TB_SC_HPI 0x1.921FB54442D18p0
#define TB_SC_C1 (-0x1.ffffffd0c621cp-2)
#define TB_SC_C2 0x1.55553e1068f19p-5
#define TB_SC_C3 (-0x1.6c087e89a359dp-10)
#define TB_SC_C4 0x1.99343027bf8c3p-16
#define TB_SC_S1 (-0x1.555545995a603p-3)
#define TB_SC_S2 0x1.1107605230bc4p-7
#define TB_SC_S3 (-0x1.994eb3774cf24p-13)

TB_HD float sincos_poly(double x, double x2, double csgn, int n) {
    if ((n & 1) == 0) {
        double x3 = TB_DMUL(x, x2);
        double s1 = TB_DADD(TB_SC_S2, TB_DMUL(x2, TB_SC_S3));
        double x7 = TB_DMUL(x3, x2);
        double s = TB_DADD(x, TB_DMUL(x3, TB_SC_S1));
        return (float)TB_DADD(s, TB_DMUL(x7, s1));
    }
    double x4 = TB_DMUL(x2, x2);
    double c2 = TB_DADD(csgn * TB_SC_C3, TB_DMUL(x2, csgn * TB_SC_C4));
    double c1 = TB_DADD(csgn * 1.0, TB_DMUL(x2, csgn * TB_SC_C1));
    double x6 = TB_DMUL(x4, x2);
    double c = TB_DADD(c1, TB_DMUL(x4, csgn * TB_SC_C2));
    return (float)TB_DADD(c, TB_DMUL(x6, c2));
}

TB_HD void sincosf_rn(float y, float* sn, float* cs) {
    double x = (double)y;
    if (abstop12(y) < abstop12(0x1.921FB6p-1f)) {
        double x2 = TB_DMUL(x, x);
        if (abstop12(y) < abstop12(0x1p-12f)) {
            *cs = 1.0f;
            *sn = y;
            return;
        }
        *cs = sincos_poly(x, x2, 1.0, 1);
        *sn = sincos_poly(x, x2, 1.0, 0);
        return;
    }
    double r = TB_DMUL(x, TB_SC_HPI_INV);
    int n = ((int32_t)r + 0x800000) >> 24;
    double xr = TB_DSUB(x, TB_DMUL((double)n, TB_SC_HPI));
    const int q = n & 3;
    const double s = (q == 1 || q == 2) ? -1.0 : 1.0;
    const double csgn = (n & 2) ? -1.0 : 1.0;
    double xs = TB_DMUL(xr, s);
    double x2 = TB_DMUL(xr, xr);
    *cs = sincos_poly(xs, x2, csgn, n ^ 1);
    *sn = sincos_poly(xs, x2, csgn, n);
}

TB_HD float fast_atan2(float y, float x) {
    const float p1 = 0.9997878412794807f * (float)(180.0 / 3.14159265358979323846);
    const float p3 = -0.3258083974640975f * (float)(180.0 / 3.14159265358979323846);
    const float p5 = 0.1555786518463281f * (float)(180.0 / 3.14159265358979323846);
    const float p7 = -0.04432655554792128f * (float)(180.0 / 3.14159265358979323846);
    const float eps = (float)2.2204460492503131e-16;
    float ax = fabsf(x), ay = fabsf(y);
    float a, c, c2;
    if (ax >= ay) {
        c = TB_FDIV(ay, TB_FADD(ax, eps));
        c2 = TB_FMUL(c, c);
        a = TB_FMUL(TB_FADD(TB_FMUL(TB_FADD(TB_FMUL(TB_FADD(TB_FMUL(p7, c2), p5), c2), p3), c2), p1), c);
    } else {
        c = TB_FDIV(ax, TB_FADD(ay, eps));
        c2 = TB_FMUL(c, c);
        a = TB_FSUB(90.f, TB_FMUL(TB_FADD(TB_FMUL(TB_FADD(TB_FMUL(TB_FADD(TB_FMUL(p7, c2), p5), c2), p3), c2), p1), c));
    }
    if (x < 0) a = TB_FSUB(180.f, a);
    if (y < 0) a = TB_FSUB(360.f, a);
    return a;
}

TB_HD __attribute__((always_inline)) void three_maxima(const int* sizes, int L, int* ind1, int* ind2, int* ind3) {
    int max1 = 0, max2 = 0, max3 = 0, i1 = *ind1, i2 = *ind2, i3 = *ind3;
    for (int i = 0; i < L; i++) {
        const int s = sizes[i];
        if (s > max1) { max3 = max2; max2 = max1; max1 = s; i3 = i2; i2 = i1; i1 = i; }
        else if (s > max2) { max3 = max2; max2 = s; i3 = i2; i2 = i; }
        else if (s > max3) { max3 = s; i3 = i; }
    }
    if ((float)max2 < 0.1f * (float)max1) { i2 = -1; i3 = -1; }
    else if ((float)max3 < 0.1f * (float)max1) { i3 = -1; }
    *ind1 = i1; *ind2 = i2; *ind3 = i3;
}

TB_HD __attribute__((always_inline)) void kept_bins_ascending(int i1, int i2, int i3, int* keep) {
    int a = i1 < 0 ? (1 << 30) : i1, b = i2 < 0 ? (1 << 30) : i2, c = i3 < 0 ? (1 << 30) : i3, t;
    if (a > b) { t = a; a = b; b = t; }
    if (b > c) { t = b; b = c; c = t; }
    if (a > b) { t = a; a = b; b = t; }
    keep[0] = a < (1 << 30) ? a : -1; keep[1] = b < (1 << 30) ? b : -1; keep[2] = c < (1 << 30) ? c : -1;
}

}
#endif
```

Measured before the change: 31060 frames/s.

## Stream BA observations in wave-interleaved int4 layout for coalesced point passes

Local BA observations are repacked during preparation into a wave-interleaved int4 stream: for each step j, the lanes of a wave that still have an edge read consecutive slots, located with ballot and mbcnt. The points-linearisation and update kernels walk this stream instead of the per-point strided tb_ba_obs arrays. The trial pass also batches its loads, and the Hessian records are read and written as double2 and indexed directly by point when points are renumbered. The aim is coalesced observation loads and fewer dependent index lookups in memory-bound BA kernels. In exchange, preparation does an extra scatter pass, code paths are duplicated through templates, and a debug switch plus a host helper are added to fall back to or check the old layout.

```diff
diff --git a/include/tb_capi.h b/include/tb_capi.h
--- a/include/tb_capi.h
+++ b/include/tb_capi.h
@@ -24,6 +24,7 @@
 int tb_set_concurrency(tb_ctx* ctx, int peers);
 int tb_measure_copy_seconds(tb_ctx* ctx, const void* d_src, void* d_dst, size_t bytes, int reps, double* seconds);
 int tb_debug_force_dense_fast(tb_ctx* ctx, int on);
+int tb_debug_ba_plain_obs(tb_ctx* ctx, int on);
 int tb_profile_report(tb_ctx* ctx, char* buf, int cap);
 
 int tb_scale_factors(int nlevels, float scale, float* sf, float* inv_sf, float* sigma2, float* inv_sigma2);
@@ -246,6 +247,7 @@
 int tb_local_ba_batch_dev(tb_ctx* ctx, int nwindows, const double K[4], int nkf, int nfixed, float* poses, int npt,
                           float* pts, const tb_ba_obs* obs, const int32_t* obs_counts, int obs_pitch, int iters,
                           double* stats);
+int tb_ba_obs_stream_positions(const int32_t* pt_start, int npt, int32_t* pos);
 
 typedef struct tb_vo tb_vo;
 typedef struct tb_vo_params {
diff --git a/trackingbench_slam_amd/capi.py b/trackingbench_slam_amd/capi.py
--- a/trackingbench_slam_amd/capi.py
+++ b/trackingbench_slam_amd/capi.py
@@ -22,7 +22,7 @@
 
 EXPORTS = [
     "tb_create", "tb_destroy", "tb_last_error", "tb_strerror", "tb_version", "tb_set_stream", "tb_synchronize",
-    "tb_profile_enable", "tb_profile_only", "tb_profile_report", "tb_debug_force_dense_fast", "tb_measure_copy_seconds", "tb_set_concurrency", "tb_pack_rows_dev",
+    "tb_profile_enable", "tb_profile_only", "tb_profile_report", "tb_debug_force_dense_fast", "tb_debug_ba_plain_obs", "tb_measure_copy_seconds", "tb_set_concurrency", "tb_pack_rows_dev",
     "tb_scale_factors", "tb_pyramid_sizes", "tb_orb_quotas",
     "tb_extractor_create", "tb_extractor_destroy", "tb_extractor_set_images_host", "tb_extractor_set_images_dev",
     "tb_extractor_set_levels_host", "tb_extractor_build_pyramid", "tb_extractor_get_level_host", "tb_extractor_orb",
@@ -33,7 +33,7 @@
     "tb_search_by_violence", "tb_search_by_bow", "tb_search_by_projection", "tb_search_by_projection_map", "tb_frame_grid_batch_dev",
     "tb_search_by_projection_batch_dev", "tb_search_by_projection_map_batch_dev",
     "tb_search_by_violence_batch_dev", "tb_stereo_tracks_to_obs_batch_dev", "tb_vocab_create", "tb_vocab_destroy", "tb_bow_transform",
-    "tb_bow_transform_batch_dev", "tb_search_by_bow_batch_dev", "tb_pose_opt", "tb_pose_opt_batch_dev", "tb_local_ba", "tb_local_ba_batch_dev",
+    "tb_bow_transform_batch_dev", "tb_search_by_bow_batch_dev", "tb_pose_opt", "tb_pose_opt_batch_dev", "tb_local_ba", "tb_local_ba_batch_dev", "tb_ba_obs_stream_positions",
     "tb_clahe", "tb_clahe_dev", "tb_optical_flow_pyr_lk", "tb_optical_flow_pyr_lk_dev", "tb_optical_flow_pyr_lk_batch_dev", "tb_search_by_opflow", "tb_search_by_opflow_batch_dev",
     "tb_find_fundamental_ransac", "tb_reject_with_f", "tb_reject_with_f_batch_dev", "tb_add_map_points_by_stereo", "tb_add_map_points_by_stereo_batch_dev",
     "tb_batch_run", "tb_vo_create", "tb_vo_destroy", "tb_vo_reset_dev", "tb_vo_step_dev", "tb_vo_state_dev",
@@ -163,6 +163,15 @@
     return i1.value, i2.value, i3.value
 
 
+def ba_obs_stream_positions(pt_start):
+    pt_start = np.ascontiguousarray(pt_start, np.int32)
+    pos = np.full(int(pt_start[-1]), -1, np.int32)
+    rc = lib().tb_ba_obs_stream_positions(_p(pt_start), len(pt_start) - 1, _p(pos))
+    if rc:
+        raise TBError(rc, "tb_ba_obs_stream_positions")
+    return pos
+
+
 class BatchParams(C.Structure):
     _fields_ = [("width", C.c_int), ("height", C.c_int), ("nlevels", C.c_int), ("scale", C.c_float), ("target", C.c_int),
                 ("init_th", C.c_float), ("min_th", C.c_float), ("bf_ratio", C.c_float), ("bf_min_th", C.c_float)]
@@ -433,6 +442,9 @@
     def set_concurrency(self, peers):
         self.check(lib().tb_set_concurrency(self._h, int(peers)))
 
+    def ba_plain_obs(self, on=True):
+        self.check(lib().tb_debug_ba_plain_obs(self._h, int(on)))
+
     def force_dense_fast(self, on=True):
         self.check(lib().tb_debug_force_dense_fast(self._h, int(on)))
 
diff --git a/trackingbench_slam_amd/csrc/k_ba.hip b/trackingbench_slam_amd/csrc/k_ba.hip
--- a/trackingbench_slam_amd/csrc/k_ba.hip
+++ b/trackingbench_slam_amd/csrc/k_ba.hip
@@ -3,6 +3,7 @@
 #include "tb_internal.h"
 #include "tb_device.h"
 #include "tb_se3.h"
+#include "tb_math.h"
 
 #define BA_T 256
 #ifndef BA_KFCH
@@ -16,6 +17,9 @@
 #define BA_SORT_LDS 8192
 #ifndef BA_EMAX
 #define BA_EMAX 64
+#endif
+#ifndef BA_UPD_BATCH
+#define BA_UPD_BATCH 4
 #endif
 #ifndef BA_PCAP
 #define BA_PCAP 21
@@ -44,6 +48,7 @@
     unsigned long long oGCut;
     int renum;
     unsigned long long oPerm;
+    int stream;
     int schurWaveLds;
     int wgReduce;
 };
@@ -293,30 +298,87 @@
     if (!ok) st->sing = 1;
     const double u00 = i00, u11 = i11, u22 = i22, u01 = -c10 * i00 * i11, u12 = -c21 * i11 * i22,
                  u02 = -(c20 * i00 + c21 * u01) * i22;
-    q[0] = ok ? u00 : 0.0; q[1] = ok ? u01 : 0.0; q[2] = ok ? u02 : 0.0;
-    q[3] = ok ? u11 : 0.0; q[4] = ok ? u12 : 0.0; q[5] = ok ? u22 : 0.0;
-    q[6] = bl[0]; q[7] = bl[1]; q[8] = bl[2];
-    q[9] = X[0]; q[10] = X[1]; q[11] = X[2];
-}
+    ba_d2* q2 = reinterpret_cast<ba_d2*>(q);
+    q2[0] = ba_d2{ok ? u00 : 0.0, ok ? u01 : 0.0};
+    q2[1] = ba_d2{ok ? u02 : 0.0, ok ? u11 : 0.0};
+    q2[2] = ba_d2{ok ? u12 : 0.0, ok ? u22 : 0.0};
+    q2[3] = ba_d2{bl[0], bl[1]};
+    q2[4] = ba_d2{bl[2], X[0]};
+    q2[5] = ba_d2{X[1], X[2]};
+}
+__device__ __forceinline__ void ba_load_rec(const double* __restrict__ q, double* __restrict__ r) {
+    const ba_d2* q2 = reinterpret_cast<const ba_d2*>(q);
+#pragma unroll
+    for (int i = 0; i < 6; i++) { const ba_d2 v = q2[i]; r[2 * i] = v.x; r[2 * i + 1] = v.y; }
+}
+
+struct BaStreamPos { int base, deg; int4 first; };
+template <class F>
+__device__ __forceinline__ void ba_stream_walk(const int4* __restrict__ S, const BaStreamPos& sp, F f) {
+    const int deg = sp.deg;
+    int base = sp.base;
+    unsigned long long m = __ballot(0 < deg);
+    int4 rn = sp.first;
+    for (int j = 0; m != 0; j++) {
+        const int4 r = rn;
+        const unsigned long long mn = __ballot(j + 1 < deg);
+        const int idx = tbm::ba_stream_slot_self(mn, &base);
+        if (j + 1 < deg) rn = S[idx];
+        if (j < deg) f(r);
+        m = mn;
+    }
+}
+template <int N, class F>
+__device__ __forceinline__ void ba_stream_walk_batched(const int4* __restrict__ S, const BaStreamPos& sp, F f) {
+    const int deg = sp.deg;
+    int base = sp.base - __popcll(__ballot(0 < deg));
+    for (int j0 = 0; __ballot(j0 < deg) != 0; j0 += N) {
+        int4 r[N];
+#pragma unroll
+        for (int i = 0; i < N; i++) {
+            const unsigned long long m = __ballot(j0 + i < deg);
+            const int idx = tbm::ba_stream_slot_self(m, &base);
+            r[i] = make_int4(0, 0, 0, 0);
+            if (j0 + i < deg) r[i] = S[idx];
+        }
+#pragma unroll
+        for (int i = 0; i < N; i++)
+            if (j0 + i < deg) f(r[i]);
+    }
+}
+__device__ __forceinline__ BaStreamPos ba_stream_begin(const BaDims& d, const int* __restrict__ I, int p) {
+    BaStreamPos sp;
+    sp.base = I[d.oPtStart + min(p & ~63, d.npt)];
+    sp.deg = (p < d.npt) ? I[d.oPtStart + p + 1] - I[d.oPtStart + p] : 0;
+    sp.first = make_int4(0, 0, 0, 0);
+    const int idx = tbm::ba_stream_slot_self(__ballot(0 < sp.deg), &sp.base);
+    if (0 < sp.deg) sp.first = reinterpret_cast<const int4*>(I + d.oFreeKP)[idx];
+    return sp;
+}
+
 __device__ __forceinline__ void ba_rec_utb(const double* q, double* t) {
     t[0] = q[0] * q[6];
     t[1] = q[1] * q[6] + q[3] * q[7];
     t[2] = q[2] * q[6] + q[4] * q[7] + q[5] * q[8];
 }
 
+template <bool STREAM>
 __device__ __forceinline__ void ba_points_pass(const BaDims& d, const tb_ba_obs* __restrict__ obsAll, double* __restrict__ dw, const int* __restrict__ iw,
                                                BaState* __restrict__ states, const int* __restrict__ errflag, int bx, int w) {
     __shared__ double red[4];
     extern __shared__ __attribute__((aligned(16))) double sRt[];
     const int tid = threadIdx.x;
+    double* D = dw + (size_t)w * d.wstride;
+    const int* I = iw + (size_t)w * d.istride;
+    const int p = bx * BA_T + tid;
+    BaStreamPos sp;
+    if (STREAM) sp = ba_stream_begin(d, I, p);
     if (errflag[w]) {
         if (bx == 0 && tid == 0) { states[w].status = 1; states[w].err = 1; }
         return;
     }
     const BaState st = states[w];
     if (st.status) return;
-    double* D = dw + (size_t)w * d.wstride;
-    const int* I = iw + (size_t)w * d.istride;
     const bool lam_known = st.iter > 0 || !st.need_lin;
     const tb_ba_obs* obs = obsAll + (size_t)w * d.obs_pitch;
     const double* T = D + d.oT + (size_t)st.cur * d.nkf * 7;
@@ -324,33 +386,42 @@
     for (int k = tid; k < d.nkf; k += BA_T) ba_pose_to_Rt(T + k * 7, sRt + k * 12);
     __syncthreads();
     const double delta = (double)sqrtf(5.991f);
-    const int p = bx * BA_T + tid;
+    const bool in = p < d.npt;
     double chi = 0, maxd = 0;
-    if (p < d.npt) {
-        double Hll[6] = {0, 0, 0, 0, 0, 0}, bl[3] = {0, 0, 0};
-        const double X[3] = {P[3 * p], P[3 * p + 1], P[3 * p + 2]};
+    double Hll[6] = {0, 0, 0, 0, 0, 0}, bl[3] = {0, 0, 0}, X[3] = {0, 0, 0};
+    if (in) { X[0] = P[3 * p]; X[1] = P[3 * p + 1]; X[2] = P[3 * p + 2]; }
+    auto edge = [&](int kf, float ou, float ov, float ow) {
+        BaLin L;
+        ba_linearize(sRt + kf * 12, X, ou, ov, ow, d.fx, d.fy, d.cx, d.cy, delta, L);
+        const double ww = L.ww, e0 = L.e0, e1 = L.e1;
+        const double* Jl = L.Jl;
+        chi += ba_huber_rho0(L.c2, delta);
+        for (int a = 0; a < 3; a++) bl[a] = fma(-ww, fma(Jl[a], e0, Jl[3 + a] * e1), bl[a]);
+        Hll[0] = fma(ww, fma(Jl[0], Jl[0], Jl[3] * Jl[3]), Hll[0]);
+        Hll[1] = fma(ww, fma(Jl[0], Jl[1], Jl[3] * Jl[4]), Hll[1]);
+        Hll[2] = fma(ww, fma(Jl[0], Jl[2], Jl[3] * Jl[5]), Hll[2]);
+        Hll[3] = fma(ww, fma(Jl[1], Jl[1], Jl[4] * Jl[4]), Hll[3]);
+        Hll[4] = fma(ww, fma(Jl[1], Jl[2], Jl[4] * Jl[5]), Hll[4]);
+        Hll[5] = fma(ww, fma(Jl[2], Jl[2], Jl[5] * Jl[5]), Hll[5]);
+    };
+    if (STREAM) {
+        ba_stream_walk(reinterpret_cast<const int4*>(I + d.oFreeKP), sp,
+                       [&](const int4& r) { edge(r.x, __int_as_float(r.y), __int_as_float(r.z), __int_as_float(r.w)); });
+    } else if (in) {
         const int eBeg = I[d.oPtStart + p], eEnd = I[d.oPtStart + p + 1];
         tb_ba_obs on = obs[min(eBeg, d.obs_pitch - 1)];
         for (int e = eBeg; e < eEnd; e++) {
             const tb_ba_obs o = on;
             on = obs[min(e + 1, d.obs_pitch - 1)];
-            BaLin L;
-            ba_linearize(sRt + o.kf * 12, X, o.u, o.v, o.inv_sigma2, d.fx, d.fy, d.cx, d.cy, delta, L);
-            const double ww = L.ww, e0 = L.e0, e1 = L.e1;
-            const double* Jl = L.Jl;
-            chi += ba_huber_rho0(L.c2, delta);
-            for (int a = 0; a < 3; a++) bl[a] = fma(-ww, fma(Jl[a], e0, Jl[3 + a] * e1), bl[a]);
-            Hll[0] = fma(ww, fma(Jl[0], Jl[0], Jl[3] * Jl[3]), Hll[0]);
-            Hll[1] = fma(ww, fma(Jl[0], Jl[1], Jl[3] * Jl[4]), Hll[1]);
-            Hll[2] = fma(ww, fma(Jl[0], Jl[2], Jl[3] * Jl[5]), Hll[2]);
-            Hll[3] = fma(ww, fma(Jl[1], Jl[1], Jl[4] * Jl[4]), Hll[3]);
-            Hll[4] = fma(ww, fma(Jl[1], Jl[2], Jl[4] * Jl[5]), Hll[4]);
-            Hll[5] = fma(ww, fma(Jl[2], Jl[2], Jl[5] * Jl[5]), Hll[5]);
-        }
+            edge(o.kf, o.u, o.v, o.inv_sigma2);
+        }
+    }
+    if (in) {
         if (!lam_known) {
             for (int a = 0; a < 6; a++) D[d.oHll + (size_t)p * 6 + a] = Hll[a];
             for (int a = 0; a < 3; a++) D[d.oBl + (size_t)p * 3 + a] = bl[a];
-        } else ba_write_rec(D + d.oHq + (size_t)I[d.oPtRank + p] * 12, Hll, bl, X, st.lambda, states + w);
+        } else
+            ba_write_rec(D + d.oHq + (size_t)(d.renum ? p : I[d.oPtRank + p]) * 12, Hll, bl, X, st.lambda, states + w);
         maxd = fmax(fabs(Hll[0]), fmax(fabs(Hll[3]), fabs(Hll[5])));
     }
     const double s = ba_block_sum1(chi, red);
@@ -456,23 +527,25 @@
     }
 }
 
+template <bool STREAM>
 __global__ void __launch_bounds__(BA_T)
 k_ba_points(BaDims d, const tb_ba_obs* __restrict__ obsAll, double* __restrict__ dw, const int* __restrict__ iw, BaState* __restrict__ states,
             const int* __restrict__ errflag) {
-    ba_points_pass(d, obsAll, dw, iw, states, errflag, (int)blockIdx.x, (int)blockIdx.y);
+    ba_points_pass<STREAM>(d, obsAll, dw, iw, states, errflag, (int)blockIdx.x, (int)blockIdx.y);
 }
 __global__ void __launch_bounds__(BA_T)
 k_ba_kf(BaDims d, const tb_ba_obs* __restrict__ obsAll, double* __restrict__ dw, const int* __restrict__ iw, const BaState* __restrict__ states,
         const int* __restrict__ errflag) {
     ba_kf_pass(d, obsAll, dw, iw, states, errflag, (int)blockIdx.x);
 }
+template <bool STREAM>
 __global__ void __launch_bounds__(BA_T)
 k_ba_lin(BaDims d, const tb_ba_obs* __restrict__ obsAll, double* __restrict__ dw, const int* __restrict__ iw, BaState* __restrict__ states,
          const int* __restrict__ errflag, int nKfBlocks) {
     if ((int)blockIdx.x < nKfBlocks) ba_kf_pass(d, obsAll, dw, iw, states, errflag, (int)blockIdx.x);
     else {
         const int b = (int)blockIdx.x - nKfBlocks;
-        ba_points_pass(d, obsAll, dw, iw, states, errflag, b % d.nblkP, b / d.nblkP);
+        ba_points_pass<STREAM>(d, obsAll, dw, iw, states, errflag, b % d.nblkP, b / d.nblkP);
     }
 }
 
@@ -530,7 +603,7 @@
     for (int i = 0; i < 6; i++) ph[i] = D[d.oHll + (size_t)p * 6 + i];
 #pragma unroll
     for (int i = 0; i < 3; i++) { pb[i] = D[d.oBl + (size_t)p * 3 + i]; X[i] = D[d.oP + ((size_t)st.cur * d.npt + p) * 3 + i]; }
-    ba_write_rec(D + d.oHq + (size_t)I[d.oPtRank + p] * 12, ph, pb, X, st.lambda, states + w);
+    ba_write_rec(D + d.oHq + (size_t)(d.renum ? p : I[d.oPtRank + p]) * 12, ph, pb, X, st.lambda, states + w);
 }
 
 #define BA_MAXT 4
@@ -689,6 +762,22 @@
     }
     __threadfence_block();
     __syncthreads();
+    if (d.stream) {
+        int4* S = reinterpret_cast<int4*>(I + d.oFreeKP);
+        for (int r0 = 64 * wave; r0 < d.npt; r0 += 64 * NW) {
+            const int r = r0 + lane, eBeg = (r < d.npt) ? start2[r] : 0, deg = (r < d.npt) ? start2[r + 1] - eBeg : 0;
+            int base = start2[r0];
+            for (int j = 0;; j++) {
+                const unsigned long long m = __ballot(j < deg);
+                if (m == 0) break;
+                const int idx = tbm::ba_stream_slot_self(m, &base);
+                if (j < deg) {
+                    const tb_ba_obs o = obs2[eBeg + j];
+                    S[idx] = make_int4(o.kf, __float_as_int(o.u), __float_as_int(o.v), __float_as_int(o.inv_sigma2));
+                }
+            }
+        }
+    }
     for (int r = tid; r < d.npt; r += BA_RT) {
         const unsigned m = word[pa_[r]] & 0xffffu;
         first[r] = __popc(m);
@@ -1916,6 +2005,7 @@
     }
 }
 
+template <bool STREAM>
 __global__ void __launch_bounds__(BA_T)
 k_ba_update(BaDims d, const tb_ba_obs* __restrict__ obsAll, double* __restrict__ dw, const int* __restrict__ iw,
             const BaState* __restrict__ states) {
@@ -1925,64 +2015,84 @@
     double* const sRtc = sdyn + (size_t)d.nkf * 12;
     double* const sx = sdyn + (size_t)d.nkf * 24;
     const int w = blockIdx.y, tid = threadIdx.x;
+    double* D = dw + (size_t)w * d.wstride;
+    const int* I = iw + (size_t)w * d.istride;
+    const int p = blockIdx.x * BA_T + tid;
+    BaStreamPos sp;
+    if (STREAM) sp = ba_stream_begin(d, I, p);
+    const bool in = p < d.npt;
+    double q[12] = {0, 0, 0, 0, 0, 0, 0, 0, 0, 0, 0, 0};
+    if (STREAM && in) ba_load_rec(D + d.oHq + (size_t)p * 12, q);
     const BaState st = states[w];
     if (st.status) return;
+    if (!STREAM && in) ba_load_rec(D + d.oHq + (size_t)(d.renum ? p : I[d.oPtRank + p]) * 12, q);
     const tb_ba_obs* obs = obsAll + (size_t)w * d.obs_pitch;
-    double* D = dw + (size_t)w * d.wstride;
-    const int* I = iw + (size_t)w * d.istride;
     const double* Tn = D + d.oT + (size_t)(st.cur ^ 1) * d.nkf * 7;
     for (int k = tid; k < d.nkf; k += BA_T) ba_pose_to_Rt(D + d.oT + ((size_t)st.cur * d.nkf + k) * 7, sRtc + k * 12);
-    const double* P = D + d.oP + (size_t)st.cur * d.npt * 3;
     double* Pn = D + d.oP + (size_t)(st.cur ^ 1) * d.npt * 3;
     for (int k = tid; k < d.nkf; k += BA_T) ba_pose_to_Rt(Tn + k * 7, sRt + k * 12);
     for (int i = tid; i < d.np; i += BA_T) sx[i] = D[d.oXp + i];
     __syncthreads();
     const double delta = (double)sqrtf(5.991f);
-    const int p = blockIdx.x * BA_T + tid;
     double chi = 0, sc = 0;
-    if (p < d.npt) {
-        const double* q = D + d.oHq + (size_t)I[d.oPtRank + p] * 12;
-        double r[3] = {q[6], q[7], q[8]};
-        const double bl[3] = {r[0], r[1], r[2]};
-        double xl[3] = {0, 0, 0};
+    double r[3] = {q[6], q[7], q[8]};
+    const double bl[3] = {r[0], r[1], r[2]};
+    const double Xc[3] = {q[9], q[10], q[11]};
+    double xl[3] = {0, 0, 0}, X[3] = {0, 0, 0};
+    auto back = [&](int kf, float ou, float ov, float ow) {
+        if (kf < d.nfixed) return;
+        BaLin L;
+        double Jp[12];
+        ba_linearize(sRtc + kf * 12, Xc, ou, ov, ow, d.fx, d.fy, d.cx, d.cy, delta, L);
+        ba_jac_pose_iz(L.pc, L.invz, d.fx, d.fy, Jp);
+        const double* xp = sx + 6 * (kf - d.nfixed);
+        double s0 = 0, s1 = 0;
+#pragma unroll
+        for (int a = 0; a < 6; a++) { s0 = fma(Jp[a], xp[a], s0); s1 = fma(Jp[6 + a], xp[a], s1); }
+#pragma unroll
+        for (int c = 0; c < 3; c++) r[c] = fma(-L.ww, fma(L.Jl[c], s0, L.Jl[3 + c] * s1), r[c]);
+    };
+    auto step = [&]() {
+        if (st.ok2) {
+            const double u00 = q[0], u01 = q[1], u02 = q[2], u11 = q[3], u12 = q[4], u22 = q[5];
+            const double t0 = u00 * r[0], t1 = u01 * r[0] + u11 * r[1], t2 = u02 * r[0] + u12 * r[1] + u22 * r[2];
+            xl[0] = u00 * t0 + u01 * t1 + u02 * t2;
+            xl[1] = u11 * t1 + u12 * t2;
+            xl[2] = u22 * t2;
+        }
+        for (int a = 0; a < 3; a++) {
+            X[a] = Xc[a] + xl[a];
+            Pn[3 * p + a] = X[a];
+            sc += xl[a] * (st.lambda * xl[a] + bl[a]);
+        }
+    };
+    auto trial = [&](int kf, float ou, float ov, float ow) {
+        BaLin L;
+        ba_residual(sRt + kf * 12, X, ou, ov, ow, d.fx, d.fy, d.cx, d.cy, delta, L);
+        chi += ba_huber_rho0(L.c2, delta);
+    };
+    if (STREAM) {
+        const int4* S = reinterpret_cast<const int4*>(I + d.oFreeKP);
+        if (st.ok2)
+            ba_stream_walk(S, sp, [&](const int4& e) { back(e.x, __int_as_float(e.y), __int_as_float(e.z), __int_as_float(e.w)); });
+        if (in) step();
+        ba_stream_walk_batched<BA_UPD_BATCH>(S, sp, [&](const int4& e) { trial(e.x, __int_as_float(e.y), __int_as_float(e.z), __int_as_float(e.w)); });
+    } else if (in) {
         const int eBeg = I[d.oPtStart + p], eEnd = I[d.oPtStart + p + 1];
         if (st.ok2) {
-            const double u00 = q[0], u01 = q[1], u02 = q[2], u11 = q[3], u12 = q[4], u22 = q[5];
-            const double Xc[3] = {P[3 * p], P[3 * p + 1], P[3 * p + 2]};
             tb_ba_obs on = obs[min(eBeg, d.obs_pitch - 1)];
             for (int e = eBeg; e < eEnd; e++) {
                 const tb_ba_obs o = on;
                 on = obs[min(e + 1, d.obs_pitch - 1)];
-                if (o.kf < d.nfixed) continue;
-                BaLin L;
-                double Jp[12];
-                ba_linearize(sRtc + o.kf * 12, Xc, o.u, o.v, o.inv_sigma2, d.fx, d.fy, d.cx, d.cy, delta, L);
-                ba_jac_pose_iz(L.pc, L.invz, d.fx, d.fy, Jp);
-                const double* xp = sx + 6 * (o.kf - d.nfixed);
-                double s0 = 0, s1 = 0;
-#pragma unroll
-                for (int a = 0; a < 6; a++) { s0 = fma(Jp[a], xp[a], s0); s1 = fma(Jp[6 + a], xp[a], s1); }
-#pragma unroll
-                for (int c = 0; c < 3; c++) r[c] = fma(-L.ww, fma(L.Jl[c], s0, L.Jl[3 + c] * s1), r[c]);
-            }
-            const double t0 = u00 * r[0], t1 = u01 * r[0] + u11 * r[1], t2 = u02 * r[0] + u12 * r[1] + u22 * r[2];
-            xl[0] = u00 * t0 + u01 * t1 + u02 * t2;
-            xl[1] = u11 * t1 + u12 * t2;
-            xl[2] = u22 * t2;
-        }
-        double X[3];
-        for (int a = 0; a < 3; a++) {
-            X[a] = P[3 * p + a] + xl[a];
-            Pn[3 * p + a] = X[a];
-            sc += xl[a] * (st.lambda * xl[a] + bl[a]);
-        }
+                back(o.kf, o.u, o.v, o.inv_sigma2);
+            }
+        }
+        step();
         tb_ba_obs on2 = obs[min(eBeg, d.obs_pitch - 1)];
         for (int e = eBeg; e < eEnd; e++) {
             const tb_ba_obs o = on2;
             on2 = obs[min(e + 1, d.obs_pitch - 1)];
-            BaLin L;
-            ba_residual(sRt + o.kf * 12, X, o.u, o.v, o.inv_sigma2, d.fx, d.fy, d.cx, d.cy, delta, L);
-            chi += ba_huber_rho0(L.c2, delta);
+            trial(o.kf, o.u, o.v, o.inv_sigma2);
         }
     }
     const double s1 = ba_block_sum1(chi, red);
@@ -2088,6 +2198,7 @@
     }
     d.big = d.nfree > BA_SMALL_MAXF;
     d.renum = (!d.big && npt <= BA_SORT_LDS && nkf <= BA_PREP_MAXKF) ? 1 : 0;
+    d.stream = d.renum;
     d.schurWaveLds = d.big ? 0 : ba_c_wave_lds(d.nfree);
     d.npairs = d.nfree * (d.nfree + 1) / 2;
     d.maxItems = (unsigned long long)obs_pitch * (d.nfree + 1) / 2 + 1;
@@ -2153,6 +2264,7 @@
     if (iters > 99) return tb_fail(ctx, TB_EUNSUPPORTED, "local BA: more than 99 LM iterations (one still-running counter per trial, 1000 of them)");
     BaDims d;
     ba_dims(d, ctx->num_cu, ctx->peers, W, K, nkf, nfixed, npt, obs_pitch, iters);
+    if (ctx->dbg_ba_plain_obs) d.stream = 0;
     if (tbk_local_ba_work_bytes(ctx, W, nkf, nfixed, npt, obs_pitch) > work_bytes) return tb_fail(ctx, TB_ENOMEM, "local BA workspace too small");
     char* base = (char*)d_work;
     double* dw = (double*)base;
@@ -2203,12 +2315,12 @@
             const int nKfBlocks = ((W + 7) / 8) * 8 * std::min(BA_KFBLK, d.kfChunks) * d.nfree;
             if (W <= 32) {
                 tb_prof_begin(ctx, "k_ba_lin");
-                hipLaunchKernelGGL(k_ba_lin, dim3(nKfBlocks + d.nblkP * W), dim3(BA_T), (size_t)d.nkf * 12 * sizeof(double), s, d, d_obs, dw, iw, states,
+                hipLaunchKernelGGL(d.stream ? k_ba_lin<true> : k_ba_lin<false>, dim3(nKfBlocks + d.nblkP * W), dim3(BA_T), (size_t)d.nkf * 12 * sizeof(double), s, d, d_obs, dw, iw, states,
                                    errflag, nKfBlocks);
                 tb_prof_end(ctx);
             } else {
                 tb_prof_begin(ctx, "k_ba_points");
-                hipLaunchKernelGGL(k_ba_points, dim3(d.nblkP, W), dim3(BA_T), (size_t)d.nkf * 12 * sizeof(double), s, d, d_obs, dw, iw, states, errflag);
+                hipLaunchKernelGGL(d.stream ? k_ba_points<true> : k_ba_points<false>, dim3(d.nblkP, W), dim3(BA_T), (size_t)d.nkf * 12 * sizeof(double), s, d, d_obs, dw, iw, states, errflag);
                 tb_prof_end(ctx);
                 tb_prof_begin(ctx, "k_ba_kf");
                 hipLaunchKernelGGL(k_ba_kf, dim3(nKfBlocks), dim3(BA_T), 0, s, d, d_obs, dw, iw, states, errflag);
@@ -2245,7 +2357,7 @@
             tb_prof_end(ctx);
         }
         tb_prof_begin(ctx, "k_ba_update");
-        hipLaunchKernelGGL(k_ba_update, dim3(d.nblkP, W), dim3(BA_T), ((size_t)d.nkf * 24 + d.np) * sizeof(double), s, d, d_obs, dw, iw, states);
+        hipLaunchKernelGGL(d.stream ? k_ba_update<true> : k_ba_update<false>, dim3(d.nblkP, W), dim3(BA_T), ((size_t)d.nkf * 24 + d.np) * sizeof(double), s, d, d_obs, dw, iw, states);
         tb_prof_end(ctx);
         tb_prof_begin(ctx, "k_ba_decide");
         hipLaunchKernelGGL(k_ba_decide, dim3(W), dim3(64), 0, s, d, dw, states, running + round % ring);
diff --git a/trackingbench_slam_amd/csrc/tb_capi.cpp b/trackingbench_slam_amd/csrc/tb_capi.cpp
--- a/trackingbench_slam_amd/csrc/tb_capi.cpp
+++ b/trackingbench_slam_amd/csrc/tb_capi.cpp
@@ -185,6 +185,12 @@
 int tb_debug_force_dense_fast(tb_ctx* ctx, int on) {
     if (!ctx) return TB_EINVAL;
     ctx->dbg_fast_dense = on ? 1 : 0;
+    return TB_OK;
+}
+
+int tb_debug_ba_plain_obs(tb_ctx* ctx, int on) {
+    if (!ctx) return TB_EINVAL;
+    ctx->dbg_ba_plain_obs = on ? 1 : 0;
     return TB_OK;
 }
 
@@ -843,6 +849,24 @@
     return dist;
 }
 
+int tb_ba_obs_stream_positions(const int32_t* pt_start, int npt, int32_t* pos) {
+    if (npt < 0 || !pt_start || (!pos && pt_start[npt] > 0)) return TB_EINVAL;
+    for (int r0 = 0; r0 < npt; r0 += 64) {
+        int base = pt_start[r0];
+        for (int j = 0;; j++) {
+            unsigned long long m = 0;
+            for (int l = 0; l < 64 && r0 + l < npt; l++)
+                if (pt_start[r0 + l + 1] - pt_start[r0 + l] > j) m |= 1ull << l;
+            if (m == 0) break;
+            int next = base;
+            for (int l = 0; l < 64; l++)
+                if ((m >> l) & 1) { next = base; pos[pt_start[r0 + l] + j] = tbm::ba_stream_slot(m, l, &next); }
+            base = next;
+        }
+    }
+    return TB_OK;
+}
+
 void tb_three_maxima(const int* sizes, int L, int* ind1, int* ind2, int* ind3) {
     tbm::three_maxima(sizes, L, ind1, ind2, ind3);
 }
diff --git a/trackingbench_slam_amd/csrc/tb_internal.h b/trackingbench_slam_amd/csrc/tb_internal.h
--- a/trackingbench_slam_amd/csrc/tb_internal.h
+++ b/trackingbench_slam_amd/csrc/tb_internal.h
@@ -40,6 +40,7 @@
     std::vector<std::pair<std::string, hipGraphExec_t>> ba_graphs;
     int peers = 1;
     int dbg_fast_dense = 0;
+    int dbg_ba_plain_obs = 0;
     hipStream_t own_stream = nullptr;
     hipStream_t stream = nullptr;
     std::string err;
diff --git a/trackingbench_slam_amd/csrc/tb_math.h b/trackingbench_slam_amd/csrc/tb_math.h
--- a/trackingbench_slam_amd/csrc/tb_math.h
+++ b/trackingbench_slam_amd/csrc/tb_math.h
@@ -157,5 +157,18 @@
     keep[0] = a < (1 << 30) ? a : -1; keep[1] = b < (1 << 30) ? b : -1; keep[2] = c < (1 << 30) ? c : -1;
 }
 
+TB_HD __attribute__((always_inline)) int ba_stream_slot(unsigned long long m, int lane, int* base) {
+    const int idx = *base + __builtin_popcountll(m & ((1ull << lane) - 1ull));
+    *base += __builtin_popcountll(m);
+    return idx;
+}
+#if defined(__HIPCC__)
+__device__ __forceinline__ int ba_stream_slot_self(unsigned long long m, int* base) {
+    const int idx = *base + (int)__builtin_amdgcn_mbcnt_hi((unsigned)(m >> 32), __builtin_amdgcn_mbcnt_lo((unsigned)m, 0u));
+    *base += __builtin_popcountll(m);
+    return idx;
 }
 #endif
+
+}
+#endif
```

New measurement: 31620 frames/s, median of 6. 1.02x the previous value.
